# luccachiang/GSWorld

Measured on AMD Instinct MI355X. Metric: rendered frames/sec @640x480, 1.5M Gaussians, higher is better.
Workload: dtype f32

## Files before the change

### gsworld_amd/_lib.py

```python
from __future__ import annotations

import ctypes as C
import os

_HERE = os.path.dirname(os.path.abspath(__file__))
LIB_PATH = os.path.join(_HERE, "libgsr_hip.so")

GSR_OK = 0
GSR_E_INVALID = -1
GSR_E_HIP = -2
GSR_E_ALLOC = -3
GSR_E_OVERFLOW = -4
GSR_E_TRUNCATED = -5
GSR_NEAR_PLANE = 0.05
MAX_FRAMES_PER_LAUNCH = 8


class GsrSettings(C.Structure):
    _fields_ = [
        ("image_height", C.c_int32), ("image_width", C.c_int32),
        ("tanfovx", C.c_float), ("tanfovy", C.c_float), ("scale_modifier", C.c_float),
        ("sh_degree", C.c_int32), ("sh_coeffs", C.c_int32),
        ("prefiltered", C.c_int32), ("antialiasing", C.c_int32), ("debug", C.c_int32),
        ("near_plane", C.c_float),
# ... 87 lines not shown
                ("out_depth", C.c_void_p)]


PC_DENSE, PC_STRIDE, PC_FPS = 0, 1, 2
PC_MAX_VIEWS, PC_MAX_K, PC_MAX_FPS_CANDIDATES, PC_MAX_VIEW_PIXELS = 64, 8192, 16384, 1 << 24


class GsrCloudView(C.Structure):
    _fields_ = [("width", C.c_int32), ("height", C.c_int32), ("tanfovx", C.c_float), ("tanfovy", C.c_float),
                ("viewmatrix", C.c_void_p), ("depth", C.c_void_p), ("depth_scale", C.c_float), ("label", C.c_void_p),
                ("rgb8", C.c_void_p)]


class GsrCloudSpec(C.Structure):
    _fields_ = [("struct_size", C.c_int32), ("E", C.c_int32), ("C", C.c_int32), ("views", C.POINTER(GsrCloudView)),
                ("out_from_scene", C.c_float * 12), ("crop", C.c_int32), ("crop_lo", C.c_float * 3),
                ("crop_hi", C.c_float * 3), ("exclude", C.c_void_p), ("mode", C.c_int32), ("K", C.c_int32),
                ("fps_candidates", C.c_int32), ("out_xyzw", C.c_void_p), ("out_rgb", C.c_void_p),
                ("out_segmentation", C.c_void_p), ("out_count", C.c_void_p), ("workspace", C.c_void_p),
                ("workspace_bytes", C.c_int64)]


CAM_MAX_VIEWS, CAM_RECORD_FLOATS = 4096, 36


class GsrSensorCameras(C.Structure):
    _fields_ = [("struct_size", C.c_int32), ("n", C.c_int32), ("extrinsic", C.c_void_p), ("projection", C.c_void_p),
                ("out", C.c_void_p), ("offsets", C.c_void_p), ("rigid_sim2real", C.c_double * 16),
                ("scale_sim2real", C.c_double)]


class GsrProfile(C.Structure):
    _fields_ = [("frames", C.c_int32), ("stage_ms", C.c_double * 5)]


PROFILE_STAGES = ("preprocess", "depth_sort", "tile_counts+ranges", "placement", "render")


class GsrError(RuntimeError):
    def __init__(self, code: int, message: str):
        super().__init__(f"libgsr_hip error {code}: {message}")
        self.code = code


_lib = None


def lib() -> C.CDLL:
    global _lib
    if _lib is not None:
        return _lib
    if not os.path.exists(LIB_PATH):
        raise RuntimeError(
            f"{LIB_PATH} is missing: the HIP extension has not been built. Run "
            "`python -c 'import __graft_entry__ as g; g.build()'` (or `make -C gsworld_amd/csrc`). "
            "There is no CPU fallback for the rasterizer.")
    L = C.CDLL(LIB_PATH)
    L.gsr_last_error.restype = C.c_char_p
    L.gsr_version.restype = C.c_char_p
    if not hasattr(L, "gsr_abi_sizes"):
        raise RuntimeError(f"{LIB_PATH} predates the ABI handshake (gsr_abi_sizes): rebuild it (make -C gsworld_amd/csrc)")
    sizes = (C.c_int32 * 6)()
    L.gsr_abi_sizes(sizes)
    mine = (C.sizeof(GsrSettings), C.sizeof(GsrInputs), C.sizeof(GsrOutputs), C.sizeof(GsrBuffers))
    if tuple(sizes[:4]) != mine:
        raise RuntimeError(f"{LIB_PATH} was built from a different include/gsr.h (struct sizes {tuple(sizes[:4])} there, "
                           f"{mine} in gsworld_amd/_lib.py): rebuild the library")
    L.gsr_geom_bytes.restype = C.c_size_t
    L.gsr_geom_bytes.argtypes = [C.c_int32, C.c_int32, C.c_int32]
    L.gsr_binning_bytes.restype = C.c_size_t
    L.gsr_binning_bytes.argtypes = [C.c_int64]
    L.gsr_image_bytes.restype = C.c_size_t
    L.gsr_image_bytes.argtypes = [C.c_int32, C.c_int32]
    L.gsr_forward.restype = C.c_int
    L.gsr_forward.argtypes = [C.POINTER(GsrSettings), C.POINTER(GsrInputs), C.POINTER(GsrOutputs),
                              C.POINTER(GsrBuffers), C.c_int64, C.POINTER(GsrFrameStats), C.c_void_p]
    L.gsr_forward_batch.restype = C.c_int
    L.gsr_forward_batch.argtypes = [C.c_int32, C.POINTER(GsrSettings), C.POINTER(GsrInputs), C.POINTER(GsrOutputs),
                                    C.POINTER(GsrBuffers), C.POINTER(C.c_int64), C.c_void_p]
    L.gsr_frame_stats.restype = C.c_int
    L.gsr_frame_stats.argtypes = [C.c_void_p, C.POINTER(GsrFrameStats), C.c_void_p]
    L.gsr_debug_sort_state.argtypes = [C.c_void_p, C.POINTER(C.c_int32), C.c_void_p]
    L.gsr_debug_sort_state.restype = C.c_int
    L.gsr_state_view.restype = C.c_int
    L.gsr_state_view.argtypes = [C.c_int32, C.c_int32, C.c_int32, C.c_int64, C.c_void_p, C.c_void_p, C.c_void_p,
                                 C.POINTER(GsrStateView)]
    L.gsr_mark_visible.restype = C.c_int
    L.gsr_mark_visible.argtypes = [C.c_int32, C.c_void_p, C.c_void_p, C.c_float, C.c_void_p, C.c_void_p]
    L.gsr_pack_rgb8.restype = C.c_int
    L.gsr_pack_rgb8.argtypes = [C.c_void_p, C.c_int32, C.c_int32, C.c_void_p, C.c_void_p]
    L.gsr_plan_query.restype = C.c_int
    L.gsr_plan_query.argtypes = [C.POINTER(GsrSettings), C.c_int32, C.c_int32, C.c_int64, C.POINTER(C.c_int32)]
    L.gsr_pinned_device_address.restype = C.c_int
    L.gsr_pinned_device_address.argtypes = [C.c_void_p, C.POINTER(C.c_void_p)]
    L.gsr_stage_step.restype = C.c_int
    L.gsr_stage_step.argtypes = [C.c_int32, C.c_void_p, C.c_void_p, C.c_int32, C.c_int32, C.c_int32, C.c_void_p, C.c_void_p]
    L.gsr_render_maps.restype = C.c_int
    L.gsr_render_maps.argtypes = [C.c_int32, C.POINTER(GsrMapFrame), C.c_void_p]
    L.gsr_render_pointcloud.restype = C.c_int
    L.gsr_render_pointcloud.argtypes = [C.POINTER(GsrCloudSpec), C.c_void_p]
    L.gsr_pointcloud_workspace.restype = C.c_int
    L.gsr_pointcloud_workspace.argtypes = [C.POINTER(GsrCloudSpec), C.POINTER(C.c_int64)]
    L.gsr_cameras_from_extrinsics.restype = C.c_int
    L.gsr_cameras_from_extrinsics.argtypes = [C.POINTER(GsrSensorCameras), C.c_void_p]
    L.gsr_profile_enable.restype = C.c_int
    L.gsr_profile_enable.argtypes = [C.c_int]
    L.gsr_profile_collect.restype = C.c_int
    L.gsr_profile_collect.argtypes = [C.POINTER(GsrProfile)]
    _lib = L
    return L


def check(code: int) -> None:
    if code != GSR_OK:
        raise GsrError(code, lib().gsr_last_error().decode("utf-8", "replace"))


def plan_query(width: int, height: int, P: int, permuted: bool = False, forward_only: bool = True,
               r_capacity: int = 1, tuned: bool = True) -> dict | None:
    st = GsrSettings(int(height), int(width), 1.0, 1.0, 1.0, 3, 16, 0, 0, 0, float(GSR_NEAR_PLANE))
    st.forward_only = int(bool(forward_only))
    if tuned:
        apply_tuning(st)
    out = (C.c_int32 * 8)()
    if lib().gsr_plan_query(C.byref(st), int(P), int(bool(permuted)), int(r_capacity), out) != GSR_OK:
        return None
    keys = ("mode", "placement", "infer", "super", "lean", "radix_depth", "order_early", "exact")
    return dict(zip(keys, (int(v) for v in out)))


def exported_symbols() -> list[str]:
    import re

    header = os.path.join(os.path.dirname(_HERE), "include", "gsr.h")
    text = open(header).read()
    text = re.sub(r"/\*.*?\*/", "", text, flags=re.S)
    return sorted(set(re.findall(r"\b(gsr_[a-z0-9_]+)\s*\(", text)) - {"gsr_resize_fn"})
```

### gsworld_amd/csrc/api.hip

```cpp
#include <stdarg.h>
#include <stdio.h>
#include <string.h>

#include <vector>

#include "gsr_internal.h"

namespace {
thread_local char g_err[512] = "";

constexpr int kStages = GSR_PROFILE_STAGES;
constexpr int kMaxFrames = 4096;
struct Profiler {
    int mode = 0;
    int frames = 0;
    std::vector<hipEvent_t> ev;
    hipEvent_t &at(int frame, int k) { return ev[(size_t)frame * (kStages + 1) + k]; }
};
thread_local Profiler g_prof;

inline void prof_mark(int k, hipStream_t stream) {
    if (g_prof.mode == 0 || g_prof.frames >= kMaxFrames) return;
    if (g_prof.mode == 1 && k < kStages - 1) return;
    (void)hipEventRecord(g_prof.at(g_prof.frames, k), stream);
}
inline void prof_end_frame() {
    if (g_prof.mode != 0 && g_prof.frames < kMaxFrames) g_prof.frames++;
}
}

void gsr_set_error(const char *fmt, ...) {
    va_list ap;
    va_start(ap, fmt);
    vsnprintf(g_err, sizeof(g_err), fmt, ap);
    va_end(ap);
}

int gsr_check_launch(const char *what, bool debug, hipStream_t stream) {
    hipError_t e = hipGetLastError();
    if (e == hipSuccess && debug) e = hipStreamSynchronize(stream);
    if (e != hipSuccess) {
        gsr_set_error("%s: %s", what, hipGetErrorString(e));
        return GSR_E_HIP;
    }
    return GSR_OK;
}

extern "C" {

const char *gsr_last_error(void) { return g_err; }
const char *gsr_version(void) {
    static char v[96] = "";
    if (v[0] == 0) snprintf(v, sizeof(v), "gsworld_amd-gsr 0.4 (gfx950; %s)", gsr_render_build_flags());
    return v;
}
void gsr_abi_sizes(int32_t out[6]) {
    out[0] = (int32_t)sizeof(GsrSettings);
    out[1] = (int32_t)sizeof(GsrInputs);
    out[2] = (int32_t)sizeof(GsrOutputs);
    out[3] = (int32_t)sizeof(GsrBuffers);
    out[4] = (int32_t)sizeof(GsrBackwardInputs);
    out[5] = (int32_t)sizeof(GsrGrads);
}

size_t gsr_geom_bytes(int32_t P, int32_t width, int32_t height) {
    return GeomState::required(P, gsr_div_up(width, GSR_TILE) * gsr_div_up(height, GSR_TILE), gsr_div_up(width, GSR_TILE));
}
size_t gsr_binning_bytes(int64_t r_capacity) { return BinningState::required(r_capacity); }
size_t gsr_image_bytes(int32_t width, int32_t height) { return ImageState::required(width, height); }

static int validate(const GsrSettings *st, const GsrInputs *in, const GsrOutputs *out, const GsrBuffers *buf) {
    if (!st || !in || !out || !buf) {
        gsr_set_error("gsr_forward: null argument struct");
        return GSR_E_INVALID;
    }
    if (st->image_width <= 0 || st->image_height <= 0) {
        gsr_set_error("gsr_forward: image size must be positive");
        return GSR_E_INVALID;
    }
    if (gsr_div_up(st->image_width, GSR_TILE) > 65535 || gsr_div_up(st->image_height, GSR_TILE) > 65535) {
        gsr_set_error("gsr_forward: image too large for 16-bit tile rects");
        return GSR_E_INVALID;
    }
    if (in->P < 0) {
        gsr_set_error("gsr_forward: negative P");
        return GSR_E_INVALID;
    }
    const bool no_float = !out->out_color && !out->out_invdepth && st->forward_only && out->out_rgb8;
    if (((!out->out_color || !out->out_invdepth) && !no_float) || !in->background) {
        gsr_set_error("gsr_forward: out_color, out_invdepth and background are required (the two images may be NULL "
                      "together for a forward_only frame with out_rgb8)");
        return GSR_E_INVALID;
    }
    if (in->P > 0) {
        if (!in->means3D || !in->opacities || !in->viewmatrix || !in->projmatrix || !in->campos ||
            (!out->radii && !st->forward_only)) {
            gsr_set_error("gsr_forward: means3D, opacities, viewmatrix, projmatrix, campos and radii are required "
                          "(radii may be NULL for forward_only frames)");
            return GSR_E_INVALID;
        }
        if ((in->shs == nullptr) == (in->colors_precomp == nullptr)) {
            gsr_set_error("Please provide excatly one of either SHs or precomputed colors!");
            return GSR_E_INVALID;
        }
        const bool have_sr = in->scales != nullptr && in->rotations != nullptr;
        if (have_sr == (in->cov3D_precomp != nullptr) || (in->scales != nullptr) != (in->rotations != nullptr)) {
            gsr_set_error("Please provide exactly one of either scale/rotation pair or precomputed 3D covariance!");
            return GSR_E_INVALID;
        }
        if (in->shs) {
            if (st->sh_degree < 0 || st->sh_degree > 3 || st->sh_coeffs < (st->sh_degree + 1) * (st->sh_degree + 1)) {
                gsr_set_error("gsr_forward: sh_degree must be 0..3 and sh_coeffs >= (degree+1)^2");
// ... 49 lines not shown

namespace {

struct Plan {
    int W, H, tiles, tiles_x, tiles_y;
    int mode;
    bool chunk, band;
    bool exact;
    bool infer, super, lean, order_early, lean_bin;
    bool radix_depth;
    GsrSettings st_bin;
};

int make_plan(const GsrSettings *st, const GsrInputs *in, int64_t r_capacity, Plan &p, const GsrOutputs *out = nullptr) {
    p.W = st->image_width;
    p.H = st->image_height;
    p.tiles_x = gsr_div_up(p.W, GSR_TILE);
    p.tiles = p.tiles_x * gsr_div_up(p.H, GSR_TILE);
    p.tiles_y = p.tiles / p.tiles_x;
    if (r_capacity > 0xFFFFFFFFll) {
        gsr_set_error("gsr_forward: r_capacity exceeds 32-bit instance offsets");
        return GSR_E_INVALID;
    }
    const int want = (st->binning_path == 0 || st->binning_path >= 3) ? 1 : (st->binning_path == 1 ? 0 : 2);
    p.mode = GeomState::counting(p.tiles) && p.tiles_x <= 2048 ? want : 0;
    p.chunk = p.mode == 1 && st->binning_path == 4 && gsr_chunk_supported(p.tiles_x, p.tiles / p.tiles_x);
    p.band = p.mode == 1 && (st->binning_path == 0 || (st->binning_path == 4 && !p.chunk)) &&
             gsr_band_supported(p.tiles_x);
    p.exact = r_capacity <= 0;
    p.radix_depth = st->depth_sort == 1 || !gsr_ss_supported(in->P);
    p.infer = st->forward_only != 0 && (p.band || p.chunk) && !p.radix_depth;
    p.super = p.infer && st->render_variant == 0 && p.tiles_x <= 255 && p.tiles_y <= 255 &&
              gsr_render_uses_quad_order(*st, p.tiles) && gsr_render_split_blocks(*st, p.tiles) == 0;
    p.lean = p.infer && !p.chunk;
    p.st_bin = *st;
    if (p.super) {
        p.st_bin.image_width = gsr_div_up(p.tiles_x, 1 << GSR_SUPER_SX) * GSR_TILE;
        p.st_bin.image_height = gsr_div_up(p.tiles_y, 1 << GSR_SUPER_SY) * GSR_TILE;
    }
    if (in->orig_index != nullptr && !(p.infer && p.mode == 1)) {
        gsr_set_error("gsr_forward: orig_index (a permuted model) needs a forward_only frame on the default sort / "
                      "placement path");
        return GSR_E_INVALID;
    }
    if (out && !out->out_color && !p.super) {
        gsr_set_error("gsr_forward: out_color / out_invdepth may only be NULL for an inference frame on the default path "
                      "(super-tile lists, stream compositor)");
        return GSR_E_INVALID;
    }
    p.order_early = (p.band || p.chunk) && !p.radix_depth && gsr_render_uses_quad_order(*st, p.tiles);
    p.lean_bin = p.band || p.chunk;
    return GSR_OK;
}

int run_frames(int B, const GsrSettings *st, const GsrInputs *in, const GsrOutputs *out, const GsrBuffers *buf,
               const int64_t *r_capacity, const Plan *plans, GsrFrameStats *stats, hipStream_t stream) {
    const Plan &p = plans[0];
    const bool debug = st[0].debug != 0;
    const int mode = p.mode;
    const bool chunk = p.chunk, band = p.band, exact = p.exact, infer = p.infer, super = p.super;
    const int coop = super && band && mode == 1 && !p.radix_depth && p.order_early ? gsr_render_coop_blocks(st[0], p.tiles, B) : 0;
    GsrFrame fr[GSR_MAX_BATCH];
    for (int k = 0; k < B; k++) {
        GsrFrame &f = fr[k];
        f.st = &st[k];
        f.st_bin = &plans[k].st_bin;
        f.in = &in[k];
        f.out = &out[k];
        char *geom_mem = buf[k].geom_resize(buf[k].geom_user, GeomState::required(in[k].P, p.tiles, p.tiles_x, p.lean));
        char *img_mem = buf[k].image_resize(buf[k].image_user, ImageState::required(p.W, p.H));
        if (!geom_mem || !img_mem) {
            gsr_set_error("gsr_forward: resize callback returned NULL");
            return GSR_E_ALLOC;
        }
        f.g = GeomState::carve(geom_mem, in[k].P, p.tiles, nullptr, p.tiles_x, p.lean);
        f.img = ImageState::carve(img_mem, p.W, p.H);
        f.cap32 = exact ? 0xFFFFFFFFu : (uint32_t)r_capacity[k];
        f.pc = GSR_PREP_BLOCK_CACHE && infer && band && mode == 1 && !p.radix_depth && ((uint32_t)in[k].param_space >> 8) != 0u &&
               in[k].part_labels != nullptr && in[k].cull_blocks != nullptr && out[k].radii == nullptr &&
               in[k].part_count <= GSR_PC_MAX_PARTS &&
               (in[k].appearance == nullptr || in[k].appearance_versions != nullptr);
        f.td = GSR_TILE_REUSE && f.pc && super && (in[k].param_space & GSR_FRAME_KEPT) != 0 && out[k].out_rgb8 != nullptr &&
               out[k].out_color == nullptr && out[k].out_invdepth == nullptr;
    }
    const GeomState &g = fr[0].g;
    const ImageState &img = fr[0].img;

    if (mode == 2) {
        const size_t head = offsetof(GsrHeader, of_magic);
        const size_t clear = (size_t)((char *)g.tile_cursor - (char *)g.tile_accum);
        if (hipMemsetAsync(g.hdr, 0, head, stream) != hipSuccess ||
            hipMemsetAsync(g.tile_accum, 0, clear, stream) != hipSuccess) {
            gsr_set_error("gsr_forward: hipMemsetAsync(header) failed");
            return GSR_E_HIP;
        }
    }
    prof_mark(0, stream);
    if (int e = gsr_launch_preprocess(B, fr, mode == 2, infer, stream)) return e;
    if (int e = gsr_check_launch("preprocess", debug, stream)) return e;
    prof_mark(1, stream);
    if (mode != 2) {
        if (p.radix_depth) {
            if (int e = gsr_launch_compact_and_depth_sort(in[0].P, g, debug, stream)) return e;
            if (band || chunk)
                if (int e = gsr_launch_gather_rects(in[0].P, g, debug, stream)) return e;
        } else {
            if (int e = gsr_launch_sample_depth_sort(B, fr, p.order_early, 4 * p.tiles, super ? 1 : 0, coop, debug, stream))
                return e;
        }
    }
    prof_mark(2, stream);
    if (mode == 2) {
        if (int e = gsr_launch_bin_starts(st[0], g, img, fr[0].cap32, debug, stream)) return e;
    } else if (chunk) {
        if (int e = gsr_launch_chunk_count(p.st_bin, in[0].P, g, debug, stream)) return e;
        if (int e = gsr_launch_tile_starts(1, fr, p.order_early, debug, stream)) return e;
    } else if (band) {
        bool starts_done = false;
        if (int e = gsr_launch_band_count(B, fr, !p.radix_depth, p.order_early, &starts_done, debug, stream)) return e;
        if (!starts_done)
            if (int e = gsr_launch_tile_starts(B, fr, p.order_early, debug, stream)) return e;
    } else if (mode == 1) {
        if (int e = gsr_launch_tile_count(st[0], in[0].P, g, img, fr[0].cap32, debug, stream)) return e;
    } else {
        if (int e = gsr_launch_tile_offsets(in[0].P, g, fr[0].cap32, debug, stream)) return e;
    }
    prof_mark(3, stream);
    if (!(band || chunk))
        for (int k = 0; k < B; k++)
            if (out[k].overflow_mirror &&
                hipMemcpyAsync(out[k].overflow_mirror, &fr[k].g.hdr->of_magic, 8, hipMemcpyDefault, stream) != hipSuccess) {
                gsr_set_error("gsr_forward: overflow mirror copy failed: %s", hipGetErrorString(hipGetLastError()));
                return GSR_E_HIP;
            }
    int64_t cap0 = r_capacity[0];
    if (exact) {
        GsrHeader h;
        if (hipMemcpyAsync(&h, g.hdr, sizeof(h), hipMemcpyDeviceToHost, stream) != hipSuccess ||
            hipStreamSynchronize(stream) != hipSuccess) {
            gsr_set_error("gsr_forward: header read-back failed: %s", hipGetErrorString(hipGetLastError()));
            return GSR_E_HIP;
        }
        cap0 = h.R_raw;
        if (stats) {
            stats->num_visible = h.V;
            stats->num_rendered = h.R_raw;
            stats->overflow = 0;
            stats->overflow_frames = h.of_magic == GSR_OF_MAGIC ? (int32_t)h.overflow_frames : 0;
        }
    }
    for (int k = 0; k < B; k++) {
        const int64_t cap = k == 0 ? cap0 : r_capacity[k];
        char *bin_mem = buf[k].binning_resize(buf[k].binning_user, BinningState::required(cap, p.lean_bin));
        if (!bin_mem) {
            gsr_set_error("gsr_forward: binning resize callback returned NULL");
            return GSR_E_ALLOC;
        }
        fr[k].b = BinningState::carve(bin_mem, cap, nullptr, p.lean_bin);
    }
    const BinningState &b = fr[0].b;
    if (mode == 2) {
        if (int e = gsr_launch_bin_scatter_and_sort(st[0], in[0].P, g, b, img, debug, stream)) return e;
    } else if (chunk) {
        if (int e = gsr_launch_chunk_place(p.st_bin, in[0].P, g, b, img, debug, stream)) return e;
    } else if (band) {
        if (int e = gsr_launch_band_place(B, fr, debug, stream)) return e;
    } else if (mode == 1) {
        if (int e = gsr_launch_tile_place(st[0], in[0].P, g, b, img, debug, stream)) return e;
    } else {
        if (int e = gsr_launch_emit_and_tile_sort(st[0], in[0].P, g, b, img, cap0, debug, stream)) return e;
    }
    prof_mark(4, stream);
    if (int e = gsr_launch_render(B, fr, mode != 0, mode == 1, super, coop, stream)) return e;
    prof_mark(5, stream);
    prof_end_frame();
    return gsr_check_launch("render", debug, stream);
}

int zero_outputs(const GsrSettings *st, const GsrOutputs *out, hipStream_t stream) {
    const size_t n = (size_t)st->image_width * st->image_height;
    if ((out->out_color && hipMemsetAsync(out->out_color, 0, 3 * n * sizeof(float), stream) != hipSuccess) ||
        (out->out_invdepth && hipMemsetAsync(out->out_invdepth, 0, n * sizeof(float), stream) != hipSuccess) ||
        (out->out_rgb8 && hipMemsetAsync(out->out_rgb8, 0, 3 * n, stream) != hipSuccess)) {
        gsr_set_error("gsr_forward: hipMemsetAsync(outputs) failed");
        return GSR_E_HIP;
    }
    return GSR_OK;
}

}

extern "C" {

int gsr_forward(const GsrSettings *st, const GsrInputs *in, const GsrOutputs *out, const GsrBuffers *buf,
                int64_t r_capacity, GsrFrameStats *stats, void *stream_) {
    if (int e = validate(st, in, out, buf)) return e;
    hipStream_t stream = (hipStream_t)stream_;
    if (stats) memset(stats, 0, sizeof(*stats));
    if (in->P == 0) return zero_outputs(st, out, stream);
    Plan p;
    if (int e = make_plan(st, in, r_capacity, p, out)) return e;
    return run_frames(1, st, in, out, buf, &r_capacity, &p, stats, stream);
}

int gsr_forward_batch(int32_t B, const GsrSettings *st, const GsrInputs *in, const GsrOutputs *out,
                      const GsrBuffers *buf, const int64_t *r_capacity, void *stream_) {
    if (B < 0 || (B > 0 && (!st || !in || !out || !buf || !r_capacity))) {
        gsr_set_error("gsr_forward_batch: null argument array or negative B");
        return GSR_E_INVALID;
    }
    hipStream_t stream = (hipStream_t)stream_;
    for (int k = 0; k < B; k++)
        if (int e = validate(&st[k], &in[k], &out[k], &buf[k])) return e;
    Plan plans[GSR_MAX_BATCH];
    auto shares = [&](int a, int b, const Plan &pa, const Plan &pb) {
        const GsrSettings &x = st[a], &y = st[b];
        return in[a].P == in[b].P && pa.W == pb.W && pa.H == pb.H && pa.mode == pb.mode && pa.band == pb.band &&
               pa.infer == pb.infer && pa.super == pb.super && pa.lean == pb.lean && pa.order_early == pb.order_early &&
               x.sh_degree == y.sh_degree && x.sh_coeffs == y.sh_coeffs && x.debug == y.debug &&
               x.render_variant == y.render_variant && x.render_blocks_per_cu == y.render_blocks_per_cu &&
               x.render_split == y.render_split && x.depth_sort == y.depth_sort &&
               (in[a].colors_precomp == nullptr) == (in[b].colors_precomp == nullptr);
    };
    int k = 0;
    while (k < B) {
        if (in[k].P == 0) {
            if (int e = zero_outputs(&st[k], &out[k], stream)) return e;
            k++;
            continue;
        }
        if (int e = make_plan(&st[k], &in[k], r_capacity[k], plans[0], &out[k])) return e;
        int n = 1;
        const bool batchable = plans[0].mode == 1 && plans[0].band && !plans[0].radix_depth && !plans[0].exact &&
                               st[k].render_variant == 0;
        while (batchable && n < GSR_MAX_BATCH && k + n < B && in[k + n].P != 0 && r_capacity[k + n] > 0) {
            if (int e = make_plan(&st[k + n], &in[k + n], r_capacity[k + n], plans[n], &out[k + n])) return e;
            if (!shares(k, k + n, plans[0], plans[n])) break;
            n++;
        }
        if (int e = run_frames(n, st + k, in + k, out + k, buf + k, r_capacity + k, plans, nullptr, stream)) return e;
        k += n;
    }
    return GSR_OK;
}

int gsr_plan_query(const GsrSettings *st, int32_t P, int32_t permuted, int64_t r_capacity, int32_t out[8]) {
    if (!st || !out || P < 0 || st->image_width <= 0 || st->image_height <= 0) {
        gsr_set_error("gsr_plan_query: null argument, negative P or empty image");
        return GSR_E_INVALID;
    }
    GsrInputs in;
    memset(&in, 0, sizeof(in));
    in.P = P;
    static const int32_t one = 0;
    in.orig_index = permuted ? &one : nullptr;
    Plan p;
    if (int e = make_plan(st, &in, r_capacity, p)) return e;
    out[0] = p.mode;
    out[1] = p.band ? 1 : (p.chunk ? 2 : 0);
    out[2] = p.infer ? 1 : 0;
    out[3] = p.super ? 1 : 0;
    out[4] = p.lean ? 1 : 0;
    out[5] = p.radix_depth ? 1 : 0;
    out[6] = p.order_early ? 1 : 0;
    out[7] = p.exact ? 1 : 0;
    return GSR_OK;
}

int gsr_render_maps(int32_t B, const GsrMapFrame *frames, void *stream_) {
    if (B < 0 || (B > 0 && !frames)) {
        gsr_set_error("gsr_render_maps: null frame array or negative B");
        return GSR_E_INVALID;
    }
    hipStream_t stream = (hipStream_t)stream_;
    std::vector<GsrMapsArgs> jobs;
    jobs.reserve((size_t)B);
    bool debug = false;
    for (int k = 0; k < B; k++) {
        const GsrMapFrame &f = frames[k];
        if (f.struct_size != (int32_t)sizeof(GsrMapFrame)) {
            gsr_set_error("gsr_render_maps: frame %d: struct_size %d, this library's GsrMapFrame has %d bytes", k,
                          (int)f.struct_size, (int)sizeof(GsrMapFrame));
            return GSR_E_INVALID;
        }
        const GsrSettings *st = f.settings;
        if (!st || st->image_width <= 0 || st->image_height <= 0 || f.P < 0) {
            gsr_set_error("gsr_render_maps: frame %d: null settings, empty image or negative P", k);
            return GSR_E_INVALID;
        }
        if (f.out_label && !f.labels) {
            gsr_set_error("gsr_render_maps: frame %d: out_label needs labels", k);
            return GSR_E_INVALID;
        }
        if (f.P > 0 && (!f.geom || !f.binning || !f.image)) {
            gsr_set_error("gsr_render_maps: frame %d: the frame's three state buffers are required", k);
            return GSR_E_INVALID;
        }
        GsrInputs in;
        memset(&in, 0, sizeof(in));
        in.P = f.P;
        static const int32_t one = 0;
        in.orig_index = f.permuted ? &one : nullptr;
        Plan p;
        if (make_plan(st, &in, f.r_capacity, p) != GSR_OK) {
            gsr_set_error("gsr_render_maps: frame %d is not one gsr_forward renders (permuted model on another path, or "
                          "r_capacity beyond 32 bits)", k);
            return GSR_E_INVALID;
        }
        debug = debug || st->debug != 0;
        const size_t n = (size_t)p.W * p.H;
        if (f.P == 0) {
            if ((f.out_label && hipMemsetAsync(f.out_label, 0xFF, n * sizeof(int16_t), stream) != hipSuccess) ||
                (f.out_depth && hipMemsetAsync(f.out_depth, 0, n * sizeof(float), stream) != hipSuccess)) {
                gsr_set_error("gsr_render_maps: hipMemsetAsync failed");
                return GSR_E_HIP;
            }
            continue;
        }
        if (!f.out_label && !f.out_depth) continue;
        const GeomState g = GeomState::carve((char *)f.geom, f.P, p.tiles);
        const BinningState b = BinningState::carve((char *)f.binning, 1);
        const ImageState s = ImageState::carve((char *)f.image, p.W, p.H);
        GsrMapsArgs a;
        a.ranges = s.ranges;
        a.point_list = b.gidx[0];
        a.splat = g.splat;
        a.hdr = g.hdr;
        a.labels = f.labels;
        a.out_label = f.out_label;
        a.out_depth = f.out_depth;
        a.depth_scale = f.depth_scale;
        a.W = p.W;
        a.H = p.H;
        a.gx = p.tiles_x;
        a.gy = p.tiles_y;
        a.super = p.super ? 1 : 0;
        jobs.push_back(a);
    }
    if (jobs.empty()) return GSR_OK;
    return gsr_launch_maps((int)jobs.size(), jobs.data(), debug, stream);
}

int gsr_profile_enable(int mode) {
    if (mode < 0 || mode > 2) {
        gsr_set_error("gsr_profile_enable: mode must be 0, 1 or 2");
        return GSR_E_INVALID;
    }
    if (mode != 0 && g_prof.ev.empty()) {
        g_prof.ev.resize((size_t)kMaxFrames * (kStages + 1));
        for (auto &e : g_prof.ev)
            if (hipEventCreate(&e) != hipSuccess) {
                gsr_set_error("gsr_profile_enable: hipEventCreate failed");
                return GSR_E_HIP;
            }
    }
    g_prof.mode = mode;
    g_prof.frames = 0;
    return GSR_OK;
}

int gsr_profile_collect(GsrProfile *out) {
    if (!out) {
        gsr_set_error("gsr_profile_collect: null output");
        return GSR_E_INVALID;
    }
    memset(out, 0, sizeof(*out));
    out->frames = g_prof.frames;
    for (int f = 0; f < g_prof.frames; f++) {
        for (int k = (g_prof.mode == 1 ? kStages - 1 : 0); k < kStages; k++) {
            if (hipEventSynchronize(g_prof.at(f, k + 1)) != hipSuccess) {
                gsr_set_error("gsr_profile_collect: hipEventSynchronize failed");
                return GSR_E_HIP;
            }
            float ms = 0.f;
            if (hipEventElapsedTime(&ms, g_prof.at(f, k), g_prof.at(f, k + 1)) != hipSuccess) {
                gsr_set_error("gsr_profile_collect: hipEventElapsedTime failed");
                return GSR_E_HIP;
            }
            out->stage_ms[k] += (double)ms;
        }
    }
    g_prof.frames = 0;
    return GSR_OK;
}

int gsr_debug_ss_stamps(int32_t P, int32_t width, int32_t height, const void *geom, uint64_t *out64) {
    if (!geom || !out64) {
        gsr_set_error("gsr_debug_ss_stamps: null argument");
        return GSR_E_INVALID;
    }
    const bool lean = height < 0;
    if (lean) height = -height;
    const GeomState g = GeomState::carve((char *)geom, P, gsr_div_up(width, GSR_TILE) * gsr_div_up(height, GSR_TILE),
                                         nullptr, gsr_div_up(width, GSR_TILE), lean);
    if (hipDeviceSynchronize() != hipSuccess ||
        hipMemcpy(out64, g.ss_dbg, 64 * sizeof(uint64_t), hipMemcpyDeviceToHost) != hipSuccess) {
        gsr_set_error("gsr_debug_ss_stamps: copy failed");
        return GSR_E_HIP;
    }
    return GSR_OK;
}

int gsr_debug_sort_state(const void *geom, int32_t out[8], void *stream_) {
    if (!geom || !out) {
        gsr_set_error("gsr_debug_sort_state: null argument");
        return GSR_E_INVALID;
    }
    hipStream_t stream = (hipStream_t)stream_;
    GsrHeader h;
    if (hipMemcpyAsync(&h, geom, sizeof(h), hipMemcpyDeviceToHost, stream) != hipSuccess ||
        hipStreamSynchronize(stream) != hipSuccess) {
        gsr_set_error("gsr_debug_sort_state: read-back failed: %s", hipGetErrorString(hipGetLastError()));
        return GSR_E_HIP;
    }
    out[0] = (int32_t)h.ss_blind;
    out[1] = (int32_t)h.ss_fresh;
    out[2] = (int32_t)h.ss_bad;
    out[3] = (int32_t)h.ss_trust;
    out[4] = (int32_t)h.ss_B;
    out[5] = (int32_t)h.ss_stride;
    out[6] = (int32_t)h.coop_quads;
    out[7] = (int32_t)((h.ss_near & 1u) | ((h.pc_hit_last & 1u) << 1) | ((h.td_skipped & 1u) << 2));
    return GSR_OK;
}

int gsr_frame_stats(const void *geom, GsrFrameStats *stats, void *stream_) {
    if (!geom || !stats) {
        gsr_set_error("gsr_frame_stats: null argument");
        return GSR_E_INVALID;
    }
    hipStream_t stream = (hipStream_t)stream_;
    GsrHeader h;
    if (hipMemcpyAsync(&h, geom, sizeof(h), hipMemcpyDeviceToHost, stream) != hipSuccess ||
        hipStreamSynchronize(stream) != hipSuccess) {
        gsr_set_error("gsr_frame_stats: read-back failed: %s", hipGetErrorString(hipGetLastError()));
        return GSR_E_HIP;
    }
    stats->num_visible = h.V;
    stats->num_rendered = h.R_raw;
    stats->overflow = (int32_t)h.overflow;
    stats->overflow_frames = h.of_magic == GSR_OF_MAGIC ? (int32_t)h.overflow_frames : 0;
    stats->truncated = h.coop_timeout_now != 0u ? 1 : 0;
    stats->coop_timeouts = h.of_magic == GSR_OF_MAGIC ? (int32_t)h.coop_timeouts : 0;
    return h.overflow ? GSR_E_OVERFLOW : (stats->truncated ? GSR_E_TRUNCATED : GSR_OK);
}

int gsr_state_view(int32_t P, int32_t width, int32_t height, int64_t r_capacity, const void *geom, const void *binning,
                   const void *image, GsrStateView *v) {
    if (!v) {
        gsr_set_error("gsr_state_view: null view");
        return GSR_E_INVALID;
    }
    memset(v, 0, sizeof(*v));
    if (geom) {
        const GeomState g = GeomState::carve((char *)geom, P, gsr_div_up(width, GSR_TILE) * gsr_div_up(height, GSR_TILE));
        v->splat = reinterpret_cast<const float *>(g.splat);
        v->cov3D = g.cov3D;
        v->clamped = reinterpret_cast<const uint8_t *>(g.clamped);
        v->tiles_touched = g.tiles_touched;
        v->rects = reinterpret_cast<const uint16_t *>(g.rects);
        v->depth_order = g.order;
    }
    if (binning) {
        const BinningState b = BinningState::carve((char *)binning, r_capacity);
        v->point_list = b.gidx[0];
        v->point_tiles = nullptr;
    }
    if (image) {
        const ImageState s = ImageState::carve((char *)image, width, height);
        v->ranges = reinterpret_cast<const uint32_t *>(s.ranges);
        v->final_T = s.final_T;
        v->n_contrib = s.n_contrib;
    }
    return GSR_OK;
}

}
```

### gsworld_amd/csrc/bandplace.hip

```cpp
#include "gsr_internal.h"

#ifndef GSR_BAND_EXACT_CUTS
#define GSR_BAND_EXACT_CUTS 0
#endif

namespace {

constexpr int kBT = GSR_BLOCK;
constexpr int kBW = kBT / GSR_WAVE;
constexpr int kRing = 128;
constexpr uint32_t kSplit2 = 1024u, kSplit4 = 2048u;
constexpr int kMaxSegments = 4;

constexpr uint32_t kCutsMagic = 0x43555453u;

__device__ __forceinline__ uint32_t band_cuts_block(const GsrHeader *__restrict__ hdr, int bmax,
                                                    const uint32_t *__restrict__ bucket_start,
                                                    const uint32_t *__restrict__ bucket_tiles,
                                                    const uint32_t *__restrict__ tile_cum,
                                                    const uint32_t *__restrict__ wave_lo_base, uint32_t sig, uint32_t r,
                                                    uint32_t *s_cut , uint32_t *s_pre ,
                                                    uint32_t *s_bs , uint32_t *s_w ) {
    constexpr int waves = GSR_BAND_RANGES * kBW;
    static_assert(waves == kBT, "a thread per kept cut");
    const int tid = (int)threadIdx.x;
    const uint32_t V = hdr->V, base_V = hdr->br_V, magic = hdr->br_magic, hP = hdr->br_P;
    const int B = (int)hdr->ss_B;
    const uint32_t wb0 = wave_lo_base[tid], wb1 = wave_lo_base[tid + 1];
    const uint32_t wbj = tid <= kBW ? wave_lo_base[r * (uint32_t)kBW + (uint32_t)tid] : 0u;
    if (tile_cum == nullptr || V == 0u) {
        const uint32_t per = (((V + (uint32_t)waves - 1u) / (uint32_t)waves) + 63u) & ~63u;
        if (tid <= kBW) s_cut[tid] = min(V, (r * (uint32_t)kBW + (uint32_t)tid) * per);
        __syncthreads();
        return 0u;
    }
    bool keep = magic == kCutsMagic && hP == sig && base_V != 0u;
    if (keep) {
        uint32_t bad = wb0 > wb1 ? 1u : 0u;
        if (tid == 0) bad |= wb0 != 0u ? 1u : 0u;
        if (tid == waves - 1) bad |= wb1 != base_V ? 1u : 0u;
        keep = __syncthreads_or((int)bad) == 0;
    }
    if (keep) {
        if (tid <= kBW) {
            const uint32_t j = r * (uint32_t)kBW + (uint32_t)tid;
            s_cut[tid] = j == (uint32_t)waves ? V : min(V, (uint32_t)((double)wbj * ((double)V / (double)base_V)));
        }
        __syncthreads();
        return 1u;
    }
    const int PER = B / kBT;
    uint32_t bt[8], bs[8];
#pragma unroll
    for (int k = 0; k < 8; k++) {
        bt[k] = k < PER ? bucket_tiles[tid + k * kBT] : 0u;
        bs[k] = k < PER ? bucket_start[tid + k * kBT] : 0u;
    }
    const uint32_t bs_B = tid == 0 ? bucket_start[B] : 0u;
#pragma unroll
    for (int k = 0; k < 8; k++)
        if (k < PER) {
            s_pre[tid + k * kBT] = bt[k];
            s_bs[tid + k * kBT] = bs[k];
        }
    if (tid == 0) s_bs[B] = bs_B;
    __syncthreads();
    uint32_t t[8], sum = 0;
#pragma unroll
    for (int k = 0; k < 8; k++) {
        t[k] = k < PER ? s_pre[tid * PER + k] : 0u;
        sum += t[k];
    }
    uint32_t total;
    uint32_t run = gsr_block_incl_scan(sum, s_w, total) - sum;
#pragma unroll
    for (int k = 0; k < 8; k++) {
        if (k < PER && t[k] != 0u) {
            const int b = tid * PER + k;
#pragma unroll
            for (int c = 0; c <= kBW; c++) {
                const uint32_t j = r * (uint32_t)kBW + (uint32_t)c;
                const uint32_t target = (uint32_t)(((uint64_t)total * j) / (uint32_t)waves);
                if (j != (uint32_t)waves && target >= run && target - run < t[k]) {
                    const uint32_t s0 = s_bs[b], n = s_bs[b + 1] - s0, rest = target - run;
                    s_cut[c] = s0 + min(n, (uint32_t)((float)n * ((float)rest / (float)t[k])));
                }
            }
        }
        run += t[k];
    }
    if (tid <= kBW) {
        const uint32_t j = r * (uint32_t)kBW + (uint32_t)tid;
        if (j == (uint32_t)waves || total == 0u) s_cut[tid] = j == (uint32_t)waves ? V : 0u;
    }
    __syncthreads();
// ... 141 lines not shown
        v[k] = lane * PL + k < GSR_BAND_RANGES ? row[lane * PL + k] : 0u;
        sum += v[k];
    }
    const uint32_t incl = gsr_wave_incl_scan(sum);
    uint32_t run = incl - sum;
#pragma unroll
    for (int k = 0; k < PL; k++) {
        if (lane * PL + k < GSR_BAND_RANGES) row[lane * PL + k] = run;
        run += v[k];
    }
    if (lane == 63) totals[t] = incl;
}

__device__ __forceinline__ uint64_t wave_bit_transpose(uint64_t R) {
    const uint32_t lane = (uint32_t)gsr_lane();
    constexpr uint64_t kLow[6] = {0x00000000FFFFFFFFull, 0x0000FFFF0000FFFFull, 0x00FF00FF00FF00FFull,
                                  0x0F0F0F0F0F0F0F0Full, 0x3333333333333333ull, 0x5555555555555555ull};
#pragma unroll
    for (int i = 0; i < 6; i++) {
        const int s = 32 >> i;
        const uint64_t m = kLow[i];
        const uint32_t tlo = (uint32_t)__shfl_xor((int)(uint32_t)R, s, 64);
        const uint32_t thi = (uint32_t)__shfl_xor((int)(uint32_t)(R >> 32), s, 64);
        const uint64_t t = ((uint64_t)thi << 32) | tlo;
        R = (lane & (uint32_t)s) == 0u ? ((R & m) | ((t & m) << s)) : ((R & ~m) | ((t & ~m) >> s));
    }
    return R;
}

template <int NC>
__device__ __forceinline__ void band_place_round(uint32_t span, uint32_t g, bool valid, int gx, uint32_t *cur,
                                                 unsigned long long *colmask, uint32_t *__restrict__ point_list) {
    const int lane = gsr_lane();
    const uint64_t lt = gsr_lanemask_lt();
    const uint32_t minx = span & 0xffffu, maxx = span >> 16, w = valid ? maxx - minx : 0u;
    constexpr uint32_t kNarrow = 16;
    const uint32_t wn = min(w, kNarrow);
    uint32_t wmax = wn;
#pragma unroll
    for (int o = 32; o > 0; o >>= 1) wmax = max(wmax, (uint32_t)__shfl_xor((int)wmax, o, 64));
    wmax = (uint32_t)__builtin_amdgcn_readfirstlane((int)wmax);
    uint32_t add[NC];
#pragma unroll
    for (int k = 0; k < NC; k++) {
        const uint32_t lo = max(minx, (uint32_t)(64 * k)), hi = min(maxx, (uint32_t)(64 * k + 64));
        uint64_t row = 0ull;
        if (valid && hi > lo) row = (hi - lo == 64u ? ~0ull : ((1ull << (hi - lo)) - 1ull)) << (lo - (uint32_t)(64 * k));
        const uint64_t col = wave_bit_transpose(row);
        colmask[k * 64 + lane] = col;
        add[k] = (uint32_t)__popcll(col);
    }
    __builtin_amdgcn_wave_barrier();
    for (uint32_t j0 = 0; j0 < wmax; j0 += 4u) {
        unsigned long long m[4];
        uint32_t cx[4];
#pragma unroll
        for (uint32_t u = 0; u < 4u; u++) {
            m[u] = j0 + u < wn ? colmask[minx + j0 + u] : 0ull;
            cx[u] = j0 + u < wn ? cur[minx + j0 + u] : 0u;
        }
#pragma unroll
        for (uint32_t u = 0; u < 4u; u++)
            if (j0 + u < wn) point_list[cx[u] + (uint32_t)__popcll(m[u] & lt)] = g;
    }
    for (uint64_t wide = __builtin_amdgcn_ballot_w64(w > kNarrow); wide;) {
        const int src = __ffsll((unsigned long long)wide) - 1;
        wide &= wide - 1ull;
        const uint32_t sw = (uint32_t)__builtin_amdgcn_readlane((int)w, src);
        const uint32_t sx = (uint32_t)__builtin_amdgcn_readlane((int)minx, src);
        const uint32_t sg = (uint32_t)__builtin_amdgcn_readlane((int)g, src);
        const uint64_t below = (1ull << src) - 1ull;
        for (uint32_t j = kNarrow + (uint32_t)lane; j < sw; j += 64u)
            point_list[cur[sx + j] + (uint32_t)__popcll(colmask[sx + j] & below)] = sg;
    }
    __builtin_amdgcn_wave_barrier();
#pragma unroll
    for (int k = 0; k < NC; k++) cur[k * 64 + lane] += add[k];
    __builtin_amdgcn_wave_barrier();
}

constexpr int kPlaceBatch = 6;

template <int NC>
__device__ __forceinline__ void band_place_body(const uint32_t seg, const uint2 *__restrict__ rect_sorted,
                                                         const uint32_t *__restrict__ order,
                                                         const GsrHeader *__restrict__ hdr,
                                                         const uint32_t *__restrict__ wave_lo, int gx, int NR,
                                                         const uint32_t *__restrict__ table,
                                                         const uint32_t *__restrict__ wtable,
                                                         const uint2 *__restrict__ ranges,
                                                         uint32_t *__restrict__ point_list,
                                                         const uint32_t *__restrict__ nseg_tab) {
    __shared__ uint2 s_ring[kBW][kRing];
    __shared__ unsigned long long s_mask[kBW][NC * 64];
    __shared__ uint32_t s_cur[kBW][NC * 64];
    const int lane = gsr_lane(), wave = gsr_wave();
    const uint32_t r = blockIdx.x, y = blockIdx.y;
    const uint32_t nseg = (nseg_tab[(size_t)y * (uint32_t)NR + r] >> (8u * (uint32_t)__builtin_amdgcn_readfirstlane(wave))) & 255u;
    if (seg >= nseg) return;
    if (hdr->overflow) return;
    const uint32_t lo = wave_lo[r * kBW + (uint32_t)wave], hi = wave_lo[r * kBW + (uint32_t)wave + 1u];
    if (lo >= hi) return;
    uint2 *ring = s_ring[wave];
    uint32_t *cur = s_cur[wave];
    unsigned long long *colmask = s_mask[wave];
    const uint32_t *wbase = wtable + (size_t)(y * (uint32_t)NR + r) * kBW * (NC * 64);
    uint32_t x0 = 0u, x1 = (uint32_t)gx;
    if (nseg > 1u) {
        uint32_t mine[NC], total = 0u;
#pragma unroll
        for (int k = 0; k < NC; k++) {
            const int x = k * 64 + lane;
            mine[k] = x < gx ? wbase[wave * (NC * 64) + x] : 0u;
            total += mine[k];
        }
#pragma unroll
        for (int o = 32; o > 0; o >>= 1) total += (uint32_t)__shfl_xor((int)total, o, 64);
        {
            uint32_t before = 0u, first = 0xFFFFFFFFu, last = 0u;
#pragma unroll
            for (int k = 0; k < NC; k++) {
                const uint32_t incl = gsr_wave_incl_scan(mine[k]);
                const uint32_t excl = before + incl - mine[k];
                const bool in = k * 64 + lane < gx && (uint32_t)(((uint64_t)excl * nseg) / total) == seg;
                const uint64_t m = __builtin_amdgcn_ballot_w64(in);
                if (m != 0ull) {
                    first = min(first, (uint32_t)(k * 64 + __builtin_ctzll(m)));
                    last = max(last, (uint32_t)(k * 64 + 64 - __builtin_clzll(m)));
                }
                before += (uint32_t)__builtin_amdgcn_readlane((int)incl, 63);
            }
            if (first == 0xFFFFFFFFu) return;
            x0 = first;
            x1 = last;
        }
    }
#pragma unroll
    for (int k = 0; k < NC; k++) {
        const int x = k * 64 + lane;
        uint32_t s = 0u;
        if (x < gx) {
            const size_t tile = (size_t)y * gx + x;
            s = ranges[tile].x + table[tile * NR + r];
            for (int w = 0; w < wave; w++) s += wbase[w * (NC * 64) + x];
        }
        cur[x] = s;
    }
    __builtin_amdgcn_wave_barrier();
    uint32_t head = 0, tail = 0;
    for (uint32_t base = lo; base < hi; base += (uint32_t)(kPlaceBatch * GSR_WAVE)) {
        uint2 rc[kPlaceBatch];
        uint32_t g[kPlaceBatch];
#pragma unroll
        for (int u = 0; u < kPlaceBatch; u++) {
            const uint32_t i = base + (uint32_t)(u * GSR_WAVE + lane);
            rc[u] = i < hi ? rect_sorted[i] : make_uint2(0u, 0u);
            g[u] = i < hi ? order[i] : 0u;
        }
#pragma unroll
        for (int u = 0; u < kPlaceBatch; u++) {
            const uint32_t miny = rc[u].x >> 16, maxy = rc[u].y >> 16;
            const uint32_t minx = max(rc[u].x & 0xffffu, x0), maxx = min(rc[u].y & 0xffffu, x1);
            const bool keep = miny <= y && y < maxy && minx < maxx;
            const uint64_t mask = __builtin_amdgcn_ballot_w64(keep);
            if (mask == 0ull) continue;
            if (keep) {
                const uint32_t rank = __builtin_amdgcn_mbcnt_hi((uint32_t)(mask >> 32),
                                                                __builtin_amdgcn_mbcnt_lo((uint32_t)mask, 0u));
                ring[(tail + rank) & (kRing - 1)] = make_uint2(minx | (maxx << 16), g[u]);
            }
            tail += (uint32_t)__popcll(mask);
            __builtin_amdgcn_wave_barrier();
            if (tail - head >= (uint32_t)GSR_WAVE) {
                const uint2 p = ring[(head + (uint32_t)lane) & (kRing - 1)];
                __builtin_amdgcn_wave_barrier();
                band_place_round<NC>(p.x, p.y, true, gx, cur, colmask, point_list);
                head += (uint32_t)GSR_WAVE;
            }
        }
    }
    if (tail != head) {
        const bool valid = (uint32_t)lane < tail - head;
        const uint2 p = valid ? ring[(head + (uint32_t)lane) & (kRing - 1)] : make_uint2(0u, 0u);
        band_place_round<NC>(p.x, p.y, valid, gx, cur, colmask, point_list);
    }
}

struct BandArgs {
    GsrHeader *hdr;
    int bmax;
    const uint32_t *bucket_start, *bucket_tiles, *tile_cum;
    int waves;
    uint32_t *wave_lo, *wave_lo_base;
    uint32_t sig;
    const uint2 *rect_sorted;
    int gx, NR, T;
    uint32_t *table, *wtable, *totals, *nseg;
    const uint32_t *order;
    const uint2 *ranges;
    uint32_t *point_list;
    uint32_t r_capacity;
    uint2 *ranges_w;
    const uint32_t *quad_work;
    uint32_t *tile_order;
    uint32_t *mirror;
};

template <int NC>
__global__ __launch_bounds__(kBT) void band_count_kernel(const GsrBatch<BandArgs> bt) {
    const BandArgs &a = bt.f[blockIdx.z];
    band_count_body<NC>(a.rect_sorted, a.hdr, a.bmax, a.bucket_start, a.bucket_tiles, a.tile_cum, a.waves, a.wave_lo, a.wave_lo_base,
                        a.sig, a.gx, a.NR, a.table, a.wtable, a.nseg);
}
__global__ __launch_bounds__(kBT) void band_scan_kernel(const GsrBatch<BandArgs> bt) {
    const BandArgs &a = bt.f[blockIdx.y];
    if (blockIdx.x == gridDim.x - 1) {
        band_cuts_next(a.hdr, a.bucket_start, a.bucket_tiles, a.tile_cum, a.wave_lo_base, a.sig);
        return;
    }
    band_scan_body(a.table, a.T, a.totals);
}
template <int NC>
__global__ __launch_bounds__(kBT, 8) void band_place_kernel(const GsrBatch<BandArgs> bt) {
    const BandArgs &a = bt.f[blockIdx.z / (uint32_t)kMaxSegments];
    band_place_body<NC>(blockIdx.z % (uint32_t)kMaxSegments, a.rect_sorted, a.order, a.hdr, a.wave_lo, a.gx, a.NR, a.table,
                        a.wtable, a.ranges, a.point_list, a.nseg);
}

#ifndef GSR_SCAN_MODE
#define GSR_SCAN_MODE 1
#endif
constexpr int kSST = 1024, kSSW = kSST / GSR_WAVE;
constexpr int kSSMaxTiles = 8 * kSST;
constexpr int kSSMergeTiles = 1024;
static_assert(GSR_BAND_RANGES == GSR_WAVE, "a tile's row of the band table is one entry per lane");

template <int THREADS, int MAXPER>
__device__ __forceinline__ void band_starts_block(const uint32_t *totals, int T, GsrHeader *__restrict__ hdr,
                                                  uint32_t r_capacity, uint2 *__restrict__ ranges, uint32_t *s_wv,
                                                  uint32_t *__restrict__ mirror) {
    constexpr int NWV = THREADS / GSR_WAVE;
    const int tid = (int)threadIdx.x, lane = gsr_lane(), wave = tid >> 6;
    const int per = (T + THREADS - 1) / THREADS, t0 = tid * per;
    uint32_t v[MAXPER], sum = 0;
#pragma unroll
    for (int k = 0; k < MAXPER; k++) {
        v[k] = (k < per && t0 + k < T) ? totals[t0 + k] : 0u;
        sum += v[k];
    }
    const uint32_t incl = gsr_wave_incl_scan(sum);
    if (lane == 63) s_wv[wave] = incl;
    __syncthreads();
    uint32_t add = 0, grand = 0;
#pragma unroll
    for (int w = 0; w < NWV; w++) {
        const uint32_t x = s_wv[w];
        add += w < wave ? x : 0u;
        grand += x;
    }
    uint32_t run = incl - sum + add;
    const bool overflow = grand > r_capacity;
#pragma unroll
    for (int k = 0; k < MAXPER; k++) {
        const int t = t0 + k;
        if (k < per && t < T) ranges[t] = (v[k] == 0u || overflow) ? make_uint2(0u, 0u) : make_uint2(run, run + v[k]);
        run += v[k];
    }
    if (tid == 0) {
        hdr->R_raw = grand;
        hdr->r_capacity = r_capacity;
        gsr_set_overflow(hdr, overflow, mirror);
        hdr->R = overflow ? 0u : grand;
    }
}

__device__ __forceinline__ void band_scan_starts_body(uint32_t *__restrict__ table, int T, GsrHeader *__restrict__ hdr,
                                                      uint32_t r_capacity, uint2 *__restrict__ ranges,
                                                      uint32_t *__restrict__ mirror) {
    __shared__ uint32_t s_tot[kSSMaxTiles];
    __shared__ uint32_t s_wv[kSSW];
    const int lane = gsr_lane(), wave = (int)(threadIdx.x >> 6);
    constexpr int kU = 16;
    for (int t0 = wave; t0 < T; t0 += kSSW * kU) {
        uint32_t v[kU];
#pragma unroll
        for (int u = 0; u < kU; u++) {
            const int t = t0 + u * kSSW;
            v[u] = t < T ? table[(size_t)t * GSR_BAND_RANGES + lane] : 0u;
        }
#pragma unroll
        for (int u = 0; u < kU; u++) {
            const int t = t0 + u * kSSW;
            const uint32_t incl = gsr_wave_incl_scan(v[u]);
            if (t < T) {
                table[(size_t)t * GSR_BAND_RANGES + lane] = incl - v[u];
                if (lane == 63) s_tot[t] = incl;
            }
        }
    }
    __syncthreads();
    band_starts_block<kSST, kSSMaxTiles / kSST>(s_tot, T, hdr, r_capacity, ranges, s_wv, mirror);
}

__global__ __launch_bounds__(kSST) void band_scan_starts_kernel(const GsrBatch<BandArgs> bt) {
    const BandArgs &a = bt.f[blockIdx.y];
    if (blockIdx.x == 1) {
        if (threadIdx.x >= kBT) return;
        band_cuts_next(a.hdr, a.bucket_start, a.bucket_tiles, a.tile_cum, a.wave_lo_base, a.sig);
        return;
    }
    if (blockIdx.x == 2) {
        if (threadIdx.x >= kBT) return;
        __shared__ uint32_t s_bins[64], s_red[4];
        uint32_t key[32];
#pragma unroll
        for (int i = 0; i < 32; i++) {
            const int t = (int)threadIdx.x + i * kBT;
            key[i] = t < a.T ? gsr_tile_order_key(nullptr, a.quad_work, t) : 0u;
        }
        gsr_tile_order_block_keys<32>(key, a.T, a.tile_order, s_bins, s_red);
        return;
    }
    band_scan_starts_body(a.table, a.T, a.hdr, a.r_capacity, a.ranges_w, a.mirror);
}
__global__ __launch_bounds__(kBT) void band_scan_tail_kernel(const GsrBatch<BandArgs> bt) {
    const BandArgs &a = bt.f[blockIdx.y];
    __shared__ uint32_t s_last, s_wv[kBW];
    if (blockIdx.x == gridDim.x - 1) {
        band_cuts_next(a.hdr, a.bucket_start, a.bucket_tiles, a.tile_cum, a.wave_lo_base, a.sig);
        return;
    }
    band_scan_body(a.table, a.T, a.totals);
    __threadfence();
    __syncthreads();
    if (threadIdx.x == 0) s_last = atomicAdd(&a.hdr->tile_queue, 1u) == gridDim.x - 2u ? 1u : 0u;
    __syncthreads();
    if (s_last == 0u) return;
    __threadfence();
    if (threadIdx.x == 0) a.hdr->tile_queue = 0u;
    band_starts_block<kBT, kSSMaxTiles / kBT>(a.totals, a.T, a.hdr, a.r_capacity, a.ranges_w, s_wv, a.mirror);
}

__global__ __launch_bounds__(kBT) void gather_rects_kernel(const uint32_t *__restrict__ order,
                                                           const uint2 *__restrict__ rects,
                                                           const GsrHeader *__restrict__ hdr,
                                                           uint2 *__restrict__ rect_sorted) {
    const uint32_t V = hdr->V;
    for (uint32_t i = blockIdx.x * (uint32_t)kBT + threadIdx.x; i < V; i += gridDim.x * (uint32_t)kBT)
        rect_sorted[i] = rects[order[i]];
}

}

bool gsr_band_supported(int gx) { return gx <= 256; }

int gsr_launch_gather_rects(int32_t P, const GeomState &g, bool debug, hipStream_t stream) {
    const int blocks = GeomState::prep_blocks(P) < 1024 ? GeomState::prep_blocks(P) : 1024;
    hipLaunchKernelGGL(gather_rects_kernel, dim3(blocks), dim3(kBT), 0, stream, g.order, g.rects, g.hdr, g.rect_sorted);
    return gsr_check_launch("gather_rects", debug, stream);
}

static void band_args(int B, const GsrFrame *fr, bool balanced, bool place, GsrBatch<BandArgs> &bt) {
    for (int k = 0; k < B; k++) {
        const GeomState &g = fr[k].g;
        const GsrSettings &st = *fr[k].st_bin;
        BandArgs &a = bt.f[k];
        const int32_t P = fr[k].in->P;
        a.hdr = g.hdr;
        a.bmax = gsr_ss_bmax(P);
        a.bucket_start = g.ss_bucket_start;
        a.bucket_tiles = g.bucket_tiles;
        a.tile_cum = balanced ? g.tile_cum : (const uint32_t *)nullptr;
        a.waves = GSR_BAND_RANGES * kBW;
        a.wave_lo = g.wave_lo;
        a.wave_lo_base = g.wave_lo_base;
        a.sig = (uint32_t)P * 2654435761u ^ (uint32_t)((char *)g.wave_lo_base - (char *)g.hdr);
        a.rect_sorted = g.rect_sorted;
        a.gx = gsr_div_up(st.image_width, GSR_TILE);
        a.NR = GSR_BAND_RANGES;
        a.T = a.gx * gsr_div_up(st.image_height, GSR_TILE);
        a.table = g.band_table;
        a.wtable = g.band_wtable;
        a.totals = g.tile_totals;
        a.nseg = g.band_nseg;
        a.order = g.order;
        a.ranges = fr[k].img.ranges;
        a.ranges_w = fr[k].img.ranges;
        a.r_capacity = fr[k].cap32;
        a.quad_work = fr[k].img.quad_work;
        a.tile_order = fr[k].img.tile_order;
        a.mirror = fr[k].out ? fr[k].out->overflow_mirror : (uint32_t *)nullptr;
        a.point_list = place ? fr[k].b.gidx[0] : (uint32_t *)nullptr;
    }
}

int gsr_launch_band_count(int B, const GsrFrame *fr, bool balanced, bool merge_starts, bool *starts_done, bool debug,
                          hipStream_t stream) {
    const GsrSettings &st = *fr[0].st_bin;
    const int gx = gsr_div_up(st.image_width, GSR_TILE), gy = gsr_div_up(st.image_height, GSR_TILE);
    GsrBatch<BandArgs> bt{};
    band_args(B, fr, balanced, false, bt);
    const dim3 grid(GSR_BAND_RANGES, gy, B);
    if (gx <= 64)
        hipLaunchKernelGGL(band_count_kernel<1>, grid, dim3(kBT), 0, stream, bt);
    else if (gx <= 128)
        hipLaunchKernelGGL(band_count_kernel<2>, grid, dim3(kBT), 0, stream, bt);
    else
        hipLaunchKernelGGL(band_count_kernel<4>, grid, dim3(kBT), 0, stream, bt);
    if (int e = gsr_check_launch("band_count", debug, stream)) return e;
    const int T = gx * gy;
    const bool by_tiles = !merge_starts && gsr_render_wants_tile_order(st, T) && !gsr_render_uses_quad_order(st, T);
    const bool merged = GSR_SCAN_MODE != 0 && (merge_starts || (by_tiles && GSR_SCAN_MODE == 1)) && T <= kSSMergeTiles &&
                        gsr_render_split_blocks(st, T) == 0;
    if (starts_done) *starts_done = merged;
    if (merged && GSR_SCAN_MODE == 1) {
        hipLaunchKernelGGL(band_scan_starts_kernel, dim3(by_tiles ? 3 : 2, B), dim3(kSST), 0, stream, bt);
        return gsr_check_launch("band_scan_starts", debug, stream);
    }
    if (merged) {
        hipLaunchKernelGGL(band_scan_tail_kernel, dim3(gsr_div_up(T, kBW) + 1, B), dim3(kBT), 0, stream, bt);
        return gsr_check_launch("band_scan_tail", debug, stream);
    }
    hipLaunchKernelGGL(band_scan_kernel, dim3(gsr_div_up(T, kBW) + 1, B), dim3(kBT), 0, stream, bt);
    return gsr_check_launch("band_scan", debug, stream);
}

int gsr_launch_band_place(int B, const GsrFrame *fr, bool debug, hipStream_t stream) {
    const GsrSettings &st = *fr[0].st_bin;
    const int gx = gsr_div_up(st.image_width, GSR_TILE), gy = gsr_div_up(st.image_height, GSR_TILE);
    GsrBatch<BandArgs> bt{};
    band_args(B, fr, true, true, bt);
    const dim3 grid(GSR_BAND_RANGES, gy, kMaxSegments * B);
    if (gx <= 64)
        hipLaunchKernelGGL(band_place_kernel<1>, grid, dim3(kBT), 0, stream, bt);
    else if (gx <= 128)
        hipLaunchKernelGGL(band_place_kernel<2>, grid, dim3(kBT), 0, stream, bt);
    else
        hipLaunchKernelGGL(band_place_kernel<4>, grid, dim3(kBT), 0, stream, bt);
    return gsr_check_launch("band_place", debug, stream);
}
```

### gsworld_amd/csrc/depthsort.hip

```cpp
#include "gsr_internal.h"
#include <type_traits>

namespace {

#ifdef GSR_SS_TIMING
#define SS_STAMP(buf, slot) do { __syncthreads(); if (blockIdx.x == (buf##_wg) && threadIdx.x == 0) (buf)[slot] = __builtin_amdgcn_s_memtime(); } while (0)
#else
#define SS_STAMP(buf, slot) do { } while (0)
#endif

constexpr int kT = GSR_BLOCK;
#ifndef GSR_SS_TRUST_MIN
#define GSR_SS_TRUST_MIN 2
#endif
#ifndef GSR_SS_IGNORE_BAD
#define GSR_SS_IGNORE_BAD 0
#endif
#ifndef GSR_SS_SPB
#define GSR_SS_SPB 4
#endif
constexpr int kSamplesPerBucket = GSR_SS_SPB;
constexpr int kMinSamples = 2048;
constexpr int kMaxSamples = 4096;
constexpr uint32_t kSplitMagic = 0x53504c54u;
// ... 297 lines not shown
__device__ __forceinline__ void ss_prepare_body(int P, int nb1, int bmax, int nbc,
                                                const uint2 *__restrict__ block_recs,
                                                const uint32_t *__restrict__ block_counts,
                                                const uint32_t *__restrict__ splitters,
                                                uint32_t *__restrict__ splitters_new, uint32_t *__restrict__ seg_off,
                                                uint32_t *__restrict__ seg_first, GsrHeader *__restrict__ hdr,
                                                uint64_t *__restrict__ dbg, const float *__restrict__ view,
                                                uint32_t sig, const int role, const bool pc_enabled) {
    const unsigned dbg_wg = 0; (void)dbg_wg;
    SS_STAMP(dbg, 0);
#ifdef GSR_SS_TIMING
    if (role == 0 && threadIdx.x < 8) dbg[48 + threadIdx.x] = 0ull;
#endif
    __shared__ uint32_t s_key[2 * kMaxSamples];
    __shared__ __attribute__((aligned(16))) uint32_t s_cur[kPW * 256];
    __shared__ uint32_t s_split[2048], s_hist[2048];
    __shared__ uint32_t s_pex[kPT + 8];
    __shared__ __attribute__((aligned(16))) uint16_t s_cnt16[kPrepBlocks];
    __shared__ uint32_t s_w16[kPW];
    const int tid = (int)threadIdx.x, wave = tid >> 6, lane = gsr_lane();
    const int per = ss_prepare_per(nb1);
    const uint32_t h_magic = hdr->ss_magic, h_buckets = hdr->ss_buckets, h_bad = hdr->ss_bad, h_trust = hdr->ss_trust,
                   h_P = hdr->ss_P, h_near = hdr->ss_near, h_near_fail = hdr->ss_near_fail, h_vfail = hdr->ss_vfail;
    const uint32_t h_pc_pending = hdr->pc_pending, h_pc_parity = hdr->pc_parity, h_pc_sig_next = hdr->pc_sig_next,
                   h_pc_hit = hdr->pc_hit;
    bool same_view = true, near_view = true;
#pragma unroll
    for (int k = 0; k < 16; k++) {
        const uint32_t was = hdr->ss_view[k];
        same_view = same_view && __float_as_uint(view[k]) == was;
        near_view = near_view && fabsf(view[k] - __uint_as_float(was)) <= kNearTol;
    }
    uint32_t pre_sp[2];
#pragma unroll
    for (int k = 0; k < 2; k++) pre_sp[k] = tid + k * kPT < bmax - 1 ? splitters[tid + k * kPT] : 0xFFFFFFFFu;
    for (int i0 = tid; i0 < per * kPT; i0 += 8 * kPT) {
        uint32_t c[8];
#pragma unroll
        for (int u = 0; u < 8; u++) c[u] = i0 + u * kPT < nb1 ? block_counts[i0 + u * kPT] : 0u;
#pragma unroll
        for (int u = 0; u < 8; u++)
            if (i0 + u * kPT < per * kPT) s_cnt16[i0 + u * kPT] = (uint16_t)c[u];
    }
    __syncthreads();
    uint32_t mine = 0;
    {
        uint4 *sl = reinterpret_cast<uint4 *>(s_cnt16 + (size_t)tid * per);
        for (int w = 0; w < (per >> 3); w++) {
            const uint4 v = sl[w];
            const uint32_t x[4] = {v.x, v.y, v.z, v.w};
            uint32_t o[4];
#pragma unroll
            for (int h = 0; h < 4; h++) {
                mine += x[h] & 0xffffu;
                const uint32_t a = mine;
                mine += x[h] >> 16;
                o[h] = a | (mine << 16);
            }
            sl[w] = make_uint4(o[0], o[1], o[2], o[3]);
        }
    }
    SS_STAMP(dbg, 1);
    uint32_t V;
    const uint32_t p_incl = ss_scan1024(mine, s_w16, V), p_excl = p_incl - mine;
    (void)p_incl;
    s_pex[tid] = p_excl;
    if (tid == 0) s_pex[kPT] = V;
    if (tid == 0 && role == 0) {
        if (pc_enabled && h_pc_pending == GSR_PC_MAGIC) {
            hdr->pc_parity = (h_pc_parity & 1u) ^ 1u;
            hdr->pc_sig = h_pc_sig_next;
            hdr->pc_magic = GSR_PC_MAGIC;
        } else {
            hdr->pc_magic = 0u;
        }
        hdr->pc_pending = 0u;
        hdr->pc_hit_last = pc_enabled ? h_pc_hit : 0u;
        hdr->pc_hit = 0u;
        hdr->td_skipped = 0u;
        hdr->V = V;
        hdr->R = 0u;
        hdr->overflow = 0u;
        hdr->coop_timeout_now = 0u;
        hdr->r_capacity = 0u;
        hdr->R_raw = 0u;
        hdr->tile_queue = 0u;
    }
    if (V == 0u) {
        if (role == 1)
            for (int j = tid; j <= nbc; j += kPT) {
                seg_off[j] = 0u;
                seg_first[j] = (uint32_t)nb1;
            }
        if (tid == 0 && role == 0) {
            hdr->ss_fresh = 0u;
            hdr->ss_B = 256u;
            hdr->ss_stride = 1u;
            hdr->ss_near = 0u;
            hdr->ss_moved = 1u;
        }
        return;
    }
    __syncthreads();
    SS_STAMP(dbg, 22);
    if (role == 1) {
    if (tid <= nbc) {
        uint32_t j = 0u, before_j = 0u;
        if (tid == nbc) {
            j = (uint32_t)nb1;
            before_j = V;
        } else if (tid > 0) {
            const uint32_t W = V + kBlockCost * (uint32_t)nb1;
            const uint32_t t = (uint32_t)((double)W * (double)tid / (double)nbc);
            uint32_t us = 0u;
#pragma unroll
            for (int st = kPT / 2; st > 0; st >>= 1)
                if (s_pex[us + (uint32_t)st] + kBlockCost * min((uint32_t)nb1, (us + (uint32_t)st) * (uint32_t)per) <= t)
                    us += (uint32_t)st;
            const uint32_t jb = min((uint32_t)nb1, us * (uint32_t)per), je = min((uint32_t)nb1, jb + (uint32_t)per);
            uint32_t pos = 0u;
#pragma unroll
            for (int st = 16; st > 0; st >>= 1) {
                const uint32_t k = jb + pos + (uint32_t)st;
                if (pos + (uint32_t)st < (uint32_t)per && k < je &&
                    s_pex[us] + (uint32_t)s_cnt16[k - 1u] + kBlockCost * k <= t)
                    pos += (uint32_t)st;
            }
            j = jb + pos;
            before_j = s_pex[us] + (pos > 0u ? (uint32_t)s_cnt16[j - 1u] : 0u);
        }
        seg_off[tid] = before_j;
        seg_first[tid] = j;
    }
        return;
    }
    int B0 = ss_num_buckets(V, bmax, (uint32_t)GSR_SS_PER_BUCKET);
    if (GSR_SS_NEAR != 0 && h_magic == kSplitMagic && h_P == sig && h_buckets >= 256u && h_buckets <= (uint32_t)bmax &&
        (h_buckets & (h_buckets - 1u)) == 0u && V >= h_buckets * 224u && V <= h_buckets * 576u)
        B0 = (int)h_buckets;
    const int Bf = ss_num_buckets(V, bmax, (uint32_t)GSR_SS_PER_BUCKET_FULL);
    const bool table_ok = h_magic == kSplitMagic && h_buckets <= (uint32_t)bmax && (GSR_SS_IGNORE_BAD || h_bad == 0u) &&
                          h_trust <= 255u && h_P == sig;
    const bool blind_same = same_view && table_ok && (h_buckets == (uint32_t)Bf || h_buckets == 2u * (uint32_t)Bf) &&
                            h_trust >= (uint32_t)GSR_SS_TRUST_MIN;
    uint32_t near_fail = h_near_fail > 6u ? 0u : h_near_fail;
    if (h_magic == kSplitMagic && h_near == 1u && h_bad != 0u && near_fail < 6u) near_fail++;
    const bool blind_near = GSR_SS_NEAR != 0 && !same_view && near_view && table_ok && h_buckets == (uint32_t)B0 &&
                            h_trust >= (2u << near_fail);
    bool blind = blind_same || blind_near;
    const int B = blind_same ? Bf : B0;
    const uint32_t stride = blind_same ? h_buckets / (uint32_t)Bf : 1u;
    if (tid == 0) {
        hdr->ss_B = (uint32_t)B;
        hdr->ss_stride = stride;
        hdr->ss_moved = same_view ? 0u : 1u;
        hdr->ss_near_fail = near_fail;
    }
    const uint32_t S = (uint32_t)min(kMaxSamples, max(kSamplesPerBucket * B, kMinSamples));
    const int logS = ss_log2((int)S);
    const bool table_there = h_magic == kSplitMagic && h_buckets == (uint32_t)B && h_P == sig;
    const uint32_t vfail = (h_magic == kSplitMagic && h_vfail <= 255u) ? h_vfail : 0u;
    const bool attempt = table_there && (GSR_SS_PROBE_EVERY == 0 || vfail == 0u || vfail >= (uint32_t)GSR_SS_PROBE_EVERY);
    const bool need_table = blind || attempt;
    bool ascending = false;
    if (need_table) {
    if (stride == 1u) {
// ... 1096 lines not shown
```

### gsworld_amd/csrc/gsr_internal.h

```cpp
#pragma once

#include <hip/hip_runtime.h>
#include <stdint.h>
#include <stddef.h>

#include "../../include/gsr.h"

#define GSR_WAVE 64
#define GSR_BLOCK 256
#define GSR_SORT_ITEMS 8
#define GSR_SORT_CHUNK (GSR_BLOCK * GSR_SORT_ITEMS)
#define GSR_RADIX_BITS 8
#define GSR_RADIX_BINS 256
#define GSR_DEPTH_RADIX_BITS 11
#define GSR_DEPTH_RADIX_BINS 2048
#define GSR_BIN_SLOTS 16
#ifndef GSR_SS_PER_BUCKET
#define GSR_SS_PER_BUCKET 512
#endif
#ifndef GSR_SS_PER_BUCKET_FULL
#define GSR_SS_PER_BUCKET_FULL 1024
#endif
#ifndef GSR_COOP_MAX_FRAMES
#define GSR_COOP_MAX_FRAMES 8
#endif
#ifndef GSR_COOP_MAX_BLOCKS
#define GSR_COOP_MAX_BLOCKS 64
#endif
#ifndef GSR_COOP_FACTOR_X16
#define GSR_COOP_FACTOR_X16 40
#endif
#define GSR_BAND_RANGES 64
#ifndef GSR_SUPER_SX
#define GSR_SUPER_SX 1
#endif
#ifndef GSR_SUPER_SY
#define GSR_SUPER_SY 0
#endif
#define GSR_MAX_COUNT_TILES 16384

struct GsrHeader {
    uint32_t V;
    uint32_t R;
    uint32_t overflow;
    uint32_t r_capacity;
    uint32_t R_raw;
    uint32_t tile_queue;
    uint32_t ss_magic;
    uint32_t ss_buckets;
    uint32_t ss_bad;
    uint32_t ss_view[16];
    uint32_t ss_blind;
    uint32_t br_magic;
    uint32_t br_V;
    uint32_t br_age;
    uint32_t ss_P;
    uint32_t br_P;
    uint32_t ss_trust;
    uint32_t ss_prev_fresh;
    uint32_t ss_fresh;
    uint32_t ss_B;
    uint32_t ss_stride;
    uint32_t coop_quads;
    uint32_t br_route;
    uint32_t coop_timeouts;
    uint32_t coop_timeout_now;
    uint32_t ss_moved;
    uint32_t ss_near;
    uint32_t ss_near_fail;
    uint32_t ss_vfail;
    uint32_t pc_magic;
    uint32_t pc_parity;
    uint32_t pc_pending;
    uint32_t pc_sig;
    uint32_t pc_sig_next;
    uint32_t pc_hit;
    uint32_t pc_hit_last;
    uint32_t td_token;
    uint32_t td_reuse;
    uint32_t td_skipped;
    uint32_t pad[8];
    uint32_t of_magic;
    uint32_t overflow_frames;
};
#define GSR_OF_MAGIC 0x0F10F10Fu
#ifndef GSR_TILE_REUSE
#define GSR_TILE_REUSE 1
#endif
#ifndef GSR_PREP_BLOCK_CACHE
#define GSR_PREP_BLOCK_CACHE 1
#endif
#define GSR_PC_MAGIC 0x50434348u
#define GSR_PC_MAX_PARTS 64
#define GSR_PC_APP (40 + 17 * GSR_PC_MAX_PARTS)
#define GSR_PC_SLOT (GSR_PC_APP + 68)
__device__ inline void gsr_set_overflow(GsrHeader *hdr, bool overflow, uint32_t *mirror = nullptr) {
    const bool was = hdr->overflow != 0u;
    hdr->overflow = overflow ? 1u : 0u;
    uint32_t magic = hdr->of_magic, count = hdr->overflow_frames;
    if (overflow && !was) {
        if (magic != GSR_OF_MAGIC) {
            hdr->of_magic = magic = GSR_OF_MAGIC;
            count = 0u;
            hdr->coop_timeouts = 0u;
        }
        hdr->overflow_frames = ++count;
    }
    if (mirror != nullptr) {
        mirror[1] = magic == GSR_OF_MAGIC ? count : 0u;
        mirror[0] = magic;
    }
}
__device__ inline void gsr_note_coop_timeout(GsrHeader *hdr) {
    if (hdr->of_magic != GSR_OF_MAGIC) {
        hdr->overflow_frames = 0u;
        hdr->coop_timeouts = 0u;
        __threadfence();
        hdr->of_magic = GSR_OF_MAGIC;
    }
    atomicAdd(&hdr->coop_timeouts, 1u);
    hdr->coop_timeout_now = 1u;
}
static_assert(sizeof(GsrHeader) == 256, "header is one 256-byte line");

static inline size_t gsr_align_up(size_t x, size_t a = 256) { return (x + a - 1) / a * a; }
static inline int gsr_div_up(int64_t a, int64_t b) { return (int)((a + b - 1) / b); }

int gsr_ss_nbc(int32_t P);
int gsr_ss_bmax(int32_t P);
bool gsr_ss_supported(int32_t P);

#ifndef GSR_GRAD_F64
#define GSR_GRAD_F64 1
#endif
#if GSR_GRAD_F64
typedef double GsrGradWord;
#else
typedef float GsrGradWord;
#endif

struct GeomState {
    GsrHeader *hdr;
    uint32_t *tile_accum;
    uint32_t *tile_cursor;
    float4 *splat;
    float *cov3D;
    uint32_t *clamped;
    uint2 *block_recs;
    float *pc_slots;
    GsrGradWord *grad_rec;
    uint32_t *tiles_touched;
    uint2 *rects;
    uint32_t *block_counts;
    uint2 *pair[2];
    uint32_t *order;
    uint32_t *sort_table;
    uint32_t *sort_totals;
    uint32_t *tile_bsum;
    uint32_t *tile_table;
    uint32_t *tile_totals;
    uint32_t *vis_key;
    uint32_t *block_cand;
    uint32_t *ss_table;
    uint32_t *ss_splitters;
    uint32_t *ss_totals;
    uint32_t *ss_splitters_new;
    uint32_t *ss_bucket_start;
    uint32_t *ss_seg;
// ... 43 lines not shown
        g.sort_table = take<uint32_t>(p, lean ? 0 : (size_t)GSR_DEPTH_RADIX_BINS * sort_blocks(P));
        g.sort_totals = take<uint32_t>(p, GSR_DEPTH_RADIX_BINS);
        g.tile_bsum = take<uint32_t>(p, (size_t)sort_blocks(P) + 1);
        const size_t tt = counting(tiles) ? (size_t)tiles : 0;
        g.tile_table = take<uint32_t>(p, (lean ? 0 : tt * prep_blocks(P)) + 1);
        g.tile_totals = take<uint32_t>(p, tt + 1);
        g.vis_key = take<uint32_t>(p, 0);
        g.block_cand = take<uint32_t>(p, (size_t)prep_blocks(P));
        g.ss_table = take<uint32_t>(p, (size_t)gsr_ss_nbc(P) * gsr_ss_bmax(P));
        g.ss_splitters = take<uint32_t>(p, (size_t)gsr_ss_bmax(P));
        g.ss_bucket_start = take<uint32_t>(p, (size_t)gsr_ss_bmax(P) + 1);
        g.ss_seg = take<uint32_t>(p, (size_t)gsr_ss_nbc(P) + 1);
        g.ss_dbg = take<uint64_t>(p, 64);
        g.rect_sorted = take<uint2>(p, n);
        g.band_table = take<uint32_t>(p, (size_t)tiles * GSR_BAND_RANGES + 1);
        g.tile_cum = take<uint32_t>(p, n);
        g.bucket_tiles = take<uint32_t>(p, (size_t)gsr_ss_bmax(P));
        g.wave_lo = take<uint32_t>(p, (size_t)GSR_BAND_RANGES * 4 + 1);
        g.wave_lo_base = take<uint32_t>(p, (size_t)GSR_BAND_RANGES * 4 + 1);
        g.ss_splitters_new = take<uint32_t>(p, (size_t)gsr_ss_bmax(P));
        g.ss_totals = take<uint32_t>(p, (size_t)gsr_ss_bmax(P));
        g.band_nseg = take<uint32_t>(p, (size_t)tiles * GSR_BAND_RANGES);
        g.ss_first = take<uint32_t>(p, (size_t)gsr_ss_nbc(P) + 1);
        g.block_recs = take<uint2>(p, n);
        g.pc_slots = take<float>(p, 2 * GSR_PC_SLOT);
        g.band_wtable = take<uint32_t>(p, band_wtable_words(tiles_x, tiles));
        if (bytes) *bytes = (size_t)(p - base);
        return g;
    }
    static size_t required(int32_t P, int tiles, int tiles_x = 0, bool lean = false) {
        size_t bytes = 0;
        carve(nullptr, P, tiles, &bytes, tiles_x, lean);
        return bytes;
    }
};

struct BinningState {
    uint32_t *tile[2];
    uint32_t *gidx[2];
    uint32_t *sort_table;
    uint32_t *sort_totals;
    uint64_t *keys64;

    static int sort_blocks(int64_t rcap) { return gsr_div_up(rcap > 0 ? rcap : 1, GSR_SORT_CHUNK); }
    static BinningState carve(char *base, int64_t rcap, size_t *bytes = nullptr, bool lean = false) {
        BinningState b;
        char *p = base;
        const size_t n = (size_t)(rcap > 0 ? rcap : 1), nf = lean ? 0 : n;
        b.gidx[0] = GeomState::take<uint32_t>(p, n);
        b.keys64 = GeomState::take<uint64_t>(p, nf);
        b.tile[0] = GeomState::take<uint32_t>(p, nf);
        b.tile[1] = GeomState::take<uint32_t>(p, nf);
        b.gidx[1] = GeomState::take<uint32_t>(p, nf);
        b.sort_table = GeomState::take<uint32_t>(p, lean ? 0 : (size_t)GSR_RADIX_BINS * sort_blocks(rcap));
        b.sort_totals = GeomState::take<uint32_t>(p, lean ? 0 : GSR_RADIX_BINS);
        if (bytes) *bytes = (size_t)(p - base);
        return b;
    }
    static size_t required(int64_t rcap, bool lean = false) {
        size_t bytes = 0;
        carve(nullptr, rcap, &bytes, lean);
        return bytes;
    }
    static int tile_bits(int num_tiles) {
        int bits = 1;
        while ((1 << bits) < num_tiles) bits++;
        return bits;
    }
    static int tile_passes(int num_tiles) { return (tile_bits(num_tiles) + GSR_RADIX_BITS - 1) / GSR_RADIX_BITS; }
};

struct ImageState {
    uint2 *ranges;
    float *final_T;
    uint32_t *n_contrib;
    uint32_t *tile_order;
    uint32_t *quad_work;
    uint32_t *quad_work_b;
    uint32_t *split_flag;
    uint32_t *split_list;
    uint32_t *split_count;
    uint32_t *quad_order;
    uint32_t *tile_dirty;
    static ImageState carve(char *base, int32_t W, int32_t H, size_t *bytes = nullptr) {
        ImageState s;
        char *p = base;
        const size_t tiles = (size_t)gsr_div_up(W, GSR_TILE) * gsr_div_up(H, GSR_TILE);
        s.ranges = GeomState::take<uint2>(p, tiles);
        s.tile_order = GeomState::take<uint32_t>(p, tiles);
        s.quad_work = GeomState::take<uint32_t>(p, 4 * tiles);
        s.quad_work_b = GeomState::take<uint32_t>(p, 4 * tiles);
        s.split_flag = GeomState::take<uint32_t>(p, 4 * tiles);
        s.split_list = GeomState::take<uint32_t>(p, 4 * tiles);
        s.split_count = GeomState::take<uint32_t>(p, 64);
        s.quad_order = GeomState::take<uint32_t>(p, 4 * tiles);
        s.final_T = GeomState::take<float>(p, (size_t)W * H);
        s.n_contrib = GeomState::take<uint32_t>(p, (size_t)W * H);
        s.tile_dirty = GeomState::take<uint32_t>(p, tiles);
        if (bytes) *bytes = (size_t)(p - base);
        return s;
    }
    static size_t required(int32_t W, int32_t H) {
        size_t bytes = 0;
        carve(nullptr, W, H, &bytes);
        return bytes;
    }
};

#if defined(__HIPCC__)
__device__ __forceinline__ float exp_canonical(float x) {
    if (x > 88.72283905206835f) return __builtin_inff();
    if (x < -103.972084045410f) return 0.0f;
    const float n = __builtin_rintf(x * 1.44269504088896341f);
    float r = __builtin_fmaf(n, -0.693359375f, x);
    r = __builtin_fmaf(n, 2.12194440e-4f, r);
    float p = 1.9875691500e-4f;
    p = __builtin_fmaf(p, r, 1.3981999507e-3f);
    p = __builtin_fmaf(p, r, 8.3334519073e-3f);
    p = __builtin_fmaf(p, r, 4.1665795894e-2f);
    p = __builtin_fmaf(p, r, 1.6666665459e-1f);
    p = __builtin_fmaf(p, r, 5.0000001201e-1f);
    const float y = __builtin_fmaf(p, r * r, r) + 1.0f;
    return __builtin_ldexpf(y, (int)n);
}

#ifndef GSR_EXP_ACCURATE
#define GSR_EXP_ACCURATE 0
#endif
__device__ __forceinline__ float gsr_exp_power(float power) {
    constexpr float L = 1.4426950408889634f;
    const float t = power * L;
#if GSR_EXP_ACCURATE
    constexpr float L_lo = (float)(1.4426950408889634073599246810019 - (double)1.4426950408889634f);
    const float e = __builtin_fmaf(power, L_lo, __builtin_fmaf(power, L, -t));
    const float x = __builtin_amdgcn_exp2f(t);
    return __builtin_fmaf(x * 0.6931471805599453f, e, x);
#else
    return __builtin_amdgcn_exp2f(t);
#endif
}

template <bool HAVE_TAU = false>
__device__ __forceinline__ bool quadrant_may_hit(float cx, float cy, const float4 q, float x0, float y0,
                                                 float yext = 7.0f, float tau_in = 0.0f) {
    const float A = q.x, B = q.y, C = q.z;
    const float dxh = cx - x0, dxl = cx - (x0 + 7.0f);
    const float dyh = cy - y0, dyl = cy - (y0 + yext);
    const float tau = HAVE_TAU ? tau_in : -0.6931471805599453f * __builtin_amdgcn_logf(255.0f * q.w);
    const float ex = fminf(fmaxf(0.0f, dxl), dxh);
    const float ey = fminf(fmaxf(0.0f, dyl), dyh);
    const float sy = fminf(fmaxf(-(B * ex) * __builtin_amdgcn_rcpf(C), dyl), dyh);
    const float sx = fminf(fmaxf(-(B * ey) * __builtin_amdgcn_rcpf(A), dxl), dxh);
    const float f1 = __builtin_fmaf(-B * ex, sy, -0.5f * __builtin_fmaf(C * sy, sy, (A * ex) * ex));
    const float f2 = __builtin_fmaf(-B * sx, ey, -0.5f * __builtin_fmaf(C * ey, ey, (A * sx) * sx));
    const float mx = fmaxf(fabsf(dxl), fabsf(dxh)), my = fmaxf(fabsf(dyl), fabsf(dyh));
    const float mag = __builtin_fmaf(A * mx, mx, __builtin_fmaf(C * my, my, 2.0f * fabsf(B) * mx * my));
    const float slack = __builtin_fmaf(4e-6f, mag, 1e-4f);
    const bool concave = A > 0.0f && C > 0.0f && A * C > B * B * 1.00001f;
    const bool miss = fmaxf(f1, f2) < tau - slack;
    return !(q.w < 1.0f / 255.0f || (concave && miss));
}

__device__ __forceinline__ float sigmoid_canonical(float x) { return 1.0f / (1.0f + exp_canonical(-x)); }

__device__ __forceinline__ void gsr_inverse3_f64(const double (&a)[3][3], double (&r)[3][3]) {
    const double c00 = a[1][1] * a[2][2] - a[1][2] * a[2][1], c01 = a[1][2] * a[2][0] - a[1][0] * a[2][2],
                 c02 = a[1][0] * a[2][1] - a[1][1] * a[2][0];
    const double det = (a[0][0] * c00 + a[0][1] * c01) + a[0][2] * c02;
    r[0][0] = c00 / det;
    r[0][1] = (a[0][2] * a[2][1] - a[0][1] * a[2][2]) / det;
    r[0][2] = (a[0][1] * a[1][2] - a[0][2] * a[1][1]) / det;
    r[1][0] = c01 / det;
    r[1][1] = (a[0][0] * a[2][2] - a[0][2] * a[2][0]) / det;
    r[1][2] = (a[0][2] * a[1][0] - a[0][0] * a[1][2]) / det;
    r[2][0] = c02 / det;
    r[2][1] = (a[0][1] * a[2][0] - a[0][0] * a[2][1]) / det;
    r[2][2] = (a[0][0] * a[1][1] - a[0][1] * a[1][0]) / det;
}
#endif

#define GSR_MAX_BATCH GSR_MAX_FRAMES_PER_LAUNCH
template <typename A>
struct GsrBatch {
    A f[GSR_MAX_BATCH];
    static_assert(sizeof(A) * GSR_MAX_BATCH <= 4096 - 128, "per-frame argument blocks must fit the 4 KiB kernarg segment");
};

struct GsrFrame {
    const GsrSettings *st;
    const GsrSettings *st_bin;
    const GsrInputs *in;
    const GsrOutputs *out;
    GeomState g;
    ImageState img;
    BinningState b;
    uint32_t cap32;
    bool pc;
    bool td;
};

struct GsrMapsArgs {
    const uint2 *ranges;
    const uint32_t *point_list;
    const float4 *splat;
    const GsrHeader *hdr;
    const float *labels;
    int16_t *out_label;
    float *out_depth;
    float depth_scale;
    int W, H, gx, gy;
    int super;
};

void gsr_set_error(const char *fmt, ...);
int gsr_check_launch(const char *what, bool debug, hipStream_t stream);

int gsr_launch_preprocess(int B, GsrFrame *fr, bool count_tiles, bool infer, hipStream_t stream);
int gsr_launch_bin_starts(const GsrSettings &st, const GeomState &g, const ImageState &img, uint32_t r_capacity,
                          bool debug, hipStream_t stream);
int gsr_launch_bin_scatter_and_sort(const GsrSettings &st, int32_t P, const GeomState &g, const BinningState &b,
                                    const ImageState &img, bool debug, hipStream_t stream);
int gsr_launch_compact_and_depth_sort(int32_t P, const GeomState &g, bool debug, hipStream_t stream);
int gsr_launch_sample_depth_sort(int B, const GsrFrame *fr, bool order_early, int num_quads, int super_shift,
                                 int coop_blocks, bool debug, hipStream_t stream);
bool gsr_band_supported(int gx);
int gsr_launch_gather_rects(int32_t P, const GeomState &g, bool debug, hipStream_t stream);
int gsr_launch_band_count(int B, const GsrFrame *fr, bool balanced, bool merge_starts, bool *starts_done, bool debug,
                          hipStream_t stream);
int gsr_launch_band_place(int B, const GsrFrame *fr, bool debug, hipStream_t stream);
bool gsr_chunk_supported(int gx, int gy);
int gsr_launch_chunk_count(const GsrSettings &st, int32_t P, const GeomState &g, bool debug, hipStream_t stream);
int gsr_launch_chunk_place(const GsrSettings &st, int32_t P, const GeomState &g, const BinningState &b,
                           const ImageState &img, bool debug, hipStream_t stream);
int gsr_launch_tile_starts(int B, const GsrFrame *fr, bool order_done, bool debug, hipStream_t stream);
int gsr_launch_tile_starts(const GsrSettings &st, const GeomState &g, const ImageState &img, uint32_t r_capacity,
                           bool order_done, bool debug, hipStream_t stream);
int gsr_launch_tile_offsets(int32_t P, const GeomState &g, uint32_t r_capacity, bool debug, hipStream_t stream);
int gsr_launch_emit_and_tile_sort(const GsrSettings &st, int32_t P, const GeomState &g, const BinningState &b,
                                  const ImageState &img, int64_t r_capacity, bool debug, hipStream_t stream);
bool gsr_render_wants_tile_order(const GsrSettings &st, int num_tiles);
const char *gsr_render_build_flags();
int gsr_render_split_blocks(const GsrSettings &st, int num_tiles);
bool gsr_render_uses_quad_order(const GsrSettings &st, int num_tiles);
int gsr_render_cus_per_xcd();
int gsr_render_coop_blocks(const GsrSettings &st, int num_tiles, int frames);
int gsr_launch_render(int B, const GsrFrame *fr, bool order_ready, bool split_ready, bool super_tiles, int coop_blocks,
                      hipStream_t stream);
int gsr_launch_maps(int B, const GsrMapsArgs *frames, bool debug, hipStream_t stream);
int gsr_launch_tile_count(const GsrSettings &st, int32_t P, const GeomState &g, const ImageState &img,
                          uint32_t r_capacity, bool debug, hipStream_t stream);
int gsr_launch_tile_place(const GsrSettings &st, int32_t P, const GeomState &g, const BinningState &b,
                          const ImageState &img, bool debug, hipStream_t stream);
int gsr_launch_rowscan(uint32_t *table, const uint32_t *n_ptr, int nb_stride, int chunk, int rows, uint32_t *totals,
                       bool debug, hipStream_t stream);
int gsr_radix_passes(int bits, int bits_per_pass);
int gsr_radix_sort_u32(uint32_t *key[2], uint32_t *val[2], const uint32_t *n_ptr, int64_t n_max, int bits,
                       int bits_per_pass, int start_side, uint32_t *table, uint32_t *totals, bool debug,
                       hipStream_t stream);

#ifdef __HIPCC__
__device__ __forceinline__ int gsr_lane() { return (int)(threadIdx.x & 63u); }
__device__ __forceinline__ int gsr_wave() { return (int)(threadIdx.x >> 6); }
__device__ __forceinline__ uint64_t gsr_lanemask_lt() { return (1ull << gsr_lane()) - 1ull; }

#ifndef GSR_DPP_SCAN
#define GSR_DPP_SCAN 1
#endif
__device__ __forceinline__ uint32_t gsr_wave_incl_scan(uint32_t v) {
#if GSR_DPP_SCAN
    int x = (int)v;
    x += __builtin_amdgcn_update_dpp(0, x, 0x111, 0xf, 0xf, true);
    x += __builtin_amdgcn_update_dpp(0, x, 0x112, 0xf, 0xf, true);
    x += __builtin_amdgcn_update_dpp(0, x, 0x114, 0xf, 0xf, true);
    x += __builtin_amdgcn_update_dpp(0, x, 0x118, 0xf, 0xf, true);
    x += __builtin_amdgcn_update_dpp(0, x, 0x142, 0xa, 0xf, false);
    x += __builtin_amdgcn_update_dpp(0, x, 0x143, 0xc, 0xf, false);
    return (uint32_t)x;
#else
    const int lane = gsr_lane();
#pragma unroll
    for (int o = 1; o < 64; o <<= 1) {
        const uint32_t t = __shfl_up(v, o, 64);
        if (lane >= o) v += t;
    }
    return v;
#endif
}

__device__ __forceinline__ uint32_t gsr_block_incl_scan(uint32_t v, uint32_t *s_w, uint32_t &total) {
    const uint32_t incl = gsr_wave_incl_scan(v);
    const int lane = gsr_lane(), wave = gsr_wave();
    if (lane == 63) s_w[wave] = incl;
    __syncthreads();
    const uint32_t w0 = s_w[0], w1 = s_w[1], w2 = s_w[2], w3 = s_w[3];
    uint32_t add = 0;
    if (wave > 0) add += w0;
    if (wave > 1) add += w1;
    if (wave > 2) add += w2;
    total = w0 + w1 + w2 + w3;
    __syncthreads();
    return incl + add;
}

#define GSR_XCDS 8
__device__ __forceinline__ void gsr_quad_order_block(const uint32_t *__restrict__ quad_work, int Q,
                                                     uint32_t *__restrict__ quad_order, uint32_t *s_w ,
                                                     int cus_per_xcd) {
    __shared__ uint32_t s_qb[GSR_XCDS * 256];
    __shared__ uint32_t s_xbase[GSR_XCDS];
    const int T = Q >> 2;
    uint32_t c[32], qmx = 0;
#pragma unroll
    for (int k = 0; k < 32; k++) {
        const int q = (int)threadIdx.x + k * GSR_BLOCK;
        c[k] = q < Q ? min(quad_work[q], (1u << 24) - 1u) : 0u;
        qmx = max(qmx, c[k]);
    }
#pragma unroll
    for (int o = 32; o > 0; o >>= 1) qmx = max(qmx, (uint32_t)__shfl_xor((int)qmx, o, 64));
    if ((threadIdx.x & 63u) == 0u) s_w[threadIdx.x >> 6] = qmx;
#pragma unroll
    for (int k = 0; k < GSR_XCDS; k++) s_qb[k * GSR_BLOCK + (int)threadIdx.x] = 0u;
    __syncthreads();
    qmx = max(max(s_w[0], s_w[1]), max(s_w[2], s_w[3]));
    const int sh = qmx >= (1u << 16) ? 8 : 0;
    const uint32_t div = (qmx >> sh) + 1u;
    const float inv = 256.0f / (float)div;
#pragma unroll
    for (int k = 0; k < 32; k++) {
        const int q = (int)threadIdx.x + k * GSR_BLOCK;
// ... 176 lines not shown
```

### gsworld_amd/csrc/render.hip

```cpp
#include "gsr_internal.h"

namespace {

constexpr int kDefaultBlocksPerCu = 6;
struct RenderChoice {
    int variant;
    int blocks_per_cu;
};
inline RenderChoice render_choice(const GsrSettings &st) {
    RenderChoice c;
    c.variant = st.render_variant == 0 ? 4 : (st.render_variant == 1 ? 0 : st.render_variant);
    c.blocks_per_cu = st.render_blocks_per_cu > 0 ? st.render_blocks_per_cu : kDefaultBlocksPerCu;
    return c;
}

__device__ __forceinline__ float fma_(float a, float b, float c) { return __builtin_fmaf(a, b, c); }

__global__ __launch_bounds__(GSR_BLOCK) void render_kernel(const uint2 *__restrict__ ranges,
                                                           const uint32_t *__restrict__ point_list,
                                                           const float4 *__restrict__ splat, int W, int H, int gx,
                                                           const float *__restrict__ bg,
                                                           float *__restrict__ out_color,
                                                           float *__restrict__ out_invdepth,
                                                           float *__restrict__ final_T,
// ... 325 lines not shown
        oma[2 * h] = d.x;
        oma[2 * h + 1] = d.y;
    }
    const uint64_t saved = __builtin_amdgcn_read_exec();
#pragma unroll
    for (int k = 0; k < kBatch; k++) {
        const v2f crg = {b.col[k].x, b.col[k].y}, cbd = {b.col[k].z, b.col[k].w};
        asm volatile(
            "v_cmpx_le_f32 0x3b808081, %[a]\n\t"
            "v_mul_f32 v95, %[T], %[oma]\n\t"
            "v_cmp_gt_f32 vcc, 0x38d1b717, v95\n\t"
            "v_mul_f32 v94, %[a], %[T]\n\t"
            "s_nop 0\n\t"
            "v_cndmask_b32_e64 v94, v94, 0, vcc\n\t"
            "v_cndmask_b32_e64 %[T], v95, -|%[T]|, vcc\n\t"
            "v_pk_fma_f32 %[rg], %[crg], v[94:95], %[rg] op_sel_hi:[1,0,1]\n\t"
            "v_pk_fma_f32 %[bd], %[cbd], v[94:95], %[bd] op_sel_hi:[1,0,1]\n\t"
            "s_mov_b64 exec, %[sv]"
            : [T] "+v"(T), [rg] "+v"(acc_rg), [bd] "+v"(acc_bd)
            : [a] "v"(b.araw[k]), [oma] "v"(oma[k]), [crg] "v"(crg), [cbd] "v"(cbd), [sv] "s"(saved)
            : "vcc", "v94", "v95");
    }
}

#define GSR_ALIVE_STEP(A, AO, CRG, CBD, NEXT)                                                                        \
    "v_cmpx_le_f32 0x3b808081, " A "\n\t"                                           \
    "v_pk_mul_f32 v[94:95], " AO ", v[92:93] op_sel_hi:[1,0]\n\t"                         \
    "v_cmp_gt_f32 vcc, 0x38d1b717, v95\n\t"                                         \
    "s_andn2_b64 %[alive], %[alive], vcc\n\t"                                                                         \
    "s_andn2_b64 exec, exec, vcc\n\t"                                                                                 \
    "v_mov_b32 v92, v95\n\t"                                                                                          \
    "v_pk_fma_f32 %[rg], " CRG ", v[94:95], %[rg] op_sel_hi:[1,0,1]\n\t"                                              \
    "v_pk_fma_f32 %[bd], " CBD ", v[94:95], %[bd] op_sel_hi:[1,0,1]\n\t"                                              \
    "s_mov_b64 exec, " NEXT "\n\t"
__device__ __forceinline__ void stream_blend_alive(const StreamBatch &b, v2f &Tp, v2f &acc_rg, v2f &acc_bd,
                                                   uint64_t &alive, int &limit, const uint64_t saved) {
    static_assert(kBatch == 4, "the block below takes four survivors");
    const v2f crg0 = {b.col[0].x, b.col[0].y}, cbd0 = {b.col[0].z, b.col[0].w};
    const v2f crg1 = {b.col[1].x, b.col[1].y}, cbd1 = {b.col[1].z, b.col[1].w};
    const v2f crg2 = {b.col[2].x, b.col[2].y}, cbd2 = {b.col[2].z, b.col[2].w};
    const v2f crg3 = {b.col[3].x, b.col[3].y}, cbd3 = {b.col[3].z, b.col[3].w};
    asm volatile("s_mov_b64 exec, %[alive]\n\t"
                 GSR_ALIVE_STEP("%[a0]", "%[ao0]", "%[crg0]", "%[cbd0]", "%[alive]")
                 GSR_ALIVE_STEP("%[a1]", "%[ao1]", "%[crg1]", "%[cbd1]", "%[alive]")
                 GSR_ALIVE_STEP("%[a2]", "%[ao2]", "%[crg2]", "%[cbd2]", "%[alive]")
                 GSR_ALIVE_STEP("%[a3]", "%[ao3]", "%[crg3]", "%[cbd3]", "%[sv]")
                 "s_cmp_eq_u64 %[alive], 0\n\t"
                 "s_cmov_b32 %[lim], 0"
                 : "+{v[92:93]}"(Tp), [rg] "+v"(acc_rg), [bd] "+v"(acc_bd), [alive] "+s"(alive), [lim] "+s"(limit)
                 : [a0] "v"(b.araw[0]), [ao0] "v"(b.ao[0]), [crg0] "v"(crg0), [cbd0] "v"(cbd0),
                   [a1] "v"(b.araw[1]), [ao1] "v"(b.ao[1]), [crg1] "v"(crg1), [cbd1] "v"(cbd1),
                   [a2] "v"(b.araw[2]), [ao2] "v"(b.ao[2]), [crg2] "v"(crg2), [cbd2] "v"(cbd2),
                   [a3] "v"(b.araw[3]), [ao3] "v"(b.ao[3]), [crg3] "v"(crg3), [cbd3] "v"(cbd3),
                   [sv] "s"(saved)
                 : "vcc", "scc", "v94", "v95");
}

__device__ __forceinline__ void stream_list_put(float4 (*list)[6], int rank, float4 geo, float4 conic_op, float4 rgbd,
                                                float pos) {
    float4 *pr = list[rank >> 1];
    float *f = reinterpret_cast<float *>(pr) + (rank & 1);
    f[0] = geo.x;
    f[2] = geo.y;
    f[4] = -0.5f * conic_op.x;
    f[6] = -0.5f * conic_op.z;
    f[8] = -conic_op.y;
    f[10] = conic_op.w;
    pr[3 + (rank & 1)] = rgbd;
    f[20] = pos;
}

constexpr int kCoopCullers = GSR_BLOCK / GSR_WAVE - 1;
#ifndef GSR_COOP_SPIN_LIMIT
#define GSR_COOP_SPIN_LIMIT (1u << 20)
#endif
constexpr uint32_t kCoopSpinLimit = GSR_COOP_SPIN_LIMIT;

struct CoopFlags {
    uint32_t ready[4], done[4], n_surv[4], unsafe_lo[4], unsafe_hi[4], stop;
};

__device__ __forceinline__ uint32_t coop_load(volatile uint32_t *p) { return *p; }

template <bool SUPER>
__device__ __forceinline__ bool render_coop_quadrant(float4 (*s_list)[kStreamList / 2][6], CoopFlags *fl, const uint32_t q,
                                                     const uint2 *__restrict__ ranges,
                                                     const uint32_t *__restrict__ point_list,
                                                     const float4 *__restrict__ splat, int W, int H, int gx,
                                                     const float *__restrict__ bg, float *__restrict__ out_color,
                                                     float *__restrict__ out_invdepth, uint8_t *__restrict__ rgb8,
                                                     uint32_t *__restrict__ quad_work, float *__restrict__ final_T) {
    static_assert(SUPER, "cooperative quadrants are an inference-frame path");
#if GSR_STREAM_STAMPS
    const uint64_t stamp0 = __builtin_readcyclecounter();
#endif
    const int lane = gsr_lane(), wave = gsr_wave();
    const int tile = (int)(q >> 2), quad = (int)(q & 3u);
    const int qx0 = (tile % gx) * GSR_TILE + ((quad & 1) << 3);
    const int qy0 = (tile / gx) * GSR_TILE + ((quad >> 1) << 3);
    const uint32_t tx = (uint32_t)(tile % gx), ty = (uint32_t)(tile / gx);
    constexpr int kSX = GSR_SUPER_SX, kSY = GSR_SUPER_SY;
    const uint2 range = ranges[(int)((ty >> kSY) * (uint32_t)((gx + (1 << kSX) - 1) >> kSX) + (tx >> kSX))];
    const int n_inst = (int)(range.y - range.x);
    const uint32_t *src = point_list + range.x;
    const int rounds = (n_inst + GSR_WAVE - 1) / GSR_WAVE;
    const float4 zero4 = make_float4(0.f, 0.f, 0.f, 0.f);
    volatile uint32_t *ready = fl->ready, *done = fl->done, *stop = &fl->stop;
    if (wave != 0) {
        const int c = wave - 1;
        float4(*list)[6] = s_list[wave];
        const float qxf = (float)qx0, qyf = (float)qy0;
        float4 f0 = zero4, f1 = zero4, f2 = zero4;
        uint32_t g_next = 0;
        {
            const int p = c * GSR_WAVE + lane;
            if (p < n_inst) {
                const float4 *rec = splat + 3 * (size_t)src[p];
                f0 = rec[0]; f1 = rec[1]; f2 = rec[2];
            }
            if (p + kCoopCullers * GSR_WAVE < n_inst) g_next = src[p + kCoopCullers * GSR_WAVE];
        }
        uint32_t produced = 0;
        for (int rd = c; rd < rounds; rd += kCoopCullers) {
            const int p = rd * GSR_WAVE + lane;
            bool keep = p < n_inst;
            {
                const uint32_t rb = __float_as_uint(f2.w);
                keep = keep && tx - (rb & 255u) < ((rb >> 16) & 255u) - (rb & 255u) &&
                       ty - ((rb >> 8) & 255u) < (rb >> 24) - ((rb >> 8) & 255u);
            }
            keep = keep && quadrant_may_hit<true>(f0.x, f0.y, f1, qxf, qyf, 7.0f, f0.z);
            const uint64_t unsafe = __builtin_amdgcn_ballot_w64(keep && (__float_as_uint(f0.z) & 1u) == 0u);
            const uint64_t mask = __builtin_amdgcn_ballot_w64(keep);
            const int rank = (int)__builtin_amdgcn_mbcnt_hi((uint32_t)(mask >> 32), __builtin_amdgcn_mbcnt_lo((uint32_t)mask, 0u));
            const int n_surv = (int)__builtin_popcountll(mask);
            while (coop_load(&done[wave]) != produced && coop_load(stop) == 0u) __builtin_amdgcn_s_sleep(1);
            if (coop_load(stop) != 0u) break;
            __builtin_amdgcn_fence(__ATOMIC_ACQUIRE, "workgroup");
            if (keep)
                stream_list_put(list, rank, f0, f1, make_float4(f2.x, f2.y, f2.z, f0.w), __uint_as_float((uint32_t)p + 1u));
            if (lane < kBatch) stream_list_put(list, n_surv + lane, zero4, zero4, zero4, 0.0f);
            if (lane == 0) {
                fl->n_surv[wave] = (uint32_t)n_surv;
                fl->unsafe_lo[wave] = (uint32_t)unsafe;
                fl->unsafe_hi[wave] = (uint32_t)(unsafe >> 32);
            }
            __builtin_amdgcn_fence(__ATOMIC_RELEASE, "workgroup");
            produced++;
            if (lane == 0) ready[wave] = produced;
            const int pn = (rd + kCoopCullers) * GSR_WAVE + lane;
            f0 = zero4; f1 = zero4; f2 = zero4;
            if (pn < n_inst) {
                const float4 *rec = splat + 3 * (size_t)g_next;
                f0 = rec[0]; f1 = rec[1]; f2 = rec[2];
            }
            if (pn + kCoopCullers * GSR_WAVE < n_inst) g_next = src[pn + kCoopCullers * GSR_WAVE];
        }
        return false;
    }
    const int px = qx0 + (lane & 7), py = qy0 + (lane >> 3);
    const bool inside = px < W && py < H;
    const float pfx = (float)px, pfy = (float)py;
    const v2f pf2x = {pfx, pfx}, pf2y = {pfy, pfy};
    const float bg0 = bg[0], bg1 = bg[1], bg2 = bg[2];
    float T = inside ? 1.0f : -1.0f;
    v2f acc_rg = {0.f, 0.f}, acc_bd = {0.f, 0.f};
    uint32_t work = 0;
    bool timed_out = false;
    for (int rd = 0; rd < rounds; rd++) {
        if (__builtin_amdgcn_ballot_w64(T > 0.0f) == 0ull) break;
        const int w = 1 + rd % kCoopCullers;
        const uint32_t want = (uint32_t)(rd / kCoopCullers) + 1u;
        uint32_t spin;
        asm volatile("v_mov_b32 %0, 0" : "=v"(spin));
        while (coop_load(&ready[w]) != want && spin < kCoopSpinLimit) {
            __builtin_amdgcn_s_sleep(1);
            spin++;
        }
        if (spin >= kCoopSpinLimit) {
            timed_out = true;
            break;
        }
        __builtin_amdgcn_fence(__ATOMIC_ACQUIRE, "workgroup");
        const int n_surv = (int)__builtin_amdgcn_readfirstlane((int)fl->n_surv[w]);
        const uint64_t unsafe = ((uint64_t)(uint32_t)__builtin_amdgcn_readfirstlane((int)fl->unsafe_hi[w]) << 32) |
                                (uint64_t)(uint32_t)__builtin_amdgcn_readfirstlane((int)fl->unsafe_lo[w]);
        const float4(*list)[6] = s_list[w];
        work += 8u;
#if GSR_STREAM_MASKED_BLEND && GSR_STREAM_ALIVE_BLEND
        if (unsafe == 0ull) {
            uint64_t alive = __builtin_amdgcn_ballot_w64(T > 0.0f);
            v2f Tp = {T, 0.0f};
            int i = 0;
            int limit = n_surv;
            const uint64_t full = __builtin_amdgcn_read_exec();
            if (n_surv > 0) do {
                const StreamBatch b = stream_eval<false, false>(list, i, pf2x, pf2y);
                stream_blend_alive(b, Tp, acc_rg, acc_bd, alive, limit, full);
                work += (uint32_t)kBatch;
                i += kBatch;
            } while (i < limit);
            asm volatile("v_cndmask_b32_e64 %0, -|%1|, %1, %2" : "=v"(T) : "v"(Tp.x), "s"(alive));
        } else
#endif
        if (unsafe == 0ull) {
            int i = 0;
            if (n_surv > 0) do {
                const StreamBatch b = stream_eval<false, false>(list, i, pf2x, pf2y);
#if GSR_STREAM_MASKED_BLEND
                stream_blend_masked(b, T, acc_rg, acc_bd);
#else
                uint32_t last = 0;
                stream_blend<false>(b, T, acc_rg, acc_bd, last);
#endif
                work += (uint32_t)kBatch;
                i += kBatch;
            } while (i < n_surv && __builtin_amdgcn_ballot_w64(T > 0.0f) != 0ull);
        } else {
            int i = 0;
            uint32_t last = 0;
            if (n_surv > 0) do {
                const StreamBatch b = stream_eval<true, false>(list, i, pf2x, pf2y);
                stream_blend<false>(b, T, acc_rg, acc_bd, last);
                work += (uint32_t)kBatch;
                i += kBatch;
            } while (i < n_surv && __builtin_amdgcn_ballot_w64(T > 0.0f) != 0ull);
        }
        __builtin_amdgcn_fence(__ATOMIC_RELEASE, "workgroup");
        if (lane == 0) done[w] = want;
    }
    if (lane == 0) *stop = 1u;
    if (quad_work != nullptr && lane == 0) quad_work[q] = work;
#if GSR_STREAM_STAMPS
    if (lane == 0) {
        const uint64_t stamp1 = __builtin_readcyclecounter();
        const uint32_t hw = (uint32_t)__builtin_amdgcn_s_getreg((31 << 11) | 4) & 0x0fffffffu;
        const uint32_t xcc = (uint32_t)__builtin_amdgcn_s_getreg((3 << 11) | 20);
        reinterpret_cast<uint4 *>(final_T)[q] = make_uint4((uint32_t)stamp0, (uint32_t)stamp1, hw | (xcc << 28), work);
    }
#endif
    if (inside) {
        const size_t pid = (size_t)py * W + px;
        const size_t plane = (size_t)H * W;
        T = fabsf(T);
        const float r = fma_(T, bg0, acc_rg.x), g = fma_(T, bg1, acc_rg.y), b = fma_(T, bg2, acc_bd.x);
        if (out_color != nullptr) {
            out_color[pid] = r;
            out_color[plane + pid] = g;
            out_color[2 * plane + pid] = b;
            out_invdepth[pid] = acc_bd.y;
        }
        if (rgb8) {
            uint8_t *o = rgb8 + 3 * pid;
            o[0] = (uint8_t)fminf(fmaxf(r * 255.0f, 0.0f), 255.0f);
            o[1] = (uint8_t)fminf(fmaxf(g * 255.0f, 0.0f), 255.0f);
            o[2] = (uint8_t)fminf(fmaxf(b * 255.0f, 0.0f), 255.0f);
        }
    }
    return timed_out;
}

template <bool SUPER>
__device__ __forceinline__ void render_stream_body(const uint2 *__restrict__ ranges,
                                                                  const uint32_t *__restrict__ point_list,
                                                                  const float4 *__restrict__ splat, int W, int H, int gx,
                                                                  int num_tiles, const uint32_t *__restrict__ tile_order,
                                                                  const float *__restrict__ bg,
                                                                  float *__restrict__ out_color,
                                                                  float *__restrict__ out_invdepth,
                                                                  float *__restrict__ final_T,
                                                                  uint32_t *__restrict__ n_contrib,
                                                                  uint8_t *__restrict__ rgb8 ,
                                                                  uint32_t *__restrict__ quad_work ,
                                                                  int num_cus, int main_blocks,
                                                                  const uint32_t *__restrict__ split_flag,
                                                                  const uint32_t *__restrict__ split_list,
                                                                  const uint32_t *__restrict__ split_count,
                                                                  uint32_t *__restrict__ quad_work_b,
                                                                  const uint32_t *__restrict__ quad_order,
                                                                  const uint32_t *__restrict__ coop_list,
                                                                  int coop_blocks, GsrHeader *__restrict__ hdr,
                                                                  const uint32_t wgx ,
                                                                  const uint32_t *__restrict__ tile_dirty = nullptr) {
    __shared__ float4 s_list[GSR_BLOCK / GSR_WAVE][kStreamList / 2][6];
    const int lane = gsr_lane(), wave = gsr_wave();
    const uint32_t *dirty = nullptr;
    uint32_t td_token = 0u;
    if constexpr (SUPER) {
        if (tile_dirty != nullptr && hdr->td_reuse != 0u) {
            dirty = tile_dirty;
            td_token = hdr->td_token;
        }
    }
    if constexpr (SUPER) {
        if (coop_list != nullptr && (int)wgx < coop_blocks) {
            __shared__ CoopFlags s_coop;
            if (threadIdx.x < sizeof(CoopFlags) / sizeof(uint32_t)) reinterpret_cast<uint32_t *>(&s_coop)[threadIdx.x] = 0u;
            __syncthreads();
            const uint32_t q = coop_list[wgx];
            if (q >= 4u * (uint32_t)num_tiles) return;
            if (dirty != nullptr && dirty[q >> 2] != td_token) {
                if (threadIdx.x == 0) hdr->td_skipped = 1u;
                return;
            }
            const bool timed_out = render_coop_quadrant<true>(s_list, &s_coop, q, ranges, point_list, splat, W, H, gx, bg,
                                                              out_color, out_invdepth, rgb8, quad_work, final_T);
            if (timed_out && lane == 0) gsr_note_coop_timeout(hdr);
            return;
        }
    }
    float4(*list)[6] = s_list[wave];
    const float bg0 = bg[0], bg1 = bg[1], bg2 = bg[2];
    const float4 zero4 = make_float4(0.f, 0.f, 0.f, 0.f);
    const uint32_t num_tickets = 4u * (uint32_t)num_tiles;
    const uint32_t bx = wgx - (uint32_t)coop_blocks;
    const bool extra = (int)bx >= main_blocks;
    uint32_t extra_q = 0;
    if (extra) {
        const uint32_t e = (bx - (uint32_t)main_blocks) * (uint32_t)(GSR_BLOCK / GSR_WAVE) + (uint32_t)wave;
        if (split_count == nullptr || e >= *split_count) return;
        extra_q = split_list[e];
    }
    const uint32_t ticket_stride = (uint32_t)main_blocks * (uint32_t)(GSR_BLOCK / GSR_WAVE);
    const uint32_t wave_global = bx * (uint32_t)(GSR_BLOCK / GSR_WAVE) + (uint32_t)wave;
    for (uint32_t pass = 0, ticket = extra ? 0u : wave_global; ticket < num_tickets;
         pass++, ticket = extra ? num_tickets
                                : pass * ticket_stride + ((pass & 1u) ? ticket_stride - 1u - wave_global : wave_global)) {
        uint32_t unit = ticket >> 2;
        if (!extra && tile_order != nullptr && quad_order == nullptr && main_blocks >= num_tiles) {
            const uint32_t group = unit / (uint32_t)num_cus, idx = unit - group * (uint32_t)num_cus;
            const uint32_t size = min((uint32_t)num_cus, (uint32_t)num_tiles - group * (uint32_t)num_cus);
            unit = group * (uint32_t)num_cus + ((group & 1u) ? size - 1u - idx : idx);
        }
        int tile = extra ? (int)(extra_q >> 2) : (tile_order ? (int)tile_order[unit] : (int)unit);
        int quad = extra ? (int)(extra_q & 3u) : (int)(ticket & 3u);
        if (!extra && quad_order != nullptr && main_blocks >= num_tiles) {
            const uint32_t q = quad_order[4u * unit + (ticket & 3u)];
            if (SUPER && (q & 0x80000000u) != 0u) continue;
            tile = (int)(q >> 2);
            quad = (int)(q & 3u);
        }
        if (dirty != nullptr && dirty[tile] != td_token) {
            if (lane == 0) hdr->td_skipped = 1u;
            continue;
        }
        const int half = extra ? 2 : ((split_flag != nullptr && split_flag[4 * tile + quad] != 0u) ? 1 : 0);
        const int qx0 = (tile % gx) * GSR_TILE + ((quad & 1) << 3);
        const int qy0 = (tile / gx) * GSR_TILE + ((quad >> 1) << 3) + (half == 2 ? 4 : 0);
        const int px = qx0 + (lane & 7), py = qy0 + (lane >> 3);
        const bool inside = px < W && py < H && (half == 0 || lane < 32);
        const float pfx = (float)px, pfy = (float)py;
        const float qxf = (float)qx0, qyf = (float)qy0;
        const float yext = half == 0 ? 7.0f : 3.0f;
        const uint32_t tx = (uint32_t)(tile % gx), ty = (uint32_t)(tile / gx);
        constexpr int kSX = GSR_SUPER_SX, kSY = GSR_SUPER_SY;
        const uint2 range = ranges[SUPER ? (int)((ty >> kSY) * (uint32_t)((gx + (1 << kSX) - 1) >> kSX) + (tx >> kSX)) : tile];
        const int n_inst = (int)(range.y - range.x);
        const uint32_t *src = point_list + range.x;

#if GSR_STREAM_STAMPS
        const uint64_t stamp0 = __builtin_readcyclecounter();
#endif
        const v2f pf2x = {pfx, pfx}, pf2y = {pfy, pfy};
        float T = inside ? 1.0f : -1.0f;
        v2f acc_rg = {0.f, 0.f}, acc_bd = {0.f, 0.f};
        uint32_t last_contributor = 0;

        float4 f0[kStreamLanesItems], f1[kStreamLanesItems], f2[kStreamLanesItems];
        uint32_t g_next[kStreamLanesItems];
#pragma unroll
        for (int s = 0; s < kStreamLanesItems; s++) {
            const int p = s * GSR_WAVE + lane;
            f0[s] = zero4; f1[s] = zero4; f2[s] = zero4;
            g_next[s] = 0;
            if (p < n_inst) {
                const float4 *rec = splat + 3 * (size_t)src[p];
                f0[s] = rec[0]; f1[s] = rec[1]; f2[s] = rec[2];
            }
            if (p + kStreamRound < n_inst) g_next[s] = src[p + kStreamRound];
        }
        const int rounds = (n_inst + kStreamRound - 1) / kStreamRound;
        uint32_t work = 0;
        for (int rd = 0; rd < rounds; rd++) {
            if (__builtin_amdgcn_ballot_w64(T > 0.0f) == 0ull) break;
            int n_surv = 0;
            uint64_t unsafe = 0ull;
#pragma unroll
            for (int s = 0; s < kStreamLanesItems; s++) {
                const int p = rd * kStreamRound + s * GSR_WAVE + lane;
                bool keep = p < n_inst;
                if (SUPER) {
                    const uint32_t rb = __float_as_uint(f2[s].w);
                    keep = keep && tx - (rb & 255u) < ((rb >> 16) & 255u) - (rb & 255u) &&
                           ty - ((rb >> 8) & 255u) < (rb >> 24) - ((rb >> 8) & 255u);
                }
                if (SUPER) {
                    keep = keep && quadrant_may_hit<true>(f0[s].x, f0[s].y, f1[s], qxf, qyf, yext, f0[s].z);
                    unsafe |= __builtin_amdgcn_ballot_w64(keep && (__float_as_uint(f0[s].z) & 1u) == 0u);
                } else {
                    keep = keep && quadrant_may_hit(f0[s].x, f0[s].y, f1[s], qxf, qyf, yext);
                    unsafe |= __builtin_amdgcn_ballot_w64(keep && !stream_conic_is_safe(f1[s]));
                }
                const uint64_t mask = __builtin_amdgcn_ballot_w64(keep);
                const int rank = n_surv + (int)__builtin_amdgcn_mbcnt_hi((uint32_t)(mask >> 32),
                                                                         __builtin_amdgcn_mbcnt_lo((uint32_t)mask, 0u));
                if (keep)
                    stream_list_put(list, rank, f0[s], f1[s], make_float4(f2[s].x, f2[s].y, f2[s].z, f0[s].w),
                                    __uint_as_float((uint32_t)p + 1u));
                n_surv += (int)__builtin_popcountll(mask);
            }
            work += 8u;
            if (lane < kBatch)
                stream_list_put(list, n_surv + lane, zero4, zero4, zero4, 0.0f);
#pragma unroll
            for (int s = 0; s < kStreamLanesItems; s++) {
                const int p = (rd + 1) * kStreamRound + s * GSR_WAVE + lane;
                f0[s] = zero4; f1[s] = zero4; f2[s] = zero4;
                if (p < n_inst) {
                    const float4 *rec = splat + 3 * (size_t)g_next[s];
                    f0[s] = rec[0]; f1[s] = rec[1]; f2[s] = rec[2];
                }
                if (p + kStreamRound < n_inst) g_next[s] = src[p + kStreamRound];
            }
            __builtin_amdgcn_wave_barrier();
#if GSR_STREAM_MASKED_BLEND && GSR_STREAM_ALIVE_BLEND
            if (SUPER && unsafe == 0ull) {
                uint64_t alive = __builtin_amdgcn_ballot_w64(T > 0.0f);
                v2f Tp = {T, 0.0f};
                int i = 0;
                int limit = n_surv;
                const uint64_t full = __builtin_amdgcn_read_exec();
                if (n_surv > 0) do {
                    const StreamBatch b = stream_eval<false, false>(list, i, pf2x, pf2y);
                    stream_blend_alive(b, Tp, acc_rg, acc_bd, alive, limit, full);
                    work += (uint32_t)kBatch;
                    i += kBatch;
                } while (i < limit);
                asm volatile("v_cndmask_b32_e64 %0, -|%1|, %1, %2" : "=v"(T) : "v"(Tp.x), "s"(alive));
            } else
#endif
            if (unsafe == 0ull) {
                int i = 0;
                if (n_surv > 0) do {
                    const StreamBatch b = stream_eval<false, !SUPER>(list, i, pf2x, pf2y);
#if GSR_STREAM_MASKED_BLEND
                    if (SUPER)
                        stream_blend_masked(b, T, acc_rg, acc_bd);
                    else
#endif
                    stream_blend<!SUPER>(b, T, acc_rg, acc_bd, last_contributor);
                    work += (uint32_t)kBatch;
                    i += kBatch;
                } while (i < n_surv && __builtin_amdgcn_ballot_w64(T > 0.0f) != 0ull);
            } else {
                int i = 0;
                if (n_surv > 0) do {
                    const StreamBatch b = stream_eval<true, !SUPER>(list, i, pf2x, pf2y);
                    stream_blend<!SUPER>(b, T, acc_rg, acc_bd, last_contributor);
                    work += (uint32_t)kBatch;
                    i += kBatch;
                } while (i < n_surv && __builtin_amdgcn_ballot_w64(T > 0.0f) != 0ull);
            }
            __builtin_amdgcn_wave_barrier();
        }
        if (quad_work != nullptr && lane == 0) (half == 2 ? quad_work_b : quad_work)[4 * tile + quad] = work;
#if GSR_STREAM_STAMPS
        if (SUPER && lane == 0) {
            const uint64_t stamp1 = __builtin_readcyclecounter();
            const uint32_t hw = (uint32_t)__builtin_amdgcn_s_getreg((31 << 11) | 4) & 0x0fffffffu;
            const uint32_t xcc = (uint32_t)__builtin_amdgcn_s_getreg((3 << 11) | 20);
            reinterpret_cast<uint4 *>(final_T)[4 * tile + quad] =
                make_uint4((uint32_t)stamp0, (uint32_t)stamp1, hw | (xcc << 28), work);
        }
#endif
        if (inside) {
            const size_t pid = (size_t)py * W + px;
            const size_t plane = (size_t)H * W;
            T = fabsf(T);
            if (!SUPER) {
                final_T[pid] = T;
                n_contrib[pid] = last_contributor;
            }
            const float r = fma_(T, bg0, acc_rg.x), g = fma_(T, bg1, acc_rg.y), b = fma_(T, bg2, acc_bd.x);
            if (out_color != nullptr) {
                out_color[pid] = r;
                out_color[plane + pid] = g;
                out_color[2 * plane + pid] = b;
                out_invdepth[pid] = acc_bd.y;
            }
            if (rgb8) {
                uint8_t *o = rgb8 + 3 * pid;
                o[0] = (uint8_t)fminf(fmaxf(r * 255.0f, 0.0f), 255.0f);
                o[1] = (uint8_t)fminf(fmaxf(g * 255.0f, 0.0f), 255.0f);
                o[2] = (uint8_t)fminf(fmaxf(b * 255.0f, 0.0f), 255.0f);
            }
        }
    }
}

struct RenderStreamArgs {
    const uint2 *ranges;
    const uint32_t *point_list;
    const float4 *splat;
    int W, H, gx, num_tiles;
    const uint32_t *tile_order;
    const float *bg;
    float *out_color, *out_invdepth, *final_T;
    uint32_t *n_contrib;
    uint8_t *rgb8;
    uint32_t *quad_work;
    int num_cus, main_blocks, total_blocks;
    const uint32_t *split_flag, *split_list, *split_count;
    uint32_t *quad_work_b;
    const uint32_t *quad_order;
    const uint32_t *coop_list;
    int coop_blocks;
    GsrHeader *hdr;
    int frames;
    const uint32_t *tile_dirty;
};
template <bool SUPER>
__global__ __launch_bounds__(GSR_BLOCK) __attribute__((amdgpu_waves_per_eu(5))) void render_stream_kernel(
    const GsrBatch<RenderStreamArgs> bt) {
    const uint32_t frames = gridDim.y == 1u ? (uint32_t)bt.f[0].frames : 1u;
    const uint32_t grp = blockIdx.x >> 3;
    const uint32_t frame = gridDim.y == 1u ? grp % frames : blockIdx.y;
    const uint32_t wgx = gridDim.y == 1u ? (grp / frames) * 8u + (blockIdx.x & 7u) : blockIdx.x;
    const RenderStreamArgs &a = bt.f[frame];
    if ((int)wgx >= a.total_blocks) return;
    render_stream_body<SUPER>(a.ranges, a.point_list, a.splat, a.W, a.H, a.gx, a.num_tiles, a.tile_order, a.bg,
                              a.out_color, a.out_invdepth, a.final_T, a.n_contrib, a.rgb8, a.quad_work, a.num_cus,
                              a.main_blocks, a.split_flag, a.split_list, a.split_count, a.quad_work_b, a.quad_order,
                              a.coop_list, a.coop_blocks, a.hdr, wgx, a.tile_dirty);
}

__global__ __launch_bounds__(GSR_BLOCK) void tile_order_kernel(const uint2 *__restrict__ ranges, int num_tiles,
                                                               uint32_t *__restrict__ order) {
    __shared__ uint32_t s_bins[64];
    __shared__ uint32_t s_red[4];
    gsr_tile_order_block(ranges, num_tiles, order, s_bins, s_red);
}

__global__ __launch_bounds__(GSR_BLOCK) void pack_rgb8_kernel(const float *__restrict__ color, int n_pix,
                                                              uint8_t *__restrict__ out) {
    const int q = blockIdx.x * GSR_BLOCK + (int)threadIdx.x;
    const int p0 = q * 4;
    if (p0 >= n_pix) return;
    uint8_t v[12];
#pragma unroll
    for (int k = 0; k < 4; k++) {
        const int p = p0 + k;
#pragma unroll
        for (int c = 0; c < 3; c++) {
            float x = p < n_pix ? color[(size_t)c * n_pix + p] : 0.f;
            x = fminf(fmaxf(x * 255.0f, 0.0f), 255.0f);
            v[3 * k + c] = (uint8_t)x;
        }
    }
    if (p0 + 3 < n_pix) {
        uint32_t *o = reinterpret_cast<uint32_t *>(out + (size_t)p0 * 3);
        o[0] = v[0] | (v[1] << 8) | (v[2] << 16) | ((uint32_t)v[3] << 24);
        o[1] = v[4] | (v[5] << 8) | (v[6] << 16) | ((uint32_t)v[7] << 24);
        o[2] = v[8] | (v[9] << 8) | (v[10] << 16) | ((uint32_t)v[11] << 24);
    } else {
        for (int k = 0; k < 12 && p0 * 3 + k < n_pix * 3; k++) out[(size_t)p0 * 3 + k] = v[k];
    }
}

}

extern "C" int gsr_pack_rgb8(const float *color, int32_t width, int32_t height, uint8_t *out, void *stream) {
    if (!color || !out || width <= 0 || height <= 0 || (reinterpret_cast<uintptr_t>(out) & 3u)) {
        gsr_set_error("gsr_pack_rgb8: null / unaligned pointer or empty image");
        return GSR_E_INVALID;
    }
    const int n_pix = width * height;
    hipLaunchKernelGGL(pack_rgb8_kernel, dim3(gsr_div_up(gsr_div_up(n_pix, 4), GSR_BLOCK)), dim3(GSR_BLOCK), 0,
                       (hipStream_t)stream, color, n_pix, out);
    return gsr_check_launch("pack_rgb8", false, (hipStream_t)stream);
}

static int render_num_cus() {
    static int num_cus = 0;
    if (num_cus == 0) {
        int dev = 0;
        hipDeviceProp_t prop;
        if (hipGetDevice(&dev) == hipSuccess && hipGetDeviceProperties(&prop, dev) == hipSuccess &&
            prop.multiProcessorCount > 0)
            num_cus = prop.multiProcessorCount;
        else
            num_cus = 256;
    }
    return num_cus;
}

const char *gsr_render_build_flags() {
#if GSR_STREAM_MASKED_BLEND && GSR_STREAM_ALIVE_BLEND
    return "alive_blend=1";
#else
    return "alive_blend=0";
#endif
}

int gsr_render_cus_per_xcd() { return render_num_cus() / GSR_XCDS > 0 ? render_num_cus() / GSR_XCDS : 1; }

int gsr_render_split_blocks(const GsrSettings &st, int num_tiles) {
    const RenderChoice c = render_choice(st);
    if (c.variant != 4 || st.render_split != 1) return 0;
    const int resident = render_num_cus() * c.blocks_per_cu;
    return num_tiles < resident ? resident - num_tiles : 0;
}

bool gsr_render_uses_quad_order(const GsrSettings &st, int num_tiles) {
    const RenderChoice c = render_choice(st);
    return c.variant == 4 && num_tiles <= 2048 && num_tiles <= render_num_cus() * c.blocks_per_cu;
}

bool gsr_render_wants_tile_order(const GsrSettings &st, int num_tiles) {
    const RenderChoice c = render_choice(st);
    return c.variant == 4 || (c.variant >= 2 && num_tiles > render_num_cus() * c.blocks_per_cu);
}

int gsr_render_coop_blocks(const GsrSettings &st, int num_tiles, int frames) {
    const RenderChoice c = render_choice(st);
    if (c.variant != 4 || st.render_split == 1 || st.render_split == 3) return 0;
    if (st.render_split != 2 && frames > GSR_COOP_MAX_FRAMES) return 0;
    if (!gsr_render_uses_quad_order(st, num_tiles)) return 0;
    const int spare = render_num_cus() * 5 - num_tiles;
    const int blocks = (spare < GSR_COOP_MAX_BLOCKS ? spare : GSR_COOP_MAX_BLOCKS) / GSR_XCDS * GSR_XCDS;
    return blocks > 0 ? blocks : 0;
}

int gsr_launch_render(int B, const GsrFrame *fr, bool order_ready, bool split_ready, bool super_tiles, int coop_blocks,
                      hipStream_t stream) {
    const GsrSettings &st = *fr[0].st;
    const int W = st.image_width, H = st.image_height;
    const int gx = gsr_div_up(W, GSR_TILE), gy = gsr_div_up(H, GSR_TILE);
    const RenderChoice rc = render_choice(st);
    if (B > 1 && rc.variant != 4) {
        gsr_set_error("gsr_launch_render: only the default compositor takes several frames per launch");
        return GSR_E_INVALID;
    }
    const GeomState &g = fr[0].g;
    const ImageState &img = fr[0].img;
    const uint32_t *point_list = fr[0].b.gidx[0];
    const float *background = fr[0].in->background;
    float *out_color = fr[0].out->out_color, *out_invdepth = fr[0].out->out_invdepth;
    uint8_t *out_rgb8 = fr[0].out->out_rgb8;
    const bool pack_after = out_rgb8 != nullptr && rc.variant != 4;
    if (rc.variant >= 2) {
        const int T = gx * gy;
        const bool ordered = gsr_render_wants_tile_order(st, T);
        const uint32_t *order = ordered ? img.tile_order : nullptr;
        if (ordered && !order_ready)
            for (int k = 0; k < B; k++)
                hipLaunchKernelGGL(tile_order_kernel, dim3(1), dim3(GSR_BLOCK), 0, stream, fr[k].img.ranges, T,
                                   fr[k].img.tile_order);
        const int blocks = min(T, render_num_cus() * rc.blocks_per_cu);
        if (rc.variant == 4) {
            const int coop = super_tiles && split_ready ? coop_blocks : 0;
            const int extra = coop > 0 ? coop : (split_ready && T <= 2048 ? gsr_render_split_blocks(st, T) : 0);
            const bool use_qorder = split_ready && gsr_render_uses_quad_order(st, T);
            GsrBatch<RenderStreamArgs> bt{};
            for (int k = 0; k < B; k++) {
                const ImageState &im = fr[k].img;
                RenderStreamArgs &a = bt.f[k];
                a.ranges = im.ranges;
                a.point_list = fr[k].b.gidx[0];
                a.splat = fr[k].g.splat;
                a.W = W; a.H = H; a.gx = gx; a.num_tiles = T;
                a.tile_order = ordered ? im.tile_order : (const uint32_t *)nullptr;
                a.bg = fr[k].in->background;
                a.out_color = fr[k].out->out_color;
                a.out_invdepth = fr[k].out->out_invdepth;
                a.final_T = im.final_T;
                a.n_contrib = im.n_contrib;
                a.rgb8 = fr[k].out->out_rgb8;
                a.quad_work = im.quad_work;
                a.num_cus = render_num_cus();
                a.main_blocks = blocks;
                a.total_blocks = blocks + extra;
                a.split_flag = extra > 0 && coop == 0 ? im.split_flag : (const uint32_t *)nullptr;
                a.coop_list = coop > 0 ? im.split_list : (const uint32_t *)nullptr;
                a.coop_blocks = coop;
                a.hdr = fr[k].g.hdr;
                a.frames = B;
                a.split_list = im.split_list;
                a.split_count = im.split_count;
                a.quad_work_b = im.quad_work_b;
                a.quad_order = use_qorder ? im.quad_order : (const uint32_t *)nullptr;
                a.tile_dirty = (fr[k].pc && fr[k].td) ? im.tile_dirty : (const uint32_t *)nullptr;
            }
            const int row = B > 1 ? (blocks + extra + GSR_XCDS - 1) / GSR_XCDS * GSR_XCDS : blocks + extra;
#ifndef GSR_RENDER_INTERLEAVE
#define GSR_RENDER_INTERLEAVE 0
#endif
            const dim3 grid = (GSR_RENDER_INTERLEAVE && B > 1) ? dim3(row * B, 1) : dim3(row, B > 1 ? B : 1);
            if (B == 1) bt.f[0].frames = 1;
            if (super_tiles)
                hipLaunchKernelGGL(render_stream_kernel<true>, grid, dim3(GSR_BLOCK), 0, stream, bt);
            else
                hipLaunchKernelGGL(render_stream_kernel<false>, grid, dim3(GSR_BLOCK), 0, stream, bt);
        }
        else if (rc.variant == 3)
            hipLaunchKernelGGL(render_queue_kernel<true>, dim3(blocks), dim3(GSR_BLOCK), 0, stream, img.ranges,
                               point_list, g.splat, W, H, gx, T, order, background, out_color, out_invdepth,
                               img.final_T, img.n_contrib);
        else
            hipLaunchKernelGGL(render_queue_kernel<false>, dim3(blocks), dim3(GSR_BLOCK), 0, stream, img.ranges,
                               point_list, g.splat, W, H, gx, T, order, background, out_color, out_invdepth,
                               img.final_T, img.n_contrib);
    } else {
        hipLaunchKernelGGL(render_kernel, dim3(gx * gy), dim3(GSR_BLOCK), 0, stream, img.ranges, point_list, g.splat,
                           W, H, gx, background, out_color, out_invdepth, img.final_T, img.n_contrib);
    }
    if (pack_after) {
        const int n_pix = W * H;
        hipLaunchKernelGGL(pack_rgb8_kernel, dim3(gsr_div_up(gsr_div_up(n_pix, 4), GSR_BLOCK)), dim3(GSR_BLOCK), 0,
                           stream, out_color, n_pix, out_rgb8);
    }
    return GSR_OK;
}
```

### gsworld_amd/csrc/sort.hip

```cpp
#include "gsr_internal.h"

namespace {

__global__ __launch_bounds__(GSR_BLOCK) void scan_small_kernel(uint32_t *data, int n_static,
                                                               const uint32_t *n_items_ptr, int chunk,
                                                               GsrHeader *hdr, int mode, uint32_t r_capacity) {
    __shared__ uint32_t s_w[4];
    int n = n_static;
    if (n_items_ptr) n = (int)((*n_items_ptr + (uint32_t)chunk - 1u) / (uint32_t)chunk);
    const int per = (n + GSR_BLOCK - 1) / GSR_BLOCK;
    const int lo = min(n, (int)threadIdx.x * per), hi = min(n, lo + per);
    uint32_t mine = 0;
    for (int i = lo; i < hi; i++) mine += data[i];
    uint32_t carry;
    uint32_t run = gsr_block_incl_scan(mine, s_w, carry) - mine;
    for (int i = lo; i < hi; i++) {
        const uint32_t v = data[i];
        data[i] = run;
        run += v;
    }
    if (threadIdx.x == 0) {
        data[n] = carry;
        if (mode == 1) {
            hdr->R_raw = carry;
            hdr->r_capacity = r_capacity;
            gsr_set_overflow(hdr, carry > r_capacity);
            hdr->R = carry > r_capacity ? 0u : carry;
        }
    }
}

__global__ __launch_bounds__(GSR_BLOCK) void compact_kernel(int P, const uint32_t *__restrict__ tiles_touched,
                                                            const float4 *__restrict__ splat,
                                                            const uint32_t *__restrict__ block_counts,
                                                            uint2 *__restrict__ pairs,
                                                            GsrHeader *__restrict__ hdr) {
    __shared__ uint32_t s_w[4];
    uint32_t part = 0;
    for (int j = (int)threadIdx.x; j < (int)blockIdx.x; j += GSR_BLOCK) part += block_counts[j];
    uint32_t offset;
    (void)gsr_block_incl_scan(part, s_w, offset);
    const int i = blockIdx.x * GSR_BLOCK + (int)threadIdx.x;
    const bool vis = i < P && tiles_touched[i] != 0u;
    uint32_t total;
    const uint32_t incl = gsr_block_incl_scan(vis ? 1u : 0u, s_w, total);
    if (vis) {
        const uint32_t pos = offset + incl - 1u;
        pairs[pos] = make_uint2(__float_as_uint(splat[3 * (size_t)i].z), (uint32_t)i);
    }
    if (blockIdx.x == gridDim.x - 1 && threadIdx.x == 0) {
        hdr->V = offset + total;
        hdr->R = 0u;
        hdr->overflow = 0u;
        hdr->coop_timeout_now = 0u;
        hdr->r_capacity = 0u;
        hdr->R_raw = 0u;
        hdr->tile_queue = 0u;
    }
}

template <int BITS, bool PAIRED>
__global__ __launch_bounds__(GSR_BLOCK) void radix_hist_kernel(const uint32_t *__restrict__ keys,
                                                               const uint32_t *__restrict__ n_ptr,
                                                               uint32_t *__restrict__ table, int nb_stride, int shift,
                                                               uint32_t mask) {
    constexpr int BINS = 1 << BITS;
    const uint32_t n = *n_ptr;
    const uint32_t base = blockIdx.x * (uint32_t)GSR_SORT_CHUNK;
    if (base >= n) return;
    __shared__ uint32_t s_h[BINS];
    for (int i = (int)threadIdx.x; i < BINS; i += GSR_BLOCK) s_h[i] = 0u;
    __syncthreads();
#pragma unroll
    for (int r = 0; r < GSR_SORT_ITEMS; r++) {
        const uint32_t i = base + (uint32_t)r * GSR_BLOCK + threadIdx.x;
        if (i < n) atomicAdd(&s_h[(keys[PAIRED ? 2u * i : i] >> shift) & mask], 1u);
    }
    __syncthreads();
    for (int d = (int)threadIdx.x; d < BINS; d += GSR_BLOCK) table[(size_t)d * nb_stride + blockIdx.x] = s_h[d];
}

__global__ __launch_bounds__(GSR_BLOCK) void radix_rowscan_kernel(uint32_t *__restrict__ table,
                                                                  const uint32_t *__restrict__ n_ptr, int nb_stride,
                                                                  uint32_t *__restrict__ totals, int chunk) {
    __shared__ uint32_t s_w[4];
    const uint32_t n = *n_ptr;
    const int nb = (int)((n + (uint32_t)chunk - 1u) / (uint32_t)chunk);
    uint32_t *row = table + (size_t)blockIdx.x * nb_stride;
    uint32_t carry = 0;
    for (int base = 0; base < nb; base += GSR_BLOCK) {
        const int i = base + (int)threadIdx.x;
        const uint32_t v = i < nb ? row[i] : 0u;
        uint32_t total;
        const uint32_t incl = gsr_block_incl_scan(v, s_w, total);
        if (i < nb) row[i] = carry + incl - v;
        carry += total;
    }
    if (threadIdx.x == 0) totals[blockIdx.x] = carry;
}

template <int BITS, bool PAIRED, bool LAST>
__global__ __launch_bounds__(GSR_BLOCK) void radix_scatter_kernel(
    const uint32_t *__restrict__ keys_in, const uint32_t *__restrict__ vals_in, uint32_t *__restrict__ keys_out,
    uint32_t *__restrict__ vals_out, const uint32_t *__restrict__ n_ptr, const uint32_t *__restrict__ table,
    const uint32_t *__restrict__ totals, int nb_stride, int shift, uint32_t mask, int nbits) {
    constexpr int BINS = 1 << BITS;
    constexpr int PER = BINS / GSR_BLOCK;
    constexpr int WAVE_ITEMS = GSR_SORT_CHUNK / 4;
    const uint32_t n = *n_ptr;
    const uint32_t base = blockIdx.x * (uint32_t)GSR_SORT_CHUNK;
    if (base >= n) return;
    __shared__ uint32_t s_cur[4][BINS];
    __shared__ uint32_t s_w[4];
    const int tid = (int)threadIdx.x, wave = gsr_wave(), lane = gsr_lane();
    const uint64_t lt = gsr_lanemask_lt();
    for (int i = tid; i < 4 * BINS; i += GSR_BLOCK) (&s_cur[0][0])[i] = 0u;
    __syncthreads();
    const uint32_t wbase = base + (uint32_t)wave * WAVE_ITEMS;
    constexpr int ROUNDS = WAVE_ITEMS / 64;
    uint32_t rkey[ROUNDS], rval[ROUNDS];
#pragma unroll
    for (int r = 0; r < ROUNDS; r++) {
        const uint32_t i = wbase + (uint32_t)r * 64u + (uint32_t)lane;
        if (PAIRED) {
            const uint2 kv = i < n ? reinterpret_cast<const uint2 *>(keys_in)[i] : make_uint2(0u, 0u);
            rkey[r] = kv.x;
            rval[r] = kv.y;
        } else {
            rkey[r] = i < n ? keys_in[i] : 0u;
            rval[r] = i < n ? vals_in[i] : 0u;
        }
    }
#pragma unroll
    for (int r = 0; r < ROUNDS; r++) {
        const uint32_t i = wbase + (uint32_t)r * 64u + (uint32_t)lane;
        if (i < n) atomicAdd(&s_cur[wave][(rkey[r] >> shift) & mask], 1u);
    }
// ... 172 lines not shown
```

### gsworld_amd/debug.py

```python
from __future__ import annotations

import ctypes as C

import torch

from . import _lib
from ._lib import GsrStateView, check, lib


def set_binning_mode(mode: int) -> None:
    if mode not in (0, 1, 2, 3, 4):
        raise ValueError("binning mode must be 0, 1, 2, 3 or 4")
    _lib.TUNING["binning_path"] = {1: 0, 0: 1, 2: 2, 3: 3, 4: 4}[mode]


def set_depth_sort(variant: int) -> None:
    if variant not in (0, 1):
        raise ValueError("depth sort variant must be 0 or 1")
    _lib.TUNING["depth_sort"] = variant


def set_render_split(on) -> None:
    mode = int(on)
    if mode not in (0, 1, 2, 3):
        raise ValueError("render_split must be 0 (default), 1 (halves), 2 (cooperative always) or 3 (neither)")
    _lib.TUNING["render_split"] = mode


def set_render_variant(variant: int, blocks_per_cu: int = 0) -> None:
    if variant not in (0, 2, 3, 4) or not 0 <= blocks_per_cu <= 8:
        raise ValueError("variant must be 0, 2, 3 or 4; blocks_per_cu 0..8")
    _lib.TUNING["render_variant"] = {4: 0, 0: 1, 2: 2, 3: 3}[variant]
    if blocks_per_cu > 0:
        _lib.TUNING["render_blocks_per_cu"] = blocks_per_cu


def _view(buf: torch.Tensor, ptr, count: int, dtype: torch.dtype) -> torch.Tensor:
    off = int(ptr) - buf.data_ptr()
    nbytes = count * torch.empty((), dtype=dtype).element_size()
    assert 0 <= off and off + nbytes <= buf.numel(), "state view outside its buffer"
    return buf[off:off + nbytes].view(dtype)


def state_view(P: int, width: int, height: int, num_rendered: int, num_visible: int, geomBuffer: torch.Tensor,
               binningBuffer: torch.Tensor | None, imgBuffer: torch.Tensor | None, r_capacity: int | None = None):
    v = GsrStateView()
    cap = num_rendered if r_capacity is None else r_capacity
    check(lib().gsr_state_view(P, width, height, C.c_int64(cap), C.c_void_p(geomBuffer.data_ptr()),
                               C.c_void_p(binningBuffer.data_ptr()) if binningBuffer is not None else None,
                               C.c_void_p(imgBuffer.data_ptr()) if imgBuffer is not None else None, C.byref(v)))
    gx, gy = (width + 15) // 16, (height + 15) // 16
    out = {}
    splat = _view(geomBuffer, v.splat, 12 * P, torch.float32).view(P, 12)
    out["splat"] = splat
    out["means2D"] = splat[:, 0:2]
    out["depths"] = splat[:, 2]
    out["invdepths"] = splat[:, 3]
    out["conic_opacity"] = splat[:, 4:8]
    out["rgb"] = splat[:, 8:11]
    out["cov3D"] = _view(geomBuffer, v.cov3D, 6 * P, torch.float32).view(P, 6)
    out["clamped"] = _view(geomBuffer, v.clamped, 4 * P, torch.uint8).view(P, 4)[:, :3]
    out["tiles_touched"] = _view(geomBuffer, v.tiles_touched, P, torch.int32)
    out["rects"] = _view(geomBuffer, v.rects, 4 * P, torch.int16).view(P, 4)
    if v.depth_order and _lib.TUNING["binning_path"] != 2:
        out["depth_order"] = _view(geomBuffer, v.depth_order, max(num_visible, 0), torch.int32)
    if binningBuffer is not None and num_rendered > 0:
        out["point_list"] = _view(binningBuffer, v.point_list, num_rendered, torch.int32)
    if imgBuffer is not None and "point_list" in out:
        r = _view(imgBuffer, v.ranges, 2 * gx * gy, torch.int32).view(gx * gy, 2).to(torch.int64)
        tiles = torch.zeros(num_rendered, dtype=torch.int64, device=r.device)
        nonempty = r[:, 1] > r[:, 0]
        tiles[r[nonempty, 0]] = torch.nonzero(nonempty).squeeze(1)
        out["point_tiles"] = torch.cummax(tiles, 0).values.to(torch.int32)
    if imgBuffer is not None:
        out["ranges"] = _view(imgBuffer, v.ranges, 2 * gx * gy, torch.int32).view(gx * gy, 2)
        out["final_T"] = _view(imgBuffer, v.final_T, width * height, torch.float32).view(height, width)
        out["n_contrib"] = _view(imgBuffer, v.n_contrib, width * height, torch.int32).view(height, width)
    return out


def sort_state(geomBuffer: torch.Tensor) -> dict:
    out = (C.c_int32 * 8)()
    with torch.cuda.device(geomBuffer.device):
        check(lib().gsr_debug_sort_state(C.c_void_p(geomBuffer.data_ptr()), out,
                                         C.c_void_p(torch.cuda.current_stream(geomBuffer.device).cuda_stream)))
    return dict(blind=bool(out[0]), fresh=bool(out[1]), bad=bool(out[2]), trust=int(out[3]), buckets=int(out[4]),
                stride=int(out[5]), coop_quads=int(out[6]), near=bool(out[7] & 1), kept_blocks=bool(out[7] & 2), kept_tiles=bool(out[7] & 4))
```

### include/gsr.h

```cpp
#ifndef GSR_H
#define GSR_H

#include <stddef.h>
#include <stdint.h>

#ifdef __cplusplus
extern "C" {
#endif

#define GSR_OK 0
#define GSR_E_INVALID (-1)
#define GSR_E_HIP (-2)
#define GSR_E_ALLOC (-3)
#define GSR_E_OVERFLOW (-4)
#define GSR_E_TRUNCATED (-5)

#define GSR_TILE 16
#define GSR_NEAR_PLANE 0.05f

typedef struct GsrSettings {
    int32_t image_height;
    int32_t image_width;
    float tanfovx;
    float tanfovy;
// ... 15 lines not shown
typedef struct GsrInputs {
    int32_t P;
    const float *background;
    const float *means3D;
    const float *shs;
    const float *colors_precomp;
    const float *opacities;
    const float *scales;
    const float *rotations;
    const float *cov3D_precomp;
    const float *viewmatrix;
    const float *projmatrix;
    const float *campos;
    const float *shs_rest;
    int32_t param_space;
    const float *part_labels;
    const int32_t *part_lut;
    int32_t part_lut_size;
    const float *part_transforms;
    int32_t part_count;
    const uint8_t *part_rescale;
    const float *cull_blocks;
    const int32_t *orig_index;
    const float *appearance;
    const int32_t *appearance_lut;
    int32_t appearance_lut_size;
    int32_t appearance_groups;
    const uint32_t *appearance_versions;
    const float *appearance_labels;
} GsrInputs;
#define GSR_APPEARANCE_MAX_GROUPS 64

#define GSR_RAW_OPACITY 1
#define GSR_RAW_SCALES 2
#define GSR_RAW_ROTATIONS 4
#define GSR_MODEL_VERSION(v) ((int32_t)(((uint32_t)(v) & 0xFFFFFFu) << 8))
#define GSR_FRAME_KEPT 8

typedef struct GsrOutputs {
    float *out_color;
    float *out_invdepth;
    int32_t *radii;
    uint8_t *out_rgb8;
    uint32_t *overflow_mirror;
} GsrOutputs;

typedef char *(*gsr_resize_fn)(void *user, size_t bytes);

typedef struct GsrBuffers {
    gsr_resize_fn geom_resize;    void *geom_user;
    gsr_resize_fn binning_resize; void *binning_user;
    gsr_resize_fn image_resize;   void *image_user;
} GsrBuffers;

typedef struct GsrFrameStats {
    int64_t num_visible;
    int64_t num_rendered;
    int32_t overflow;
    int32_t overflow_frames;
    int32_t truncated;
    int32_t coop_timeouts;
} GsrFrameStats;

const char *gsr_last_error(void);
const char *gsr_version(void);
void gsr_abi_sizes(int32_t out[6]);

size_t gsr_geom_bytes(int32_t P, int32_t width, int32_t height);
size_t gsr_binning_bytes(int64_t r_capacity);
size_t gsr_image_bytes(int32_t width, int32_t height);

int gsr_forward(const GsrSettings *settings, const GsrInputs *in, const GsrOutputs *out,
                const GsrBuffers *buffers, int64_t r_capacity, GsrFrameStats *stats, void *stream);

#define GSR_MAX_FRAMES_PER_LAUNCH 8
int gsr_forward_batch(int32_t B, const GsrSettings *settings, const GsrInputs *in, const GsrOutputs *out,
                      const GsrBuffers *buffers, const int64_t *r_capacity, void *stream);

int gsr_plan_query(const GsrSettings *settings, int32_t P, int32_t permuted, int64_t r_capacity, int32_t out[8]);

int gsr_debug_ss_stamps(int32_t P, int32_t width, int32_t height, const void *geom, uint64_t *out64);

int gsr_debug_sort_state(const void *geom, int32_t out[8], void *stream);

int gsr_frame_stats(const void *geom, GsrFrameStats *stats, void *stream);

typedef struct GsrStateView {
    const float *splat;
    const float *cov3D;
    const uint8_t *clamped;
    const uint32_t *tiles_touched;
    const uint16_t *rects;
    const uint32_t *depth_order;
    const uint32_t *point_list;
    const uint32_t *point_tiles;
    const uint32_t *ranges;
    const float *final_T;
    const uint32_t *n_contrib;
} GsrStateView;
int gsr_state_view(int32_t P, int32_t width, int32_t height, int64_t r_capacity_or_R, const void *geom,
                   const void *binning, const void *image, GsrStateView *view);

typedef struct GsrMapFrame {
    int32_t struct_size;
    const GsrSettings *settings;
    int32_t P; int32_t permuted;
    int64_t r_capacity;
    const void *geom, *binning, *image;
    const float *labels;
    float depth_scale;
    int16_t *out_label;
    float *out_depth;
} GsrMapFrame;
int gsr_render_maps(int32_t B, const GsrMapFrame *frames, void *stream);

#define GSR_PROFILE_STAGES 5
typedef struct GsrProfile {
    int32_t frames;
    double stage_ms[GSR_PROFILE_STAGES];
} GsrProfile;
int gsr_profile_enable(int mode);
int gsr_profile_collect(GsrProfile *out);

typedef struct GsrBackwardInputs {
    const float *dL_dout_color;
    const float *dL_dout_invdepth;
    const int32_t *radii;
    int64_t num_rendered;
    const void *geom, *binning, *image;
} GsrBackwardInputs;

typedef struct GsrGrads {
    float *dL_dmeans2D;
    float *dL_dcolors;
    float *dL_dopacity;
    float *dL_dmeans3D;
    float *dL_dcov3D;
    float *dL_dsh;
    float *dL_dscales;
    float *dL_drots;
    float *dL_dconic;
    float *dL_dinvdepths;
    float *dL_dsh_rest;
} GsrGrads;

int gsr_backward(const GsrSettings *settings, const GsrInputs *in, const GsrBackwardInputs *bw,
                 const GsrGrads *grads, void *stream);

size_t gsr_knn_workspace_bytes(int32_t P);
int gsr_knn_dist2(int32_t P, const float *points, float *mean_dist2, void *workspace, size_t workspace_bytes,
                  void *stream);

int gsr_ssim_forward(int32_t B, int32_t CH, int32_t H, int32_t W, float C1, float C2, const float *img1,
                     const float *img2, int32_t train, float *ssim_map, float *dm_dmu1, float *dm_dsigma1_sq,
                     float *dm_dsigma12, void *stream);
int gsr_ssim_backward(int32_t B, int32_t CH, int32_t H, int32_t W, float C1, float C2, const float *img1,
                      const float *img2, const float *dL_dmap, const float *dm_dmu1, const float *dm_dsigma1_sq,
                      const float *dm_dsigma12, float *dL_dimg1, void *stream);

size_t gsr_photometric_loss_scratch_floats(int32_t planes, int32_t H, int32_t W);
int gsr_photometric_loss(int32_t planes, int32_t H, int32_t W, const float *img, const float *target,
                         float lambda_dssim, int32_t clamp01, float *scratch, float *loss, int32_t keep_for_backward,
                         void *stream);
int gsr_photometric_loss_backward(int32_t planes, int32_t H, int32_t W, const float *img, const float *target,
                                  float lambda_dssim, int32_t clamp01, const float *scratch, const float *grad_loss,
                                  float *dL_dimg, void *stream);
// ... 77 lines not shown
```

Measured before the change: 14420.

## Limit per-tile placed lists to predicted contributors with render-time repair pass

Adds a list-limit mode for batched inference frames. Band placement stops writing point-list entries for a tile once a predicted per-tile limit is reached, and the renderer records tiles whose truncated list ran out before saturation. A repair placement pass and a second render pass then complete only those tiles, and debug/state-view paths rebuild full lists on demand. The goal is to cut placement and list-write work for Gaussians hidden behind saturated pixels, at the cost of extra launches, header state and more complex correctness invariants.

```diff
diff --git a/gsworld_amd/_lib.py b/gsworld_amd/_lib.py
--- a/gsworld_amd/_lib.py
+++ b/gsworld_amd/_lib.py
@@ -193,6 +193,10 @@
     L.gsr_frame_stats.argtypes = [C.c_void_p, C.POINTER(GsrFrameStats), C.c_void_p]
     L.gsr_debug_sort_state.argtypes = [C.c_void_p, C.POINTER(C.c_int32), C.c_void_p]
     L.gsr_debug_sort_state.restype = C.c_int
+    L.gsr_debug_set_list_limit.argtypes = [C.c_int32]
+    L.gsr_debug_set_list_limit.restype = C.c_int
+    L.gsr_debug_list_limit_state.argtypes = [C.c_void_p, C.POINTER(C.c_int32), C.c_void_p]
+    L.gsr_debug_list_limit_state.restype = C.c_int
     L.gsr_state_view.restype = C.c_int
     L.gsr_state_view.argtypes = [C.c_int32, C.c_int32, C.c_int32, C.c_int64, C.c_void_p, C.c_void_p, C.c_void_p,
                                  C.POINTER(GsrStateView)]
diff --git a/gsworld_amd/csrc/api.hip b/gsworld_amd/csrc/api.hip
--- a/gsworld_amd/csrc/api.hip
+++ b/gsworld_amd/csrc/api.hip
@@ -2,12 +2,18 @@
 #include <stdio.h>
 #include <string.h>
 
+#include <atomic>
 #include <vector>
 
 #include "gsr_internal.h"
 
 namespace {
 thread_local char g_err[512] = "";
+std::atomic<int> g_list_limit{0};
+std::atomic<bool> g_ll_issued{false};
+#ifndef GSR_LIST_LIMIT_MIN_FRAMES
+#define GSR_LIST_LIMIT_MIN_FRAMES 3
+#endif
 
 constexpr int kStages = GSR_PROFILE_STAGES;
 constexpr int kMaxFrames = 4096;
@@ -28,6 +34,8 @@
     if (g_prof.mode != 0 && g_prof.frames < kMaxFrames) g_prof.frames++;
 }
 }
+
+int gsr_list_limit_mode() { return g_list_limit.load(std::memory_order_relaxed); }
 
 void gsr_set_error(const char *fmt, ...) {
     va_list ap;
@@ -243,7 +251,15 @@
                (in[k].appearance == nullptr || in[k].appearance_versions != nullptr);
         f.td = GSR_TILE_REUSE && f.pc && super && (in[k].param_space & GSR_FRAME_KEPT) != 0 && out[k].out_rgb8 != nullptr &&
                out[k].out_color == nullptr && out[k].out_invdepth == nullptr;
-    }
+        f.ll = 0;
+    }
+    const int ll_mode = gsr_list_limit_mode();
+    bool ll = GSR_LIST_LIMIT && ll_mode >= 0 && infer && super && band && mode == 1 && !p.radix_depth && !exact &&
+              p.order_early && B >= (ll_mode > 0 ? 1 : GSR_LIST_LIMIT_MIN_FRAMES);
+    if (ll && ll_mode == 0)
+        for (int k = 0; k < B; k++) ll = ll && !fr[k].td && in[k].part_labels == nullptr;
+    for (int k = 0; k < B; k++) fr[k].ll = ll ? (ll_mode >= 64 ? ll_mode : 1) : 0;
+    if (ll) g_ll_issued.store(true, std::memory_order_relaxed);
     const GeomState &g = fr[0].g;
     const ImageState &img = fr[0].img;
 
@@ -279,8 +295,11 @@
     } else if (band) {
         bool starts_done = false;
         if (int e = gsr_launch_band_count(B, fr, !p.radix_depth, p.order_early, &starts_done, debug, stream)) return e;
-        if (!starts_done)
+        if (!starts_done) {
             if (int e = gsr_launch_tile_starts(B, fr, p.order_early, debug, stream)) return e;
+            ll = false;
+            for (int k = 0; k < B; k++) fr[k].ll = 0;
+        }
     } else if (mode == 1) {
         if (int e = gsr_launch_tile_count(st[0], in[0].P, g, img, fr[0].cap32, debug, stream)) return e;
     } else {
@@ -333,9 +352,38 @@
     }
     prof_mark(4, stream);
     if (int e = gsr_launch_render(B, fr, mode != 0, mode == 1, super, coop, stream)) return e;
+    if (ll) {
+        if (int e = gsr_launch_band_place(B, fr, debug, stream, 1)) return e;
+        if (int e = gsr_launch_render(B, fr, mode != 0, mode == 1, super, 0, stream, true)) return e;
+    }
     prof_mark(5, stream);
     prof_end_frame();
     return gsr_check_launch("render", debug, stream);
+}
+
+int complete_lists(int n, const Plan *plans, const int32_t *P, void *const *geom, void *const *binning, void *const *image,
+                   bool debug, hipStream_t stream) {
+    GsrFrame fr[GSR_MAX_BATCH];
+    GsrInputs in[GSR_MAX_BATCH];
+    for (int k = 0; k < n; k++) {
+        const Plan &p = plans[k];
+        memset(&in[k], 0, sizeof(in[k]));
+        in[k].P = P[k];
+        GsrFrame &f = fr[k];
+        f.st = f.st_bin = &p.st_bin;
+        f.in = &in[k];
+        f.out = nullptr;
+        f.g = GeomState::carve((char *)geom[k], P[k], p.tiles, nullptr, p.tiles_x, p.lean);
+        f.img = ImageState::carve((char *)image[k], p.W, p.H);
+        f.b = BinningState::carve((char *)binning[k], 1, nullptr, true);
+        f.cap32 = 0u;
+        f.pc = f.td = false;
+        f.ll = 1;
+    }
+    return gsr_launch_band_place(n, fr, debug, stream, 2);
+}
+bool plan_may_limit(const Plan &p) {
+    return GSR_LIST_LIMIT && g_ll_issued.load(std::memory_order_relaxed) && p.infer && p.super && p.band && p.mode == 1 && !p.radix_depth && !p.exact && p.order_early;
 }
 
 int zero_outputs(const GsrSettings *st, const GsrOutputs *out, hipStream_t stream) {
@@ -437,6 +485,15 @@
     std::vector<GsrMapsArgs> jobs;
     jobs.reserve((size_t)B);
     bool debug = false;
+    Plan c_plan[GSR_MAX_BATCH];
+    int32_t c_P[GSR_MAX_BATCH];
+    void *c_geom[GSR_MAX_BATCH], *c_bin[GSR_MAX_BATCH], *c_img[GSR_MAX_BATCH];
+    int c_n = 0;
+    auto flush = [&]() {
+        const int n = c_n;
+        c_n = 0;
+        return n > 0 ? complete_lists(n, c_plan, c_P, c_geom, c_bin, c_img, debug, stream) : GSR_OK;
+    };
     for (int k = 0; k < B; k++) {
         const GsrMapFrame &f = frames[k];
         if (f.struct_size != (int32_t)sizeof(GsrMapFrame)) {
@@ -479,6 +536,16 @@
             continue;
         }
         if (!f.out_label && !f.out_depth) continue;
+        if (plan_may_limit(p)) {
+            if (c_n == GSR_MAX_BATCH || (c_n > 0 && (c_P[0] != f.P || c_plan[0].W != p.W || c_plan[0].H != p.H)))
+                if (int e = flush()) return e;
+            c_plan[c_n] = p;
+            c_P[c_n] = f.P;
+            c_geom[c_n] = (void *)f.geom;
+            c_bin[c_n] = (void *)f.binning;
+            c_img[c_n] = (void *)f.image;
+            c_n++;
+        }
         const GeomState g = GeomState::carve((char *)f.geom, f.P, p.tiles);
         const BinningState b = BinningState::carve((char *)f.binning, 1);
         const ImageState s = ImageState::carve((char *)f.image, p.W, p.H);
@@ -498,6 +565,7 @@
         a.super = p.super ? 1 : 0;
         jobs.push_back(a);
     }
+    if (int e = flush()) return e;
     if (jobs.empty()) return GSR_OK;
     return gsr_launch_maps((int)jobs.size(), jobs.data(), debug, stream);
 }
@@ -585,6 +653,38 @@
     return GSR_OK;
 }
 
+int gsr_debug_set_list_limit(int32_t mode) {
+    if (mode < -1 || (mode > 1 && (mode % 64) != 0)) {
+        gsr_set_error("gsr_debug_set_list_limit: mode must be -1 (off), 0 (default), 1 (any launch) or a positive multiple of 64");
+        return GSR_E_INVALID;
+    }
+    g_list_limit.store(mode, std::memory_order_relaxed);
+    return GSR_OK;
+}
+int gsr_debug_list_limit_state(const void *geom, int32_t out[8], void *stream_) {
+    if (!geom || !out) {
+        gsr_set_error("gsr_debug_list_limit_state: null argument");
+        return GSR_E_INVALID;
+    }
+    hipStream_t stream = (hipStream_t)stream_;
+    GsrHeader h;
+    if (hipMemcpyAsync(&h, geom, sizeof(h), hipMemcpyDeviceToHost, stream) != hipSuccess ||
+        hipStreamSynchronize(stream) != hipSuccess) {
+        gsr_set_error("gsr_debug_list_limit_state: read-back failed: %s", hipGetErrorString(hipGetLastError()));
+        return GSR_E_HIP;
+    }
+    const bool on = h.ll_engaged != 0u;
+    out[0] = on ? 1 : 0;
+    out[1] = on ? (int32_t)h.ll_miss : 0;
+    out[2] = on ? (int32_t)h.ll_repaired : 0;
+    out[3] = on ? (int32_t)h.ll_placed : (int32_t)h.R;
+    out[4] = (int32_t)h.R;
+    out[5] = on ? (int32_t)h.ll_held : 0;
+    out[6] = on && h.ll_magic == GSR_LL_MAGIC ? 1 : 0;
+    out[7] = 0;
+    return GSR_OK;
+}
+
 int gsr_frame_stats(const void *geom, GsrFrameStats *stats, void *stream_) {
     if (!geom || !stats) {
         gsr_set_error("gsr_frame_stats: null argument");
@@ -613,6 +713,33 @@
         return GSR_E_INVALID;
     }
     memset(v, 0, sizeof(*v));
+    if (GSR_LIST_LIMIT && g_ll_issued.load(std::memory_order_relaxed) && geom && binning && image && P > 0 && width > 0 &&
+        height > 0) {
+        GsrHeader h;
+        if (hipDeviceSynchronize() != hipSuccess || hipMemcpy(&h, geom, sizeof(h), hipMemcpyDeviceToHost) != hipSuccess) {
+            gsr_set_error("gsr_state_view: header read-back failed: %s", hipGetErrorString(hipGetLastError()));
+            return GSR_E_HIP;
+        }
+        if (h.ll_engaged != 0u) {
+            GsrSettings st;
+            memset(&st, 0, sizeof(st));
+            st.image_width = width;
+            st.image_height = height;
+            st.forward_only = 1;
+            GsrInputs in;
+            memset(&in, 0, sizeof(in));
+            in.P = P;
+            Plan p;
+            if (make_plan(&st, &in, 1, p) == GSR_OK && plan_may_limit(p)) {
+                void *gp = (void *)geom, *bp = (void *)binning, *ip = (void *)image;
+                if (int e = complete_lists(1, &p, &P, &gp, &bp, &ip, false, (hipStream_t)0)) return e;
+                if (hipDeviceSynchronize() != hipSuccess) {
+                    gsr_set_error("gsr_state_view: completing the lists failed: %s", hipGetErrorString(hipGetLastError()));
+                    return GSR_E_HIP;
+                }
+            }
+        }
+    }
     if (geom) {
         const GeomState g = GeomState::carve((char *)geom, P, gsr_div_up(width, GSR_TILE) * gsr_div_up(height, GSR_TILE));
         v->splat = reinterpret_cast<const float *>(g.splat);
diff --git a/gsworld_amd/csrc/bandplace.hip b/gsworld_amd/csrc/bandplace.hip
--- a/gsworld_amd/csrc/bandplace.hip
+++ b/gsworld_amd/csrc/bandplace.hip
@@ -11,6 +11,7 @@
 constexpr int kRing = 128;
 constexpr uint32_t kSplit2 = 1024u, kSplit4 = 2048u;
 constexpr int kMaxSegments = 4;
+constexpr uint32_t kLLGuardMin = 8u, kLLGuardDiv = 16u;
 
 constexpr uint32_t kCutsMagic = 0x43555453u;
 
@@ -318,7 +319,8 @@
 constexpr int kPlaceBatch = 6;
 
 template <int NC>
-__device__ __forceinline__ void band_place_body(const uint32_t seg, const uint2 *__restrict__ rect_sorted,
+__device__ __forceinline__ void band_place_body(const uint32_t r, const uint32_t y, const uint32_t seg,
+                                                         const uint2 *__restrict__ rect_sorted,
                                                          const uint32_t *__restrict__ order,
                                                          const GsrHeader *__restrict__ hdr,
                                                          const uint32_t *__restrict__ wave_lo, int gx, int NR,
@@ -326,12 +328,19 @@
                                                          const uint32_t *__restrict__ wtable,
                                                          const uint2 *__restrict__ ranges,
                                                          uint32_t *__restrict__ point_list,
-                                                         const uint32_t *__restrict__ nseg_tab) {
+                                                         const uint32_t *__restrict__ nseg_tab,
+                                                         const int mode, const uint32_t ll_sig,
+                                                         const uint32_t *__restrict__ ll_limit,
+                                                         const uint32_t *__restrict__ ll_miss) {
+    if (GSR_LIST_LIMIT && mode != 0) {
+        if (hdr->ll_engaged != (ll_sig | 1u)) return;
+        if (mode == 1 && hdr->ll_miss == 0u) return;
+    }
+    const bool filter = GSR_LIST_LIMIT && ((mode == 0 && ll_limit != nullptr) || mode == 1);
     __shared__ uint2 s_ring[kBW][kRing];
     __shared__ unsigned long long s_mask[kBW][NC * 64];
     __shared__ uint32_t s_cur[kBW][NC * 64];
     const int lane = gsr_lane(), wave = gsr_wave();
-    const uint32_t r = blockIdx.x, y = blockIdx.y;
     const uint32_t nseg = (nseg_tab[(size_t)y * (uint32_t)NR + r] >> (8u * (uint32_t)__builtin_amdgcn_readfirstlane(wave))) & 255u;
     if (seg >= nseg) return;
     if (hdr->overflow) return;
@@ -371,6 +380,13 @@
             x1 = last;
         }
     }
+    uint32_t thr[NC];
+    uint64_t nd[NC], nd_any = 0ull;
+#pragma unroll
+    for (int k = 0; k < NC; k++) {
+        thr[k] = 0u;
+        nd[k] = ~0ull;
+    }
 #pragma unroll
     for (int k = 0; k < NC; k++) {
         const int x = k * 64 + lane;
@@ -381,7 +397,18 @@
             for (int w = 0; w < wave; w++) s += wbase[w * (NC * 64) + x];
         }
         cur[x] = s;
-    }
+        if (filter) {
+            uint32_t t = 0u;
+            if (x < gx) {
+                const size_t tile = (size_t)y * gx + x;
+                t = mode == 1 ? (ll_miss[tile] != 0u ? 0xFFFFFFFFu : 0u) : ranges[tile].x + ll_limit[tile];
+            }
+            thr[k] = ((uint32_t)x >= x0 && (uint32_t)x < x1) ? t : 0u;
+            nd[k] = __builtin_amdgcn_ballot_w64(s < thr[k]);
+            nd_any |= nd[k];
+        }
+    }
+    if (filter && nd_any == 0ull) return;
     __builtin_amdgcn_wave_barrier();
     uint32_t head = 0, tail = 0;
     for (uint32_t base = lo; base < hi; base += (uint32_t)(kPlaceBatch * GSR_WAVE)) {
@@ -397,7 +424,21 @@
         for (int u = 0; u < kPlaceBatch; u++) {
             const uint32_t miny = rc[u].x >> 16, maxy = rc[u].y >> 16;
             const uint32_t minx = max(rc[u].x & 0xffffu, x0), maxx = min(rc[u].y & 0xffffu, x1);
-            const bool keep = miny <= y && y < maxy && minx < maxx;
+            bool keep = miny <= y && y < maxy && minx < maxx;
+            if (filter) {
+                bool open = false;
+                if (NC == 1 && gx < 32) {
+                    open = __builtin_amdgcn_ubfe((uint32_t)nd[0], minx, maxx - minx) != 0u;
+                } else {
+#pragma unroll
+                    for (int k = 0; k < NC; k++) {
+                        const uint32_t lo_ = max(minx, (uint32_t)(64 * k)), hi_ = min(maxx, (uint32_t)(64 * k + 64));
+                        if (hi_ > lo_)
+                            open = open || ((nd[k] >> ((lo_ - (uint32_t)(64 * k)) & 63u)) << ((64u - (hi_ - lo_)) & 63u)) != 0ull;
+                    }
+                }
+                keep = keep && open;
+            }
             const uint64_t mask = __builtin_amdgcn_ballot_w64(keep);
             if (mask == 0ull) continue;
             if (keep) {
@@ -412,6 +453,15 @@
                 __builtin_amdgcn_wave_barrier();
                 band_place_round<NC>(p.x, p.y, true, gx, cur, colmask, point_list);
                 head += (uint32_t)GSR_WAVE;
+                if (filter && mode == 0) {
+                    uint64_t any = 0ull;
+#pragma unroll
+                    for (int k = 0; k < NC; k++) {
+                        nd[k] = __builtin_amdgcn_ballot_w64(cur[k * 64 + lane] < thr[k]);
+                        any |= nd[k];
+                    }
+                    if (any == 0ull) return;
+                }
             }
         }
     }
@@ -440,6 +490,10 @@
     const uint32_t *quad_work;
     uint32_t *tile_order;
     uint32_t *mirror;
+    uint32_t *ll_walked, *ll_limit, *ll_miss;
+    uint32_t ll_forced;
+    uint32_t ll_td;
+    int mode;
 };
 
 template <int NC>
@@ -459,8 +513,22 @@
 template <int NC>
 __global__ __launch_bounds__(kBT, 8) void band_place_kernel(const GsrBatch<BandArgs> bt) {
     const BandArgs &a = bt.f[blockIdx.z / (uint32_t)kMaxSegments];
-    band_place_body<NC>(blockIdx.z % (uint32_t)kMaxSegments, a.rect_sorted, a.order, a.hdr, a.wave_lo, a.gx, a.NR, a.table,
-                        a.wtable, a.ranges, a.point_list, a.nseg);
+    band_place_body<NC>(blockIdx.x, blockIdx.y, blockIdx.z % (uint32_t)kMaxSegments, a.rect_sorted, a.order, a.hdr, a.wave_lo, a.gx, a.NR, a.table,
+                        a.wtable, a.ranges, a.point_list, a.nseg, a.mode, a.sig ^ ((uint32_t)a.T << 8) ^ (uint32_t)a.gx,
+                        a.ll_limit, a.ll_miss);
+}
+constexpr int kRepairBlocks = 512;
+template <int NC>
+__global__ __launch_bounds__(kBT, 8) void band_place_repair_kernel(const GsrBatch<BandArgs> bt) {
+    const BandArgs &a = bt.f[blockIdx.y];
+    const uint32_t sig = a.sig ^ ((uint32_t)a.T << 8) ^ (uint32_t)a.gx;
+    if (a.hdr->ll_engaged != (sig | 1u) || a.hdr->ll_miss == 0u) return;
+    const uint32_t gy = (uint32_t)(a.T / a.gx), units = (uint32_t)a.NR * gy * (uint32_t)kMaxSegments;
+    for (uint32_t u = blockIdx.x; u < units; u += gridDim.x) {
+        const uint32_t r = u % (uint32_t)a.NR, y = (u / (uint32_t)a.NR) % gy, seg = u / ((uint32_t)a.NR * gy);
+        band_place_body<NC>(r, y, seg, a.rect_sorted, a.order, a.hdr, a.wave_lo, a.gx, a.NR, a.table, a.wtable, a.ranges,
+                            a.point_list, a.nseg, 1, sig, a.ll_limit, a.ll_miss);
+    }
 }
 
 #ifndef GSR_SCAN_MODE
@@ -474,9 +542,20 @@
 template <int THREADS, int MAXPER>
 __device__ __forceinline__ void band_starts_block(const uint32_t *totals, int T, GsrHeader *__restrict__ hdr,
                                                   uint32_t r_capacity, uint2 *__restrict__ ranges, uint32_t *s_wv,
-                                                  uint32_t *__restrict__ mirror) {
+                                                  uint32_t *__restrict__ mirror, const BandArgs *ll = nullptr) {
     constexpr int NWV = THREADS / GSR_WAVE;
     const int tid = (int)threadIdx.x, lane = gsr_lane(), wave = tid >> 6;
+    __shared__ uint32_t s_llsum;
+    const bool limits = GSR_LIST_LIMIT && ll != nullptr && ll->ll_limit != nullptr;
+    uint32_t ll_held = 0u;
+    if (limits) {
+        const uint32_t sig = ll->sig ^ ((uint32_t)T << 8) ^ (uint32_t)ll->gx;
+        if (hdr->ll_magic != GSR_LL_MAGIC || hdr->ll_sig != sig) ll_held |= 1u;
+        if (hdr->ll_miss > kLLGuardMin + (uint32_t)T / kLLGuardDiv) ll_held |= 2u;
+        if (ll->ll_td != 0u && hdr->td_reuse != 0u) ll_held |= 4u;
+        if (ll->ll_forced != 0u) ll_held = 8u | (ll->ll_forced << 8);
+        if (tid == 0) s_llsum = 0u;
+    }
     const int per = (T + THREADS - 1) / THREADS, t0 = tid * per;
     uint32_t v[MAXPER], sum = 0;
 #pragma unroll
@@ -508,11 +587,45 @@
         gsr_set_overflow(hdr, overflow, mirror);
         hdr->R = overflow ? 0u : grand;
     }
+    if (limits) {
+        uint32_t placed = 0u;
+#pragma unroll
+        for (int k = 0; k < MAXPER; k++) {
+            const int t = t0 + k;
+            if (k < per && t < T) {
+                uint32_t lim = v[k];
+                if ((ll_held & 8u) != 0u) {
+                    lim = min(lim, ll_held >> 8);
+                } else if (ll_held == 0u) {
+                    const uint32_t w = ll->ll_walked[t];
+                    lim = min(lim, (w + (w >> 2) + 64u + 63u) & ~63u);
+                }
+                if (overflow) lim = 0u;
+                ll->ll_limit[t] = lim;
+                ll->ll_miss[t] = 0u;
+                if ((ll_held & 4u) == 0u) ll->ll_walked[t] = 0u;
+                placed += lim;
+            }
+        }
+#pragma unroll
+        for (int o = 32; o > 0; o >>= 1) placed += (uint32_t)__shfl_xor((int)placed, o, 64);
+        if (lane == 0) atomicAdd(&s_llsum, placed);
+        __syncthreads();
+        if (tid == 0) {
+            hdr->ll_magic = overflow ? 0u : GSR_LL_MAGIC;
+            hdr->ll_sig = ll->sig ^ ((uint32_t)T << 8) ^ (uint32_t)ll->gx;
+            hdr->ll_engaged = overflow ? 0u : ((ll->sig ^ ((uint32_t)T << 8) ^ (uint32_t)ll->gx) | 1u);
+            hdr->ll_miss = 0u;
+            hdr->ll_repaired = 0u;
+            hdr->ll_placed = s_llsum;
+            hdr->ll_held = ll_held;
+        }
+    }
 }
 
 __device__ __forceinline__ void band_scan_starts_body(uint32_t *__restrict__ table, int T, GsrHeader *__restrict__ hdr,
                                                       uint32_t r_capacity, uint2 *__restrict__ ranges,
-                                                      uint32_t *__restrict__ mirror) {
+                                                      uint32_t *__restrict__ mirror, const BandArgs *ll) {
     __shared__ uint32_t s_tot[kSSMaxTiles];
     __shared__ uint32_t s_wv[kSSW];
     const int lane = gsr_lane(), wave = (int)(threadIdx.x >> 6);
@@ -535,7 +648,7 @@
         }
     }
     __syncthreads();
-    band_starts_block<kSST, kSSMaxTiles / kSST>(s_tot, T, hdr, r_capacity, ranges, s_wv, mirror);
+    band_starts_block<kSST, kSSMaxTiles / kSST>(s_tot, T, hdr, r_capacity, ranges, s_wv, mirror, ll);
 }
 
 __global__ __launch_bounds__(kSST) void band_scan_starts_kernel(const GsrBatch<BandArgs> bt) {
@@ -557,7 +670,7 @@
         gsr_tile_order_block_keys<32>(key, a.T, a.tile_order, s_bins, s_red);
         return;
     }
-    band_scan_starts_body(a.table, a.T, a.hdr, a.r_capacity, a.ranges_w, a.mirror);
+    band_scan_starts_body(a.table, a.T, a.hdr, a.r_capacity, a.ranges_w, a.mirror, &a);
 }
 __global__ __launch_bounds__(kBT) void band_scan_tail_kernel(const GsrBatch<BandArgs> bt) {
     const BandArgs &a = bt.f[blockIdx.y];
@@ -574,7 +687,7 @@
     if (s_last == 0u) return;
     __threadfence();
     if (threadIdx.x == 0) a.hdr->tile_queue = 0u;
-    band_starts_block<kBT, kSSMaxTiles / kBT>(a.totals, a.T, a.hdr, a.r_capacity, a.ranges_w, s_wv, a.mirror);
+    band_starts_block<kBT, kSSMaxTiles / kBT>(a.totals, a.T, a.hdr, a.r_capacity, a.ranges_w, s_wv, a.mirror, &a);
 }
 
 __global__ __launch_bounds__(kBT) void gather_rects_kernel(const uint32_t *__restrict__ order,
@@ -596,7 +709,7 @@
     return gsr_check_launch("gather_rects", debug, stream);
 }
 
-static void band_args(int B, const GsrFrame *fr, bool balanced, bool place, GsrBatch<BandArgs> &bt) {
+static void band_args(int B, const GsrFrame *fr, bool balanced, bool place, GsrBatch<BandArgs> &bt, int mode = 0) {
     for (int k = 0; k < B; k++) {
         const GeomState &g = fr[k].g;
         const GsrSettings &st = *fr[k].st_bin;
@@ -627,6 +740,13 @@
         a.tile_order = fr[k].img.tile_order;
         a.mirror = fr[k].out ? fr[k].out->overflow_mirror : (uint32_t *)nullptr;
         a.point_list = place ? fr[k].b.gidx[0] : (uint32_t *)nullptr;
+        const bool ll = GSR_LIST_LIMIT && fr[k].ll != 0;
+        a.ll_walked = ll ? fr[k].img.ll_walked : (uint32_t *)nullptr;
+        a.ll_limit = ll ? fr[k].img.ll_limit : (uint32_t *)nullptr;
+        a.ll_miss = ll ? fr[k].img.ll_miss : (uint32_t *)nullptr;
+        a.ll_forced = fr[k].ll >= 64 ? (uint32_t)fr[k].ll : 0u;
+        a.ll_td = (fr[k].pc && fr[k].td) ? 1u : 0u;
+        a.mode = mode;
     }
 }
 
@@ -661,11 +781,21 @@
     return gsr_check_launch("band_scan", debug, stream);
 }
 
-int gsr_launch_band_place(int B, const GsrFrame *fr, bool debug, hipStream_t stream) {
+int gsr_launch_band_place(int B, const GsrFrame *fr, bool debug, hipStream_t stream, int mode) {
     const GsrSettings &st = *fr[0].st_bin;
     const int gx = gsr_div_up(st.image_width, GSR_TILE), gy = gsr_div_up(st.image_height, GSR_TILE);
     GsrBatch<BandArgs> bt{};
-    band_args(B, fr, true, true, bt);
+    band_args(B, fr, true, true, bt, mode);
+    if (mode == 1) {
+        const dim3 rgrid(kRepairBlocks, B);
+        if (gx <= 64)
+            hipLaunchKernelGGL(band_place_repair_kernel<1>, rgrid, dim3(kBT), 0, stream, bt);
+        else if (gx <= 128)
+            hipLaunchKernelGGL(band_place_repair_kernel<2>, rgrid, dim3(kBT), 0, stream, bt);
+        else
+            hipLaunchKernelGGL(band_place_repair_kernel<4>, rgrid, dim3(kBT), 0, stream, bt);
+        return gsr_check_launch("band_place_repair", debug, stream);
+    }
     const dim3 grid(GSR_BAND_RANGES, gy, kMaxSegments * B);
     if (gx <= 64)
         hipLaunchKernelGGL(band_place_kernel<1>, grid, dim3(kBT), 0, stream, bt);
diff --git a/gsworld_amd/csrc/depthsort.hip b/gsworld_amd/csrc/depthsort.hip
--- a/gsworld_amd/csrc/depthsort.hip
+++ b/gsworld_amd/csrc/depthsort.hip
@@ -403,6 +403,7 @@
         hdr->R = 0u;
         hdr->overflow = 0u;
         hdr->coop_timeout_now = 0u;
+        hdr->ll_engaged = 0u;
         hdr->r_capacity = 0u;
         hdr->R_raw = 0u;
         hdr->tile_queue = 0u;
diff --git a/gsworld_amd/csrc/gsr_internal.h b/gsworld_amd/csrc/gsr_internal.h
--- a/gsworld_amd/csrc/gsr_internal.h
+++ b/gsworld_amd/csrc/gsr_internal.h
@@ -79,11 +79,22 @@
     uint32_t td_token;
     uint32_t td_reuse;
     uint32_t td_skipped;
-    uint32_t pad[8];
+    uint32_t ll_magic;
+    uint32_t ll_sig;
+    uint32_t ll_engaged;
+    uint32_t ll_miss;
+    uint32_t ll_repaired;
+    uint32_t ll_placed;
+    uint32_t ll_held;
+    uint32_t pad[1];
     uint32_t of_magic;
     uint32_t overflow_frames;
 };
 #define GSR_OF_MAGIC 0x0F10F10Fu
+#define GSR_LL_MAGIC 0x4C4C494Du
+#ifndef GSR_LIST_LIMIT
+#define GSR_LIST_LIMIT 1
+#endif
 #ifndef GSR_TILE_REUSE
 #define GSR_TILE_REUSE 1
 #endif
@@ -293,6 +304,9 @@
     uint32_t *split_count;
     uint32_t *quad_order;
     uint32_t *tile_dirty;
+    uint32_t *ll_walked;
+    uint32_t *ll_limit;
+    uint32_t *ll_miss;
     static ImageState carve(char *base, int32_t W, int32_t H, size_t *bytes = nullptr) {
         ImageState s;
         char *p = base;
@@ -308,6 +322,9 @@
         s.final_T = GeomState::take<float>(p, (size_t)W * H);
         s.n_contrib = GeomState::take<uint32_t>(p, (size_t)W * H);
         s.tile_dirty = GeomState::take<uint32_t>(p, tiles);
+        s.ll_walked = GeomState::take<uint32_t>(p, tiles);
+        s.ll_limit = GeomState::take<uint32_t>(p, tiles);
+        s.ll_miss = GeomState::take<uint32_t>(p, tiles);
         if (bytes) *bytes = (size_t)(p - base);
         return s;
     }
@@ -408,6 +425,7 @@
     uint32_t cap32;
     bool pc;
     bool td;
+    int ll;
 };
 
 struct GsrMapsArgs {
@@ -438,7 +456,8 @@
 int gsr_launch_gather_rects(int32_t P, const GeomState &g, bool debug, hipStream_t stream);
 int gsr_launch_band_count(int B, const GsrFrame *fr, bool balanced, bool merge_starts, bool *starts_done, bool debug,
                           hipStream_t stream);
-int gsr_launch_band_place(int B, const GsrFrame *fr, bool debug, hipStream_t stream);
+int gsr_launch_band_place(int B, const GsrFrame *fr, bool debug, hipStream_t stream, int mode = 0);
+int gsr_list_limit_mode();
 bool gsr_chunk_supported(int gx, int gy);
 int gsr_launch_chunk_count(const GsrSettings &st, int32_t P, const GeomState &g, bool debug, hipStream_t stream);
 int gsr_launch_chunk_place(const GsrSettings &st, int32_t P, const GeomState &g, const BinningState &b,
@@ -456,7 +475,7 @@
 int gsr_render_cus_per_xcd();
 int gsr_render_coop_blocks(const GsrSettings &st, int num_tiles, int frames);
 int gsr_launch_render(int B, const GsrFrame *fr, bool order_ready, bool split_ready, bool super_tiles, int coop_blocks,
-                      hipStream_t stream);
+                      hipStream_t stream, bool repair = false);
 int gsr_launch_maps(int B, const GsrMapsArgs *frames, bool debug, hipStream_t stream);
 int gsr_launch_tile_count(const GsrSettings &st, int32_t P, const GeomState &g, const ImageState &img,
                           uint32_t r_capacity, bool debug, hipStream_t stream);
diff --git a/gsworld_amd/csrc/render.hip b/gsworld_amd/csrc/render.hip
--- a/gsworld_amd/csrc/render.hip
+++ b/gsworld_amd/csrc/render.hip
@@ -431,14 +431,30 @@
 
 __device__ __forceinline__ uint32_t coop_load(volatile uint32_t *p) { return *p; }
 
-template <bool SUPER>
+struct StreamLL {
+    const uint32_t *limit;
+    uint32_t *walked, *miss;
+    int repair;
+};
+__device__ __forceinline__ bool stream_ll_finish(const StreamLL &ll, GsrHeader *hdr, int st, uint32_t consumed, bool short_list,
+                                                 bool any_alive, int lane) {
+    const bool missed = short_list && any_alive;
+    if (lane == 0) {
+        atomicMax(&ll.walked[st], consumed);
+        if (missed && atomicExch(&ll.miss[st], 1u) == 0u) atomicAdd(&hdr->ll_miss, 1u);
+    }
+    return missed;
+}
+
+template <bool SUPER, bool LL = false>
 __device__ __forceinline__ bool render_coop_quadrant(float4 (*s_list)[kStreamList / 2][6], CoopFlags *fl, const uint32_t q,
                                                      const uint2 *__restrict__ ranges,
                                                      const uint32_t *__restrict__ point_list,
                                                      const float4 *__restrict__ splat, int W, int H, int gx,
                                                      const float *__restrict__ bg, float *__restrict__ out_color,
                                                      float *__restrict__ out_invdepth, uint8_t *__restrict__ rgb8,
-                                                     uint32_t *__restrict__ quad_work, float *__restrict__ final_T) {
+                                                     uint32_t *__restrict__ quad_work, float *__restrict__ final_T,
+                                                     const StreamLL ll, GsrHeader *__restrict__ hdr) {
     static_assert(SUPER, "cooperative quadrants are an inference-frame path");
 #if GSR_STREAM_STAMPS
     const uint64_t stamp0 = __builtin_readcyclecounter();
@@ -449,8 +465,13 @@
     const int qy0 = (tile / gx) * GSR_TILE + ((quad >> 1) << 3);
     const uint32_t tx = (uint32_t)(tile % gx), ty = (uint32_t)(tile / gx);
     constexpr int kSX = GSR_SUPER_SX, kSY = GSR_SUPER_SY;
-    const uint2 range = ranges[(int)((ty >> kSY) * (uint32_t)((gx + (1 << kSX) - 1) >> kSX) + (tx >> kSX))];
-    const int n_inst = (int)(range.y - range.x);
+    const int st = (int)((ty >> kSY) * (uint32_t)((gx + (1 << kSX) - 1) >> kSX) + (tx >> kSX));
+    const uint2 range = ranges[st];
+    const int n_full = (int)(range.y - range.x);
+    int n_inst = n_full;
+    if constexpr (LL) {
+        if (ll.limit != nullptr) n_inst = min(n_full, (int)ll.limit[st]);
+    }
     const uint32_t *src = point_list + range.x;
     const int rounds = (n_inst + GSR_WAVE - 1) / GSR_WAVE;
     const float4 zero4 = make_float4(0.f, 0.f, 0.f, 0.f);
@@ -516,7 +537,8 @@
     v2f acc_rg = {0.f, 0.f}, acc_bd = {0.f, 0.f};
     uint32_t work = 0;
     bool timed_out = false;
-    for (int rd = 0; rd < rounds; rd++) {
+    int rd = 0;
+    for (; rd < rounds; rd++) {
         if (__builtin_amdgcn_ballot_w64(T > 0.0f) == 0ull) break;
         const int w = 1 + rd % kCoopCullers;
         const uint32_t want = (uint32_t)(rd / kCoopCullers) + 1u;
@@ -580,6 +602,12 @@
     }
     if (lane == 0) *stop = 1u;
     if (quad_work != nullptr && lane == 0) quad_work[q] = work;
+    if constexpr (LL) {
+        if (ll.walked != nullptr && !timed_out &&
+            stream_ll_finish(ll, hdr, st, (uint32_t)min(rd * GSR_WAVE, n_inst), n_inst < n_full,
+                             __builtin_amdgcn_ballot_w64(T > 0.0f) != 0ull, lane))
+            return false;
+    }
 #if GSR_STREAM_STAMPS
     if (lane == 0) {
         const uint64_t stamp1 = __builtin_readcyclecounter();
@@ -609,7 +637,7 @@
     return timed_out;
 }
 
-template <bool SUPER>
+template <bool SUPER, bool LL = false>
 __device__ __forceinline__ void render_stream_body(const uint2 *__restrict__ ranges,
                                                                   const uint32_t *__restrict__ point_list,
                                                                   const float4 *__restrict__ splat, int W, int H, int gx,
@@ -630,7 +658,8 @@
                                                                   const uint32_t *__restrict__ coop_list,
                                                                   int coop_blocks, GsrHeader *__restrict__ hdr,
                                                                   const uint32_t wgx ,
-                                                                  const uint32_t *__restrict__ tile_dirty = nullptr) {
+                                                                  const uint32_t *__restrict__ tile_dirty = nullptr,
+                                                                  const StreamLL ll = StreamLL{nullptr, nullptr, nullptr, 0}) {
     __shared__ float4 s_list[GSR_BLOCK / GSR_WAVE][kStreamList / 2][6];
     const int lane = gsr_lane(), wave = gsr_wave();
     const uint32_t *dirty = nullptr;
@@ -652,8 +681,8 @@
                 if (threadIdx.x == 0) hdr->td_skipped = 1u;
                 return;
             }
-            const bool timed_out = render_coop_quadrant<true>(s_list, &s_coop, q, ranges, point_list, splat, W, H, gx, bg,
-                                                              out_color, out_invdepth, rgb8, quad_work, final_T);
+            const bool timed_out = render_coop_quadrant<true, LL>(s_list, &s_coop, q, ranges, point_list, splat, W, H, gx, bg,
+                                                              out_color, out_invdepth, rgb8, quad_work, final_T, ll, hdr);
             if (timed_out && lane == 0) gsr_note_coop_timeout(hdr);
             return;
         }
@@ -703,8 +732,17 @@
         const float yext = half == 0 ? 7.0f : 3.0f;
         const uint32_t tx = (uint32_t)(tile % gx), ty = (uint32_t)(tile / gx);
         constexpr int kSX = GSR_SUPER_SX, kSY = GSR_SUPER_SY;
-        const uint2 range = ranges[SUPER ? (int)((ty >> kSY) * (uint32_t)((gx + (1 << kSX) - 1) >> kSX) + (tx >> kSX)) : tile];
-        const int n_inst = (int)(range.y - range.x);
+        const int st = SUPER ? (int)((ty >> kSY) * (uint32_t)((gx + (1 << kSX) - 1) >> kSX) + (tx >> kSX)) : tile;
+        if constexpr (LL) if (ll.repair != 0) {
+            if (ll.miss[st] == 0u) continue;
+            if (quad == 0 && (tx & ((1u << kSX) - 1u)) == 0u && (ty & ((1u << kSY) - 1u)) == 0u && lane == 0)
+                atomicAdd(&hdr->ll_repaired, 1u);
+        }
+        const uint2 range = ranges[st];
+        int n_inst = (int)(range.y - range.x);
+        if constexpr (LL) {
+            if (ll.limit != nullptr) n_inst = min(n_inst, (int)ll.limit[st]);
+        }
         const uint32_t *src = point_list + range.x;
 
 #if GSR_STREAM_STAMPS
@@ -730,7 +768,8 @@
         }
         const int rounds = (n_inst + kStreamRound - 1) / kStreamRound;
         uint32_t work = 0;
-        for (int rd = 0; rd < rounds; rd++) {
+        int rd = 0;
+        for (; rd < rounds; rd++) {
             if (__builtin_amdgcn_ballot_w64(T > 0.0f) == 0ull) break;
             int n_surv = 0;
             uint64_t unsafe = 0ull;
@@ -813,6 +852,14 @@
             __builtin_amdgcn_wave_barrier();
         }
         if (quad_work != nullptr && lane == 0) (half == 2 ? quad_work_b : quad_work)[4 * tile + quad] = work;
+        if constexpr (LL) if (ll.walked != nullptr) {
+            int st2 = st;
+            asm volatile("" : "+v"(st2));
+            const uint2 rg = ranges[st2];
+            if (stream_ll_finish(ll, hdr, st2, (uint32_t)min(rd * kStreamRound, n_inst), n_inst < (int)(rg.y - rg.x),
+                                 __builtin_amdgcn_ballot_w64(T > 0.0f) != 0ull, lane))
+                continue;
+        }
 #if GSR_STREAM_STAMPS
         if (SUPER && lane == 0) {
             const uint64_t stamp1 = __builtin_readcyclecounter();
@@ -868,6 +915,10 @@
     int frames;
     const uint32_t *tile_dirty;
 };
+struct RenderStreamLLArgs {
+    RenderStreamArgs a;
+    StreamLL ll;
+};
 template <bool SUPER>
 __global__ __launch_bounds__(GSR_BLOCK) __attribute__((amdgpu_waves_per_eu(5))) void render_stream_kernel(
     const GsrBatch<RenderStreamArgs> bt) {
@@ -882,6 +933,18 @@
                               a.main_blocks, a.split_flag, a.split_list, a.split_count, a.quad_work_b, a.quad_order,
                               a.coop_list, a.coop_blocks, a.hdr, wgx, a.tile_dirty);
 }
+__global__ __launch_bounds__(GSR_BLOCK) __attribute__((amdgpu_waves_per_eu(5))) void render_stream_ll_kernel(
+    const GsrBatch<RenderStreamLLArgs> bt) {
+    const RenderStreamArgs &a = bt.f[blockIdx.y].a;
+    const StreamLL &ll = bt.f[blockIdx.y].ll;
+    const uint32_t wgx = blockIdx.x;
+    if ((int)wgx >= a.total_blocks) return;
+    if (ll.repair != 0 && a.hdr->ll_miss == 0u) return;
+    render_stream_body<true, true>(a.ranges, a.point_list, a.splat, a.W, a.H, a.gx, a.num_tiles, a.tile_order, a.bg,
+                                   a.out_color, a.out_invdepth, a.final_T, a.n_contrib, a.rgb8, a.quad_work, a.num_cus,
+                                   a.main_blocks, a.split_flag, a.split_list, a.split_count, a.quad_work_b, a.quad_order,
+                                   a.coop_list, a.coop_blocks, a.hdr, wgx, a.tile_dirty, ll);
+}
 
 __global__ __launch_bounds__(GSR_BLOCK) void tile_order_kernel(const uint2 *__restrict__ ranges, int num_tiles,
                                                                uint32_t *__restrict__ order) {
@@ -981,7 +1044,7 @@
 }
 
 int gsr_launch_render(int B, const GsrFrame *fr, bool order_ready, bool split_ready, bool super_tiles, int coop_blocks,
-                      hipStream_t stream) {
+                      hipStream_t stream, bool repair) {
     const GsrSettings &st = *fr[0].st;
     const int W = st.image_width, H = st.image_height;
     const int gx = gsr_div_up(W, GSR_TILE), gy = gsr_div_up(H, GSR_TILE);
@@ -1001,16 +1064,22 @@
         const int T = gx * gy;
         const bool ordered = gsr_render_wants_tile_order(st, T);
         const uint32_t *order = ordered ? img.tile_order : nullptr;
-        if (ordered && !order_ready)
+        if (repair && (rc.variant != 4 || !super_tiles)) {
+            gsr_set_error("gsr_launch_render: the second pass belongs to the default compositor of inference frames");
+            return GSR_E_INVALID;
+        }
+        if (ordered && !order_ready && !repair)
             for (int k = 0; k < B; k++)
                 hipLaunchKernelGGL(tile_order_kernel, dim3(1), dim3(GSR_BLOCK), 0, stream, fr[k].img.ranges, T,
                                    fr[k].img.tile_order);
-        const int blocks = min(T, render_num_cus() * rc.blocks_per_cu);
+        const int blocks = repair ? gsr_div_up(gsr_div_up(T, 4), GSR_XCDS) * GSR_XCDS : min(T, render_num_cus() * rc.blocks_per_cu);
         if (rc.variant == 4) {
-            const int coop = super_tiles && split_ready ? coop_blocks : 0;
-            const int extra = coop > 0 ? coop : (split_ready && T <= 2048 ? gsr_render_split_blocks(st, T) : 0);
-            const bool use_qorder = split_ready && gsr_render_uses_quad_order(st, T);
+            const int coop = super_tiles && split_ready && !repair ? coop_blocks : 0;
+            const int extra = repair ? 0 : (coop > 0 ? coop : (split_ready && T <= 2048 ? gsr_render_split_blocks(st, T) : 0));
+            const bool use_qorder = split_ready && !repair && gsr_render_uses_quad_order(st, T);
             GsrBatch<RenderStreamArgs> bt{};
+            GsrBatch<RenderStreamLLArgs> btl{};
+            bool any_ll = false;
             for (int k = 0; k < B; k++) {
                 const ImageState &im = fr[k].img;
                 RenderStreamArgs &a = bt.f[k];
@@ -1018,7 +1087,7 @@
                 a.point_list = fr[k].b.gidx[0];
                 a.splat = fr[k].g.splat;
                 a.W = W; a.H = H; a.gx = gx; a.num_tiles = T;
-                a.tile_order = ordered ? im.tile_order : (const uint32_t *)nullptr;
+                a.tile_order = ordered && !repair ? im.tile_order : (const uint32_t *)nullptr;
                 a.bg = fr[k].in->background;
                 a.out_color = fr[k].out->out_color;
                 a.out_invdepth = fr[k].out->out_invdepth;
@@ -1039,14 +1108,25 @@
                 a.quad_work_b = im.quad_work_b;
                 a.quad_order = use_qorder ? im.quad_order : (const uint32_t *)nullptr;
                 a.tile_dirty = (fr[k].pc && fr[k].td) ? im.tile_dirty : (const uint32_t *)nullptr;
-            }
+                const bool ll = GSR_LIST_LIMIT && super_tiles && fr[k].ll != 0;
+                any_ll = any_ll || ll;
+                StreamLL &l = btl.f[k].ll;
+                l.limit = ll && !repair ? im.ll_limit : (const uint32_t *)nullptr;
+                l.walked = ll ? im.ll_walked : (uint32_t *)nullptr;
+                l.miss = ll ? im.ll_miss : (uint32_t *)nullptr;
+                l.repair = ll && repair ? 1 : 0;
+            }
+            if (repair && !any_ll) return GSR_OK;
             const int row = B > 1 ? (blocks + extra + GSR_XCDS - 1) / GSR_XCDS * GSR_XCDS : blocks + extra;
 #ifndef GSR_RENDER_INTERLEAVE
 #define GSR_RENDER_INTERLEAVE 0
 #endif
             const dim3 grid = (GSR_RENDER_INTERLEAVE && B > 1) ? dim3(row * B, 1) : dim3(row, B > 1 ? B : 1);
             if (B == 1) bt.f[0].frames = 1;
-            if (super_tiles)
+            if (any_ll) {
+                for (int k = 0; k < B; k++) btl.f[k].a = bt.f[k];
+                hipLaunchKernelGGL(render_stream_ll_kernel, dim3(row, B), dim3(GSR_BLOCK), 0, stream, btl);
+            } else if (super_tiles)
                 hipLaunchKernelGGL(render_stream_kernel<true>, grid, dim3(GSR_BLOCK), 0, stream, bt);
             else
                 hipLaunchKernelGGL(render_stream_kernel<false>, grid, dim3(GSR_BLOCK), 0, stream, bt);
diff --git a/gsworld_amd/csrc/sort.hip b/gsworld_amd/csrc/sort.hip
--- a/gsworld_amd/csrc/sort.hip
+++ b/gsworld_amd/csrc/sort.hip
@@ -53,6 +53,7 @@
         hdr->R = 0u;
         hdr->overflow = 0u;
         hdr->coop_timeout_now = 0u;
+        hdr->ll_engaged = 0u;
         hdr->r_capacity = 0u;
         hdr->R_raw = 0u;
         hdr->tile_queue = 0u;
diff --git a/gsworld_amd/debug.py b/gsworld_amd/debug.py
--- a/gsworld_amd/debug.py
+++ b/gsworld_amd/debug.py
@@ -33,6 +33,20 @@
     _lib.TUNING["render_variant"] = {4: 0, 0: 1, 2: 2, 3: 3}[variant]
     if blocks_per_cu > 0:
         _lib.TUNING["render_blocks_per_cu"] = blocks_per_cu
+
+
+def set_list_limit(mode) -> None:
+    m = -1 if mode is False else (1 if mode is True else (0 if mode is None else int(mode)))
+    check(lib().gsr_debug_set_list_limit(m))
+
+
+def list_limit_state(geomBuffer: torch.Tensor) -> dict:
+    out = (C.c_int32 * 8)()
+    with torch.cuda.device(geomBuffer.device):
+        check(lib().gsr_debug_list_limit_state(C.c_void_p(geomBuffer.data_ptr()), out,
+                                               C.c_void_p(torch.cuda.current_stream(geomBuffer.device).cuda_stream)))
+    return dict(engaged=bool(out[0]), misses=int(out[1]), repaired=int(out[2]), placed=int(out[3]), instances=int(out[4]),
+                held=int(out[5]) & 0xFF, record=bool(out[6]))
 
 
 def _view(buf: torch.Tensor, ptr, count: int, dtype: torch.dtype) -> torch.Tensor:
diff --git a/include/gsr.h b/include/gsr.h
--- a/include/gsr.h
+++ b/include/gsr.h
@@ -121,6 +121,8 @@
 int gsr_debug_ss_stamps(int32_t P, int32_t width, int32_t height, const void *geom, uint64_t *out64);
 
 int gsr_debug_sort_state(const void *geom, int32_t out[8], void *stream);
+int gsr_debug_set_list_limit(int32_t mode);
+int gsr_debug_list_limit_state(const void *geom, int32_t out[8], void *stream);
 
 int gsr_frame_stats(const void *geom, GsrFrameStats *stats, void *stream);
 
```

Result: faster. 14760 (median of 6 runs) (+2.4%).
